# LeSN-Lab/diff-ViT

Hardware: AMD Instinct MI355X
Metric: images/sec DeiT-S int8 224^2 b=256 (quantized forward) (higher is better)
Workload: dtype int8; 1 GPU; deit_small PoT-PTQ forward, bit_config=[8]*50, 224x224, batch 256 per GPU; global_batch=256, parallelism=dp1, streams_per_gpu=3, collective=none, ranks_seen=1, distinct_devices=1

## Files before the change

diff-vit_amd/csrc/p2vit_attn.hip:

```cpp
#include "p2vit_attn_lis.h"

#define WA_HD 32
#define WA_KEYS 64
#define WA_DEAD(kb, r) (NT > 0 && (kb) * 16 + (r) >= NT)
#define WA_PAD(kb, r) (!(NT > 0 && (kb) * 16 + 12 + (r) < NT))
template <int NT, bool TAP>
__global__ __launch_bounds__(256, 3) void k_window_attention(std::conditional_t<TAP, WinAttnArgs, WinAttnKArgs> a) {
  constexpr int VSTRIDE = WA_KEYS + 4;
  __shared__ __attribute__((aligned(16))) int8_t sK[4][WA_KEYS * WA_HD];
  __shared__ __attribute__((aligned(16))) unsigned short sVt[4][WA_HD * VSTRIDE];
  __shared__ float sT[4][232];
  __shared__ __attribute__((aligned(16))) unsigned short sP[4][4][16];
  __shared__ unsigned short sMeta[WA_KEYS + 16];
  __shared__ long long lutE[258];
  __shared__ double lutFR[258];
  const int tid = threadIdx.x, lane = tid & 63, wave = tid >> 6, g = lane >> 4, l15 = lane & 15;
  const int ws = a.wa.ws, N = ws * ws, nW = a.wa.n_windows;
  const int hgroups = (a.H + 3) >> 2;
  const int blk = blockIdx.x;
  const int hg = blk % hgroups, w = (blk / hgroups) % nW, b = blk / (hgroups * nW);
  const int head = hg * 4 + wave;
  const int C = a.H * WA_HD;
  const long long ldq = a.wa.qkv_stride ? a.wa.qkv_stride : 3 * C, ldo = a.wa.out_stride ? a.wa.out_stride : C;
  const bool hok = head < a.H;
  const bool live = lane < N;
  const int rowj = a.wa.win_index[w * N + (live ? lane : 0)];
  const int tsz = (2 * ws - 1) * (2 * ws - 1);
  int8_t tcode[4] = {0, 0, 0, 0};
#pragma unroll
  for (int i = 0; i < 4; ++i)
    if (hok && lane + 64 * i < tsz) tcode[i] = a.wa.table_codes[(lane + 64 * i) * a.H + head];
  int reg_t = 0;
  if (a.wa.region && tid < N) reg_t = (int)a.wa.region[w * N + tid];
  for (int t = tid; t < 258; t += (int)blockDim.x) {
    int xi = -t;
    const int lim = 32 * a.wa.x0_int;
    xi = (xi < lim || t >= 256) ? lim : xi;
    const int q = xi / a.wa.x0_int;
    const int r = xi - a.wa.x0_int * q;
    const long long z = (long long)r * (r + a.wa.b_int) + a.wa.c_int;
    long long e = z << (32 - q);
    e = e < 0 ? 0 : e;
    if (t == 257) e = 0;
    const float ef = t == 257 ? 1.0f : (float)e;
    lutE[t] = e;
    lutFR[t] = 1.0 / (double)ef;
  }
  if (tid < WA_KEYS + 16) {
    const int t = tid < N ? tid : 0;
    sMeta[tid] = (unsigned short)(((t / ws) * (2 * ws - 1) + (t % ws)) | (reg_t << 10));
  }
  const int8_t* hbase = a.qkv + (long long)b * a.T * ldq + head * WA_HD;
  uint4 k0 = make_uint4(0, 0, 0, 0), k1 = k0, v0 = k0, v1 = k0;
  if (hok && live) {
    const int8_t* base = hbase + (long long)rowj * ldq;
    k0 = *reinterpret_cast<const uint4*>(base + C);
    k1 = *reinterpret_cast<const uint4*>(base + C + 16);
    v0 = *reinterpret_cast<const uint4*>(base + 2 * C);
    v1 = *reinterpret_cast<const uint4*>(base + 2 * C + 16);
  }
  int rowq_next = __shfl(rowj, l15 < N ? l15 : N - 1);
  v4i qc_next = {0, 0, 0, 0};
  if (hok) qc_next = *reinterpret_cast<const v4i*>(hbase + (long long)rowq_next * ldq + (g & 1) * 16);
  const float inv_sa = 1.0f / a.wa.s_attn, inv_s2 = 1.0f / a.wa.s_q2;
  const float tb_mul = a.wa.s_table * inv_s2, a1_mul = a.wa.s_attn * inv_s2;
#pragma unroll
  for (int i = 0; i < 4; ++i)
    if (lane + 64 * i < tsz) sT[wave][lane + 64 * i] = (float)tcode[i] * tb_mul;
  {
    *reinterpret_cast<uint4*>(&sK[wave][lane * WA_HD]) = k0;
    *reinterpret_cast<uint4*>(&sK[wave][lane * WA_HD + 16]) = k1;
    const unsigned vw[8] = {v0.x, v0.y, v0.z, v0.w, v1.x, v1.y, v1.z, v1.w};
#pragma unroll
    for (int c = 0; c < WA_HD; ++c) {
      const float f = (float)sx8(vw[c >> 2], c & 3);
      sVt[wave][c * VSTRIDE + lane] = (unsigned short)(__float_as_uint(f) >> 16);
    }
  }
  __syncthreads();
  if (!hok) return;
  const float sigma = a.wa.s_q1 * a.wa.qk_scale;
  const float inv_u = __uint_as_float((unsigned)(254 - (int)(__float_as_uint(sigma) >> 23) + 23) << 23);
  const float sig_m = sigma * inv_u;
  const double sig_int = (double)sig_m;
  const float x_mul = ((1.0f / inv_u) * a.wa.s_q1) * inv_sa;
  const float m100 = (float)(int)(100.0f * inv_s2);
  const float av_mul = (a.wa.s_q1 / a.wa.s_q3) * P2V_PROB_SCALE;
  const int c0 = (ws - 1) * (2 * ws - 1) + (ws - 1);
  const int nqb = (N + 15) >> 4;
  int linj[4][4];
  unsigned regj[4][4];
#pragma unroll
  for (int kb = 0; kb < 4; ++kb)
#pragma unroll
    for (int r = 0; r < 4; ++r) {
      const unsigned mj = sMeta[kb * 16 + 4 * g + r];
      linj[kb][r] = (int)(mj & 1023u);
      regj[kb][r] = mj >> 10;
    }
  for (int qb = 0; qb < nqb; ++qb) {
    const int qi = qb * 16 + l15;
    const int qr = qi < N ? qi : N - 1;
    const int rowq = rowq_next;
    const v4i qc = qc_next;
    if (qb + 1 < nqb) {
      const int qn = qi + 16 < N ? qi + 16 : N - 1;
      rowq_next = __shfl(rowj, qn);
      qc_next = *reinterpret_cast<const v4i*>(hbase + (long long)rowq_next * ldq + (g & 1) * 16);
    }
    unsigned eh[2];
    {
      const unsigned qh[2] = {(unsigned)(g < 2 ? qc[0] : qc[2]), (unsigned)(g < 2 ? qc[1] : qc[3])};
#pragma unroll
      for (int d = 0; d < 2; ++d) {
        float et[4];
#pragma unroll
        for (int e = 0; e < 4; ++e) {
          const float cf = (float)sx8(qh[d], e);
          const float v = cf * sig_m;
          et[e] = __builtin_fmaf(-cf, sig_m, v);
        }
        eh[d] = pack4_pre(et[0], et[1], et[2], et[3]);
      }
    }
    const auto up0 = __builtin_amdgcn_permlane32_swap(0u, eh[0], false, false);
    const auto up1 = __builtin_amdgcn_permlane32_swap(0u, eh[1], false, false);
    const v4i qeta = {(int)up0[0], (int)up1[0], (int)eh[0], (int)eh[1]};
    const v4i fq1 = g < 2 ? qc : (v4i){0, 0, 0, 0};
    const v4i fq2 = g < 2 ? (v4i){0, 0, 0, 0} : qeta;
    v4i s1[4], s2[4];
#pragma unroll
    for (int kb = 0; kb < 4; ++kb) {
      const v4i fk = *reinterpret_cast<const v4i*>(&sK[wave][(kb * 16 + l15) * WA_HD + (g & 1) * 16]);
      s1[kb] = __builtin_amdgcn_mfma_i32_16x16x64_i8(fk, fq1, (v4i){0, 0, 0, 0}, 0, 0, 0);
      s2[kb] = __builtin_amdgcn_mfma_i32_16x16x64_i8(fk, fq2, (v4i){0, 0, 0, 0}, 0, 0, 0);
    }
    const unsigned mi = sMeta[qr];
    const float* trow = &sT[wave][(int)(mi & 1023u) + c0];
    const unsigned reg_i = mi >> 10;
    v4i pb[2];
    if (NT == 49 && qb == 3) {
      const int t = l15 < 13 ? l15 : 12;
      int v1 = s1[0][0], v2 = s2[0][0];
#pragma unroll
      for (int u = 1; u < 13; ++u) {
        const int kb = u < 12 ? u >> 2 : 3, r = u < 12 ? u & 3 : 0;
        v1 = t == u ? s1[kb][r] : v1;
        v2 = t == u ? s2[kb][r] : v2;
      }
      const int j = t < 12 ? (t >> 2) * 16 + 4 * g + (t & 3) : 48 + 4 * g;
      const bool valid = l15 < 13 && j < N;
      const unsigned mj = sMeta[j];
      const double X = __builtin_fma(sig_int, (double)v1, (double)v2);
      const float a1 = __builtin_amdgcn_fmed3f(rintf((float)X * x_mul), -128.f, 127.f);
      const float a2 = __builtin_amdgcn_fmed3f(rintf(__builtin_fmaf(a1, a1_mul, trow[-(int)(mj & 1023u)])), -128.f, 127.f);
      float xi = a2;
      if (a.wa.region) xi -= (mj >> 10) != reg_i ? m100 : 0.f;
      xi = valid ? xi : -3.0e9f;
      float mx = xi;
#define WA_ROWMAX(ctrl) mx = fmaxf(mx, __int_as_float(__builtin_amdgcn_update_dpp(0, __float_as_int(mx), ctrl, 0xF, 0xF, false)));
      WA_ROWMAX(0xB1) WA_ROWMAX(0x4E) WA_ROWMAX(0x141) WA_ROWMAX(0x140)
#undef WA_ROWMAX
      mx = fmaxf(mx, __shfl_xor(mx, 16));
      mx = fmaxf(mx, __shfl_xor(mx, 32));
      const int d = valid ? (int)fminf(mx - xi, 256.f) : 257;
      long long S = lutE[d];
#pragma unroll
      for (int o_ = 1; o_ < 64; o_ <<= 1) S += __shfl_xor(S, o_);
      const double Sd = (double)(float)S;
      const float ratio = rintf((float)(Sd * lutFR[d]));
      const int E = (int)((__float_as_uint(ratio) + 0x00400000u) >> 23);
      if constexpr (TAP) if (valid) {
        const long long trow = (((long long)b * nW + w) * a.H + head) * N + (N - 1);
        if (a.probs_k) a.probs_k[trow * N + j] = (int8_t)(E - 127 > 16 ? 16 : E - 127);
        if (a.probs_kp) a.probs_kp[trow * a.pitch + j] = (int8_t)(E - 127 > 16 ? 16 : E - 127);
        if (a.attn1_codes) a.attn1_codes[trow * a.pitch + j] = (int8_t)(int)a1;
        if (a.qact2_codes) a.qact2_codes[trow * a.pitch + j] = (int8_t)(int)a2;
      }
      sP[wave][g][l15] = (unsigned short)((E < 143 && l15 < 13) ? (143 - E) << 7 : 0);
      __builtin_amdgcn_wave_barrier();
      asm volatile("" ::: "memory");
      pb[0] = *reinterpret_cast<const v4i*>(&sP[wave][g][0]);
      pb[1] = *reinterpret_cast<const v4i*>(&sP[wave][g][8]);
    } else {
      float xs[4][4];
      float mx = -3.0e9f;
      auto scores = [&](auto MASKc) {
        constexpr bool MASK = decltype(MASKc)::value;
#pragma unroll
        for (int kb = 0; kb < 4; ++kb) {
#pragma unroll
          for (int r = 0; r < 4; ++r) {
            if (WA_DEAD(kb, r)) continue;
            const double X = __builtin_fma(sig_int, (double)s1[kb][r], (double)s2[kb][r]);
            const float a1 = __builtin_amdgcn_fmed3f(rintf((float)X * x_mul), -128.f, 127.f);
            const float a2 = __builtin_amdgcn_fmed3f(rintf(__builtin_fmaf(a1, a1_mul, trow[-linj[kb][r]])), -128.f, 127.f);
            float xi = a2;
            if constexpr (TAP) if (qi < N && kb * 16 + 4 * g + r < N) {
              const long long at = ((((long long)b * nW + w) * a.H + head) * N + qi) * a.pitch + kb * 16 + 4 * g + r;
              if (a.attn1_codes) a.attn1_codes[at] = (int8_t)(int)a1;
              if (a.qact2_codes) a.qact2_codes[at] = (int8_t)(int)a2;
            }
            if (MASK) xi -= regj[kb][r] != reg_i ? m100 : 0.f;
            if (WA_PAD(kb, r)) xi = kb * 16 + 4 * g + r < N ? xi : -3.0e9f;
            xs[kb][r] = xi;
            mx = fmaxf(mx, xi);
          }
        }
      };
      if (a.wa.region) scores(std::integral_constant<bool, true>{});
      else scores(std::integral_constant<bool, false>{});
      mx = fmaxf(mx, __shfl_xor(mx, 16));
      mx = fmaxf(mx, __shfl_xor(mx, 32));
      long long S = 0;
#pragma unroll
      for (int kb = 0; kb < 4; ++kb)
#pragma unroll
        for (int r = 0; r < 4; ++r) {
          if (WA_DEAD(kb, r)) continue;
          int d = (int)fminf(mx - xs[kb][r], 256.f);
          if (WA_PAD(kb, r)) d = kb * 16 + 4 * g + r < N ? d : 257;
          s1[kb][r] = d;
          S += lutE[d];
        }
      S += __shfl_xor(S, 16);
      S += __shfl_xor(S, 32);
      const float Sf = (float)S;
      const double Sd = (double)Sf;
#pragma unroll
      for (int p = 0; p < 2; ++p) {
        unsigned pk[4];
#pragma unroll
        for (int e2 = 0; e2 < 4; ++e2) {
          float ratio[2];
#pragma unroll
          for (int e = 0; e < 2; ++e) {
            const int jj = 2 * e2 + e;
            const int kb = 2 * p + (jj >> 2), r = jj & 3;
            if (WA_DEAD(kb, r)) {
              ratio[e] = 4.0e9f;
              continue;
            }
            ratio[e] = rintf((float)(Sd * lutFR[s1[kb][r]]));
            if constexpr (TAP) if (qi < N && kb * 16 + 4 * g + r < N) {
              const int k = (int)((__float_as_uint(ratio[e]) + 0x00400000u) >> 23) - 127;
              const long long trow = (((long long)b * nW + w) * a.H + head) * N + qi;
              if (a.probs_k) a.probs_k[trow * N + kb * 16 + 4 * g + r] = (int8_t)(k > 16 ? 16 : k);
              if (a.probs_kp) a.probs_kp[trow * a.pitch + kb * 16 + 4 * g + r] = (int8_t)(k > 16 ? 16 : k);
            }
          }
          pk[e2] = lis_prob_pair(ratio[0], ratio[1]);
        }
        pb[p] = (v4i){(int)pk[0], (int)pk[1], (int)pk[2], (int)pk[3]};
      }
    }
    v4f o[2] = {(v4f){0.f, 0.f, 0.f, 0.f}, (v4f){0.f, 0.f, 0.f, 0.f}};
#pragma unroll
    for (int p = 0; p < 2; ++p) {
      const v8bf fb = __builtin_bit_cast(v8bf, pb[p]);
#pragma unroll
      for (int dt = 0; dt < 2; ++dt) {
        const unsigned short* vp = &sVt[wave][(dt * 16 + l15) * VSTRIDE + p * 32 + 4 * g];
        const uint2 lo = *reinterpret_cast<const uint2*>(vp);
        const uint2 hi = *reinterpret_cast<const uint2*>(vp + 16);
        v4i va = {(int)lo.x, (int)lo.y, (int)hi.x, (int)hi.y};
        o[dt] = __builtin_amdgcn_mfma_f32_16x16x32_bf16(__builtin_bit_cast(v8bf, va), fb, o[dt], 0, 0, 0);
      }
    }
    if (qi < N) {
      int8_t* dst = a.out + ((long long)b * a.T + rowq) * ldo + head * WA_HD + 4 * g;
#pragma unroll
      for (int dt = 0; dt < 2; ++dt)
        *reinterpret_cast<unsigned*>(dst + dt * 16) = pack4_rne_sat(o[dt][0] * av_mul, o[dt][1] * av_mul, o[dt][2] * av_mul, o[dt][3] * av_mul);
    }
  }
}


int g_attn_waves = 8;
int p2v_launch_window_attention_wide(const WinAttnArgs& a, hipStream_t st);
int p2v_launch_window_attention(const WinAttnArgs& a, hipStream_t st) {
  if (a.wa.ws > 8) return p2v_launch_window_attention_wide(a, st);
  const int hgroups = (a.H + 3) / 4;
  const dim3 grid((unsigned)(a.B * a.wa.n_windows * hgroups));
  if (a.wa.ws == 7) {
    if (a.tapped()) hipLaunchKernelGGL((k_window_attention<49, true>), grid, dim3(256), 0, st, a);
    else hipLaunchKernelGGL((k_window_attention<49, false>), grid, dim3(256), 0, st, a);
  } else {
    if (a.tapped()) hipLaunchKernelGGL((k_window_attention<0, true>), grid, dim3(256), 0, st, a);
    else hipLaunchKernelGGL((k_window_attention<0, false>), grid, dim3(256), 0, st, a);
  }
  CHECK_LAUNCH();
  return 0;
}

int p2v_launch_attention_wide(const AttnArgs& a, int head_dim, int nkb, hipStream_t st);

int g_attn_stream = 0;
int g_attn_packed = 1;
int p2v_attention_kernel_of(int head_dim, int tokens, int tapped) {
  const int resident = p2v_resident_tokens_of(head_dim);
  if (!resident || tokens <= 0 || tokens > P2V_MAX_TOKENS_STREAMED) return -1;
  if (g_attn_stream) return P2V_KERNEL_STREAMING;
  if (tokens <= resident) return P2V_KERNEL_RESIDENT;
  if (g_attn_packed && head_dim == 64 && !tapped && tokens <= P2V_MAX_TOKENS_PACKED) return P2V_KERNEL_PACKED;
  return P2V_KERNEL_STREAMING;
}

int p2v_launch_attention(const AttnArgs& a, int head_dim, hipStream_t st) {
  const int nkb = (a.N + 31) / 32;
  {
    int ex;
    const float m2 = a.at.s_qkv_sq * a.at.inv_s_attn;
    if (!(m2 > 0.f) || frexpf(m2, &ex) != 0.5f) return -2;
  }
  switch (p2v_attention_kernel_of(head_dim, a.N, a.tapped())) {
    case P2V_KERNEL_RESIDENT: break;
    case P2V_KERNEL_PACKED: return p2v_launch_attention_packed(a, st);
    case P2V_KERNEL_STREAMING: return p2v_launch_attention_stream(a, head_dim, st);
    default: return -1;
  }
  if (head_dim == 64) { P2V_ATTN_CASES(64, 19, true) }
  if (head_dim == 32) { P2V_ATTN_CASES(32, 19, false) }
  return p2v_launch_attention_wide(a, head_dim, nkb, st);
}
```

diff-vit_amd/csrc/p2vit_attn_lis.h:

```cpp
#pragma once
#include "p2vit_device.h"

extern int g_attn_waves;


#define P2V_PROB_SCALE 0x1p111f
__device__ __forceinline__ unsigned lis_prob_pair(float r0, float r1) {
  const unsigned hi2 = __builtin_amdgcn_perm(__float_as_uint(r1), __float_as_uint(r0), 0x07060302u);
  const unsigned eb = __builtin_bit_cast(unsigned, __builtin_bit_cast(v2u16, hi2) + (v2u16){0x40, 0x40}) & 0x7F807F80u;
  unsigned out;
  asm("v_pk_sub_u16 %0, %1, %2 clamp" : "=v"(out) : "s"(0x47804780u), "v"(eb));
  return out;
}

__device__ __forceinline__ void lis_table_entry(const p2v_attn& at, int t, long long* lutE, double* lutFR) {
  if (t >= 256) {
    lutE[256] = 0;
    lutFR[256] = 1.0;
    return;
  }
  int xi = -t;
  const int lim = 32 * at.x0_int;
  xi = xi < lim ? lim : xi;
  const int q = xi / at.x0_int;
  const int r = xi - at.x0_int * q;
  const long long z = (long long)r * (r + at.b_int) + at.c_int;
  long long e = z << (32 - q);
  e = e < 0 ? 0 : e;
  lutE[t] = e;
  lutFR[t] = 1.0 / (double)(float)e;
}

#ifdef P2V_DIAG
extern unsigned long long* g_gemm_stamps;
#define AT_STAMP(slot)                                                                                             \
  do {                                                                                                             \
    if (a.stamps && threadIdx.x == 0 && (slot) < 16) a.stamps[(long long)blockIdx.x * 16 + (slot)] = __builtin_readcyclecounter(); \
  } while (0)
#else
#define AT_STAMP(slot) do { } while (0)
#endif
template <int HD, int NKP, bool TAP, bool ISH>
__global__ __launch_bounds__(512, HD > 64 ? 2 : (NKP <= 7 ? 4 : (NKP <= 10 ? 3 : 2))) void k_lis_attention(std::conditional_t<TAP, AttnArgs, AttnKArgs> a) {
  static_assert(HD % 16 == 0 && HD >= 16 && HD <= 128, "head_dim");
  constexpr int KROWS = NKP * 32;
  constexpr int NKB = NKP * 2;
  constexpr int VSTRIDE = KROWS + 4;
  constexpr int CH = HD / 16;
  constexpr int NQ = (CH + 3) / 4;
  constexpr int NDT = HD / 16;
  extern __shared__ __attribute__((aligned(16))) unsigned char smem[];
  int8_t* sK = reinterpret_cast<int8_t*>(smem);
  unsigned short* sVt = reinterpret_cast<unsigned short*>(smem + KROWS * HD);
  unsigned char* lutE = smem + KROWS * HD + HD * VSTRIDE * 2;
  unsigned char* lutFR = lutE + 258 * 8;
  typedef __attribute__((address_space(3))) const long long* lds_i64p;
  typedef __attribute__((address_space(3))) const double* lds_f64p;
  const int ebase = (int)(unsigned)(uintptr_t)(__attribute__((address_space(3))) unsigned char*)lutE;

  const int tid = threadIdx.x, lane = tid & 63, wave = tid >> 6, g = lane >> 4, l15 = lane & 15;
  const int b = blockIdx.x / a.H, head = blockIdx.x % a.H;
  const int N = a.N, D = a.H * HD, ld = 3 * D;
  const int8_t* base = a.qkv + (long long)b * N * ld + head * HD;
  AT_STAMP(0);

  if (tid < 256) {
    int xi = -tid;
    const int lim = 32 * a.at.x0_int;
    xi = xi < lim ? lim : xi;
    const int q = xi / a.at.x0_int;
    const int r = xi - a.at.x0_int * q;
    const long long z = (long long)r * (r + a.at.b_int) + a.at.c_int;
    long long e = z << (32 - q);
    e = e < 0 ? 0 : e;
    const float ef = (float)e;
    reinterpret_cast<long long*>(lutE)[tid] = e;
    reinterpret_cast<double*>(lutFR)[tid] = 1.0 / (double)ef;
    if (tid == 0) {
      reinterpret_cast<long long*>(lutE)[256] = 0;
      reinterpret_cast<double*>(lutFR)[256] = 1.0;
    }
  }
  AT_STAMP(1);
  for (int i0 = tid; i0 < KROWS * CH; i0 += 2 * (int)blockDim.x) {
    uint4 kv[2], vv[2];
#pragma unroll
    for (int u = 0; u < 2; ++u) {
      const int i = i0 + u * (int)blockDim.x;
      const int row = i / CH, c = i % CH;
      kv[u] = make_uint4(0, 0, 0, 0);
      vv[u] = make_uint4(0, 0, 0, 0);
      if (i < KROWS * CH && row < N) {
        kv[u] = *reinterpret_cast<const uint4*>(base + (long long)row * ld + D + c * 16);
        vv[u] = *reinterpret_cast<const uint4*>(base + (long long)row * ld + 2 * D + c * 16);
      }
    }
#pragma unroll
    for (int u = 0; u < 2; ++u) {
      const int i = i0 + u * (int)blockDim.x;
      if (i >= KROWS * CH) break;
      const int row = i / CH, c = i % CH;
      const int sw = (HD == 64) ? (c ^ (((row >> 3) & 1) << 1)) : c;
      *reinterpret_cast<uint4*>(sK + row * HD + sw * 16) = kv[u];
      const unsigned w4[4] = {vv[u].x, vv[u].y, vv[u].z, vv[u].w};
#pragma unroll
      for (int j = 0; j < 16; ++j) {
        const float f = (float)sx8(w4[j >> 2], j & 3);
        sVt[(c * 16 + j) * VSTRIDE + row] = (unsigned short)(__float_as_uint(f) >> 16);
      }
    }
  }

  const float nmm = -(a.at.qk_scale * (a.at.s_qkv_sq * a.at.inv_s_attn));
  const float avm = a.at.av_mul * P2V_PROB_SCALE;
  const int nqb = ((a.nq > 0 && a.nq < N ? a.nq : N) + 15) >> 4;
  const int nwaves = (int)(blockDim.x >> 6);
  AT_STAMP(2);
  v4i fq_next[NQ];
#pragma unroll
  for (int j = 0; j < NQ; ++j) {
    fq_next[j] = (v4i){0, 0, 0, 0};
    if (4 * j + g < CH && wave < nqb) {
      const int qr0 = wave * 16 + l15;
      fq_next[j] = *reinterpret_cast<const v4i*>(base + (long long)(qr0 < N ? qr0 : N - 1) * ld + (4 * j + g) * 16);
    }
  }
  __syncthreads();
  AT_STAMP(3);
  [[maybe_unused]] int stamp_base = 4;
  for (int qb = wave; qb < nqb; qb += nwaves) {
    const int qrow = qb * 16 + l15;
    v4i fq[NQ];
#pragma unroll
    for (int j = 0; j < NQ; ++j) {
      fq[j] = fq_next[j];
      if (4 * j + g < CH && qb + nwaves < nqb) {
        const int qn = (qb + nwaves) * 16 + l15;
        fq_next[j] = *reinterpret_cast<const v4i*>(base + (long long)(qn < N ? qn : N - 1) * ld + (4 * j + g) * 16);
      }
    }
    v4i s[NKB];
#pragma unroll
    for (int kb = 0; kb < NKB; ++kb) {
      const int row = kb * 16 + l15;
#pragma unroll
      for (int j = 0; j < NQ; ++j) {
        const bool live = 4 * j + g < CH;
        const int c = live ? 4 * j + g : 0;
        const int sw = (HD == 64) ? (c ^ (((row >> 3) & 1) << 1)) : c;
        v4i fk = *reinterpret_cast<const v4i*>(sK + row * HD + sw * 16);
        if (!live) fk = (v4i){0, 0, 0, 0};
        if (j == 0) s[kb] = __builtin_amdgcn_mfma_i32_16x16x64_i8(fk, fq[0], (v4i){0, 0, 0, 0}, 0, 0, 0);
        else s[kb] = __builtin_amdgcn_mfma_i32_16x16x64_i8(fk, fq[j], s[kb], 0, 0, 0);
      }
    }
    const bool tail_empty = (NKB - 1) * 16 >= N;
#ifdef P2V_DIAG
    asm volatile("s_nop 0" :: "v"(s[NKB - 1][0]));
#endif
    AT_STAMP(stamp_base);
    long long S = 0;
    [[maybe_unused]] int rowmax = 0;
    if (ISH) {
      const int p = a.pshift, hm1 = (1 << (p - 1)) - 1;
      int mx = -100000;
#pragma unroll
      for (int kb = 0; kb < NKB; ++kb) {
        if (kb == NKB - 1 && tail_empty) continue;
#pragma unroll
        for (int r = 0; r < 4; ++r) {
          const int sv = s[kb][r];
          int code = (int)((unsigned)sv + (unsigned)hm1 + (((unsigned)sv >> p) & 1u)) >> p;
          code = code < -128 ? -128 : (code > 127 ? 127 : code);
          if (kb >= NKB - 2) code = (kb * 16 + 4 * g + r) < N ? code : -100000;
          s[kb][r] = code;
          mx = code > mx ? code : mx;
        }
      }
      {
        int o = __shfl_xor(mx, 16);
        mx = o > mx ? o : mx;
        o = __shfl_xor(mx, 32);
        mx = o > mx ? o : mx;
      }
      if (TAP) rowmax = mx;
      const int mx8 = (mx << 3) + ebase;
#pragma unroll
      for (int kb = 0; kb < NKB; ++kb) {
        if (kb == NKB - 1 && tail_empty) continue;
#pragma unroll
        for (int r = 0; r < 4; ++r) {
          int d8;
          asm("v_mad_i32_i24 %0, %1, -8, %2" : "=v"(d8) : "v"(s[kb][r]), "v"(mx8));
          if (kb >= NKB - 2) d8 = d8 > ebase + 2048 ? ebase + 2048 : d8;
          s[kb][r] = d8;
          S += *(lds_i64p)(uintptr_t)(unsigned)d8;
        }
        __builtin_amdgcn_sched_barrier(0);
      }
    } else {
    int mn = 1000;
#pragma unroll
    for (int kb = 0; kb < NKB; ++kb) {
      if (kb == NKB - 1 && tail_empty) continue;
#pragma unroll
      for (int r = 0; r < 4; ++r) {
        int nc = (int)__builtin_amdgcn_fmed3f(rintf((float)s[kb][r] * nmm), -127.f, 128.f);
        if (kb >= NKB - 2) nc = (kb * 16 + 4 * g + r) < N ? nc : 1000;
        s[kb][r] = nc;
        mn = nc < mn ? nc : mn;
      }
    }
    {
      int o = __shfl_xor(mn, 16);
      mn = o < mn ? o : mn;
      o = __shfl_xor(mn, 32);
      mn = o < mn ? o : mn;
    }
    if (TAP) rowmax = -mn;
    const int neg8mn = -8 * mn + ebase;
#pragma unroll
    for (int kb = 0; kb < NKB; ++kb) {
      if (kb == NKB - 1 && tail_empty) continue;
#pragma unroll
      for (int r = 0; r < 4; ++r) {
        int d8 = (s[kb][r] << 3) + neg8mn;
        if (kb >= NKB - 2) d8 = d8 > ebase + 2048 ? ebase + 2048 : d8;
        s[kb][r] = d8;
        S += *(lds_i64p)(uintptr_t)(unsigned)d8;
      }
      __builtin_amdgcn_sched_barrier(0);
    }
    }
    S += __shfl_xor(S, 16);
    S += __shfl_xor(S, 32);
    const float Sf = (float)S;
    const double Sd = (double)Sf;
    AT_STAMP(stamp_base + 1);

    v4f o[NDT];
#pragma unroll
    for (int dt = 0; dt < NDT; ++dt) o[dt] = (v4f){0.f, 0.f, 0.f, 0.f};
#pragma unroll
    for (int p = 0; p < NKP; ++p) {
      unsigned pk[4];
#pragma unroll
      for (int e2 = 0; e2 < 4; ++e2) {
        float ratio[2];
#pragma unroll
        for (int e = 0; e < 2; ++e) {
          const int j = 2 * e2 + e;
          const int kb = 2 * p + (j >> 2), r = j & 3;
          if (kb == NKB - 1 && tail_empty) {
            ratio[e] = 4.0e9f;
            continue;
          }
          const double rd = ((lds_f64p)(uintptr_t)(unsigned)s[kb][r])[258];
          ratio[e] = rintf((float)(Sd * rd));
          if constexpr (TAP) if (s[kb][r] < ebase + 2048 && qrow < N) {
            int k = (int)((__float_as_uint(ratio[e]) + 0x00400000u) >> 23) - 127;
            const int key = kb * 16 + 4 * g + r;
            const long long trow = ((long long)b * a.H + head) * N + qrow;
            if (a.probs_k) a.probs_k[trow * N + key] = (int8_t)(k > 16 ? 16 : k);
            if (a.probs_kp) a.probs_kp[trow * a.pitch + key] = (int8_t)(k > 16 ? 16 : k);
            if (a.score_codes) a.score_codes[trow * a.pitch + key] = (int8_t)(rowmax - ((s[kb][r] - ebase) >> 3));
          }
        }
        pk[e2] = lis_prob_pair(ratio[0], ratio[1]);
      }
      v4i pb = {(int)pk[0], (int)pk[1], (int)pk[2], (int)pk[3]};
      const v8bf fb = __builtin_bit_cast(v8bf, pb);
#pragma unroll
      for (int dt = 0; dt < NDT; ++dt) {
        const unsigned short* vp = sVt + (dt * 16 + l15) * VSTRIDE + p * 32 + 4 * g;
        const uint2 lo = *reinterpret_cast<const uint2*>(vp);
        const uint2 hi = *reinterpret_cast<const uint2*>(vp + 16);
        v4i va = {(int)lo.x, (int)lo.y, (int)hi.x, (int)hi.y};
        o[dt] = __builtin_amdgcn_mfma_f32_16x16x32_bf16(__builtin_bit_cast(v8bf, va), fb, o[dt], 0, 0, 0);
      }
      __builtin_amdgcn_sched_barrier(0);
    }
#ifdef P2V_DIAG
    asm volatile("s_nop 0" :: "v"(o[NDT - 1][0]));
#endif
    AT_STAMP(stamp_base + 2);
    {
      const int qs = qrow < N ? qrow : N - 1;
      int8_t* dst = a.out + ((long long)b * N + qs) * D + head * HD + 4 * g;
#pragma unroll
      for (int dt = 0; dt < NDT; ++dt)
        *reinterpret_cast<unsigned*>(dst + dt * 16) = pack4_rne_sat(o[dt][0] * avm, o[dt][1] * avm, o[dt][2] * avm, o[dt][3] * avm);
    }
    AT_STAMP(stamp_base + 3);
    stamp_base += 4;
  }
}

template <int HD, int NKB, bool ISH_OK = true>
static int launch_attn_t(const AttnArgs& a_, hipStream_t st) {
  constexpr int KROWS = NKB * 32;
  constexpr size_t smem = (size_t)KROWS * HD + (size_t)HD * (KROWS + 4) * 2 + 258 * 8 + 258 * 8;
  AttnArgs a = a_;
  {
    int ex;
    const float m = a.at.qk_scale * (a.at.s_qkv_sq * a.at.inv_s_attn);
    a.pshift = (m > 0.f && frexpf(m, &ex) == 0.5f && ex <= 0 && ex >= -23) ? 1 - ex : 0;
  }
#ifdef P2V_DIAG
  a.stamps = g_gemm_stamps;
#endif
  const dim3 grid(a.B * a.H), block(64 * g_attn_waves);
#define P2V_ATTN_LAUNCH(TAP_, ISH_)                                                                                          \
  do {                                                                                                                       \
    if (smem > 64 * 1024) {                      \
      static bool granted[16] = {false};                                                                                     \
      int dev = 0;                                                                                                           \
      if (hipGetDevice(&dev) != hipSuccess || dev < 0 || dev >= 16) dev = -1;                                                \
      if (dev < 0 || !granted[dev]) {                                                                                        \
        hipError_t e = hipFuncSetAttribute(reinterpret_cast<const void*>(&k_lis_attention<HD, NKB, TAP_, ISH_>),             \
                                           hipFuncAttributeMaxDynamicSharedMemorySize, (int)smem);                           \
        if (e != hipSuccess) return (int)e;                                                                                  \
        if (dev >= 0) granted[dev] = true;                                                                                   \
      }                                                                                                                      \
    }                                                                                                                        \
    hipLaunchKernelGGL((k_lis_attention<HD, NKB, TAP_, ISH_>), grid, block, smem, st, a);                                    \
  } while (0)
  if constexpr (!ISH_OK) a.pshift = 0;
  if (a.tapped()) {
    if constexpr (ISH_OK) { if (a.pshift) { P2V_ATTN_LAUNCH(true, true); CHECK_LAUNCH(); return 0; } }
    P2V_ATTN_LAUNCH(true, false);
  } else {
    if constexpr (ISH_OK) { if (a.pshift) { P2V_ATTN_LAUNCH(false, true); CHECK_LAUNCH(); return 0; } }
    P2V_ATTN_LAUNCH(false, false);
  }
// ... 16 lines not shown
```

diff-vit_amd/csrc/p2vit_capi.cpp:

```cpp
#include <hip/hip_runtime.h>
#include <math.h>
#include <stdarg.h>
#include <stdio.h>
#include <stdlib.h>
#include <string.h>

#include <initializer_list>
#include <memory>
#include <vector>

#include "p2vit_kernels.h"

static thread_local char g_err[512] = "";

static int fail(int code, const char* fmt, ...) {
  va_list ap;
  va_start(ap, fmt);
  vsnprintf(g_err, sizeof g_err, fmt, ap);
  va_end(ap);
  return code;
}
struct KeepLastError {
  char keep[sizeof g_err];
  KeepLastError() { memcpy(keep, g_err, sizeof keep); }
  ~KeepLastError() { memcpy(g_err, keep, sizeof keep); }
};
static int launch_rc(int rc, const char* what) {
  if (rc == 0) return 0;
  if (rc == -2) return fail(P2V_E_UNSUPPORTED, "%s: s_qkv_sq * inv_s_attn must be a power of two", what);
  if (rc < 0) return fail(P2V_E_UNSUPPORTED, "%s: no kernel instantiated for this shape", what);
  return fail(P2V_E_LAUNCH, "%s: %s", what, hipGetErrorString((hipError_t)rc));
}
static inline int round_up(int v, int m) { return (v + m - 1) / m * m; }
static bool is_pot(float v) {
  int ex;
  return v > 0.f && frexpf(v, &ex) == 0.5f;
}

static int check_lis_consts(const char* who, int x0_int, int b_int, int c_int) {
  if (x0_int >= 0) return fail(P2V_E_ARG, "%s: x0_int must be negative", who);
  if (c_int <= 0 || c_int >= (1 << 24) || b_int < 0 || b_int >= (1 << 23) || x0_int < -(1 << 12))
    return fail(P2V_E_UNSUPPORTED, "%s: log-int-softmax constants out of range (x0 %d, b %d, c %d): softmax input scale below 2^-11?", who, x0_int,
                b_int, c_int);
  return P2V_OK;
}
static int check_requant_scale(const char* who, float inv_s_out) {
  if (!(is_pot(inv_s_out) && inv_s_out >= 0x1p-40f && inv_s_out <= 0x1p40f))
    return fail(P2V_E_UNSUPPORTED, "%s: REQUANT 1/scale %g must be a power of two (it is folded into the column scales)", who, inv_s_out);
  return P2V_OK;
}
static int check_gelu_tab(const char* who, const p2v_gelu_tab& t) {
  if (t.table && (t.cells <= 0 || t.cells > 4096)) return fail(P2V_E_ARG, "%s: GELU table with %d cells", who, t.cells);
  return P2V_OK;
}
static int check_attn(const char* who, const p2v_attn& at) {
  const int rc = check_lis_consts(who, at.x0_int, at.b_int, at.c_int);
  if (rc != P2V_OK) return rc;
  if (!is_pot(at.s_qkv_sq * at.inv_s_attn)) return fail(P2V_E_UNSUPPORTED, "%s: s_qkv_sq * inv_s_attn must be a power of two", who);
  if (!(at.qk_scale > 0.f) || !(at.av_mul > 0.f)) return fail(P2V_E_ARG, "%s: qk_scale and av_mul must be positive", who);
  if (!is_pot(at.av_mul) || at.av_mul > 0x1p15f || at.av_mul < 0x1p-40f)
    return fail(P2V_E_UNSUPPORTED, "%s: av_mul %g must be a power of two in [2^-40, 2^15]", who, at.av_mul);
  return P2V_OK;
}

struct p2v_plan {
  p2v_model_desc d;
  int tokens, patches, k_patch, k_patch_pad, n_layers;
  std::vector<p2v_linear> lin[2];
  std::vector<char> lin_set[2];
  float inv_s_input;
  p2v_epilogue embed_epi;
  const int8_t* cls_codes;
  const int8_t* embed_cls_codes = nullptr;
  bool embed_set;
  std::vector<p2v_block> blocks;
  std::vector<char> block_set;
  p2v_ln final_ln;
  float head_inv_s, head_s;
  bool head_set;
  std::vector<float*> ln_pre_buf;
  float* final_pre_buf = nullptr;
  std::vector<char> block_folded;
  std::vector<const float*> resid_tab;
  std::vector<float*> resid_buf;
  int device = -1;
  ~p2v_plan() {
    int prev = -1;
    const bool sw = device >= 0 && hipGetDevice(&prev) == hipSuccess && prev != device && hipSetDevice(device) == hipSuccess;
    for (float* b : ln_pre_buf)
      if (b) (void)hipFree(b);
    for (float* b : resid_buf)
      if (b) (void)hipFree(b);
    if (final_pre_buf) (void)hipFree(final_pre_buf);
    if (sw) (void)hipSetDevice(prev);
  }
};

static void build_resid_tables(p2v_plan* plan, int block);
static int bit_index(int bits) { return bits == 4 ? 0 : (bits == 8 ? 1 : -1); }
template <class Block>
static auto& block_ln(Block& b, int i) { return i < 2 ? b.ln1[i] : b.ln2[(i - 2) >> 1][(i - 2) & 1]; }
static bool ln_constants_present(const p2v_ln& l, bool with_mask = true) {
  return (l.mask || !with_mask) && l.gamma && l.beta && l.inv_out && l.post_mul;
}

extern "C" {

extern int g_ln_generic;
extern int g_ln_rows;
extern int g_attn_waves;
extern int g_ln_gemm;
extern int g_ln_gemm_ver;
extern int g_gemm_tile;
extern int g_resid_pre;
extern int g_attn_stream;
extern int g_attn_packed;
extern int g_ln_pre;
extern int g_gemm_rows;
int g_cls_rows = 1;

enum { ANY_ENV = 1, ANY_API = 2 };
static const struct Switch {
  const char *name, *env;
  int* var;
  int lo, hi, step, any;
  bool takes(int v, int how) const { return (any & how) || (v >= lo && v <= hi && (v - lo) % step == 0); }
  void set(int v) const { *var = (hi == 1 && lo == 0) ? v != 0 : v; }
} kSwitches[] = {
    {"attn_waves", "P2V_ATTN_WAVES", &g_attn_waves, 4, 8, 1, 0},
    {"ln_gemm", "P2V_LN_GEMM", &g_ln_gemm, 0, 1, 1, ANY_ENV | ANY_API},
    {"ln_gemm_version", "P2V_LN_GEMM_V", &g_ln_gemm_ver, 1, 3, 1, 0},
    {"gemm_tile", "P2V_GEMM_TILE", &g_gemm_tile, 0, 256, 128, 0},
    {"attn_stream", "P2V_ATTN_STREAM", &g_attn_stream, 0, 1, 1, ANY_ENV | ANY_API},
    {"attn_packed", "P2V_ATTN_PACKED", &g_attn_packed, 0, 1, 1, 0},
    {"ln_pre", "P2V_LN_PRE", &g_ln_pre, 0, 1, 1, ANY_ENV | ANY_API},
    {"resid_pre", "P2V_RESID_PRE", &g_resid_pre, 0, 1, 1, ANY_ENV | ANY_API},
    {"gemm_rows", "P2V_GEMM_ROWS", &g_gemm_rows, 0, 2, 1, 0},
    {"cls_rows", "P2V_CLS_ROWS", &g_cls_rows, 0, 1, 1, ANY_ENV},
    {"ln_rows", "P2V_LN_ROWS", &g_ln_rows, 1, 64, 1, 0},
    {"ln_generic", "P2V_LN_GENERIC", &g_ln_generic, 0, 1, 1, ANY_API},
};

static void read_env_once() {
  static bool done = false;
  if (done) return;
  done = true;
  for (const Switch& s : kSwitches) {
    const char* e = getenv(s.env);
    if (e && s.takes(atoi(e), ANY_ENV)) s.set(atoi(e));
  }
}
int p2v_abi_version(void) { read_env_once(); return P2V_ABI_VERSION; }

int p2v_resident_tokens(int head_dim) { return p2v_resident_tokens_of(head_dim); }
int p2v_max_tokens(int head_dim) { return p2v_resident_tokens_of(head_dim) ? P2V_MAX_TOKENS_STREAMED : 0; }
int p2v_packed_tokens(int head_dim) { return head_dim == 64 ? P2V_MAX_TOKENS_PACKED : 0; }
int p2v_attention_kernel(int head_dim, int tokens, int tapped) {
  read_env_once();
  return p2v_attention_kernel_of(head_dim, tokens, tapped);
}

int p2v_set_tuning(const char* name, int value) {
  if (!name) return fail(P2V_E_ARG, "p2v_set_tuning: null name");
  read_env_once();
  for (const Switch& s : kSwitches)
    if (!strcmp(name, s.name) && s.takes(value, ANY_API)) {
      s.set(value);
      return P2V_OK;
    }
  return fail(P2V_E_ARG, "p2v_set_tuning: unknown switch or value out of range: %s = %d", name, value);
}
const char* p2v_last_error(void) { return g_err; }

int p2v_plan_create(const p2v_model_desc* desc, p2v_plan** out) {
  if (!desc || !out) return fail(P2V_E_ARG, "p2v_plan_create: null argument");
  read_env_once();
  if (desc->abi_version != P2V_ABI_VERSION) return fail(P2V_E_ARG, "ABI version %d != %d", desc->abi_version, P2V_ABI_VERSION);
  const p2v_model_desc& d = *desc;
  if (d.img_size <= 0 || d.patch_size <= 0 || d.img_size % d.patch_size) return fail(P2V_E_SHAPE, "img_size %% patch_size != 0");
  if (d.patch_size % 4) return fail(P2V_E_UNSUPPORTED, "patch_size must be a multiple of 4");
  if (d.embed_dim % d.num_heads) return fail(P2V_E_SHAPE, "embed_dim %% num_heads != 0");
  const int hd = d.embed_dim / d.num_heads;
  if (hd != 32 && hd != 48 && hd != 64 && hd != 80 && hd != 96 && hd != 128)
    return fail(P2V_E_UNSUPPORTED, "head_dim %d (32, 48, 64, 80, 96 and 128 are instantiated)", hd);
  if (d.embed_dim % 16 || d.mlp_hidden % 16) return fail(P2V_E_UNSUPPORTED, "embed_dim and mlp_hidden must be multiples of 16");
  {
    const int tokens = (d.img_size / d.patch_size) * (d.img_size / d.patch_size) + 1;
    if (tokens > P2V_MAX_TOKENS_STREAMED)
      return fail(P2V_E_UNSUPPORTED, "%d tokens per image: the attention kernels cover up to %d", tokens, P2V_MAX_TOKENS_STREAMED);
  }
  if (d.embed_dim > 2048) return fail(P2V_E_UNSUPPORTED, "embed_dim %d: the LayerNorm kernel covers up to 2048 channels", d.embed_dim);
  p2v_plan* p = new p2v_plan();
  p->d = d;
  p->patches = (d.img_size / d.patch_size) * (d.img_size / d.patch_size);
  p->tokens = p->patches + 1;
  p->k_patch = d.in_chans * d.patch_size * d.patch_size;
  p->k_patch_pad = round_up(p->k_patch, GBK_PAD);
  p->n_layers = 4 * d.depth + 2;
  for (int b = 0; b < 2; ++b) {
    p->lin[b].assign(p->n_layers, p2v_linear{nullptr, nullptr, nullptr, nullptr, 0});
    p->lin_set[b].assign(p->n_layers, 0);
  }
  p->blocks.resize(d.depth);
  p->block_set.assign(d.depth, 0);
  p->ln_pre_buf.assign(d.depth, nullptr);
  p->block_folded.assign(d.depth, 0);
  p->resid_tab.assign((size_t)d.depth * 4, nullptr);
  p->resid_buf.assign(d.depth, nullptr);
  p->embed_set = p->head_set = false;
  p->cls_codes = nullptr;
  *out = p;
  return P2V_OK;
}

void p2v_plan_destroy(p2v_plan* plan) { delete plan; }

int p2v_plan_set_linear(p2v_plan* plan, int layer, int bits, const p2v_linear* lin) {
  if (!plan || !lin) return fail(P2V_E_ARG, "p2v_plan_set_linear: null argument");
  const int bi = bit_index(bits);
  if (bi < 0) return fail(P2V_E_BITS, "bits %d not in {4, 8}", bits);
  if (layer < 0 || layer >= plan->n_layers) return fail(P2V_E_ARG, "layer %d out of range [0,%d)", layer, plan->n_layers);
  if (!lin->w_codes || !lin->colscale || !lin->bias) return fail(P2V_E_ARG, "p2v_plan_set_linear: null device pointer");
  if (lin->packed4 && bits != 4) return fail(P2V_E_BITS, "packed4 weights for a %d-bit layer", bits);
  plan->lin[bi][layer] = *lin;
  plan->lin_set[bi][layer] = 1;
  if (layer >= 1 && layer < plan->n_layers - 1 && ((layer - 1) & 1)) {
    const int block = (layer - 1) / 4;
    if (plan->block_set[block]) build_resid_tables(plan, block);
  }
  return P2V_OK;
}

int p2v_plan_set_embed(p2v_plan* plan, float inv_s_input, const p2v_epilogue* e, const int8_t* cls_row_codes) {
  if (!plan || !e || !cls_row_codes) return fail(P2V_E_ARG, "p2v_plan_set_embed: null argument");
  plan->inv_s_input = inv_s_input;
  plan->embed_epi = *e;
  plan->embed_epi.patches = plan->patches;
  plan->cls_codes = cls_row_codes;
  plan->embed_set = true;
  return P2V_OK;
}

int p2v_plan_set_embed_tap_cls(p2v_plan* plan, const int8_t* cls_embed_codes) {
  if (!plan || !cls_embed_codes) return fail(P2V_E_ARG, "p2v_plan_set_embed_tap_cls: null argument");
  plan->embed_cls_codes = cls_embed_codes;
  return P2V_OK;
}

struct OwnerDevice {
  int prev = -1, own = -1;
  explicit OwnerDevice(const void* ptr) {
    hipPointerAttribute_t pa;
    if (hipGetDevice(&prev) != hipSuccess || hipPointerGetAttributes(&pa, ptr) != hipSuccess) {
      (void)hipGetLastError();
      return;
    }
    if (pa.type != hipMemoryTypeDevice && pa.type != hipMemoryTypeManaged) return;
    own = pa.device;
    if (own != prev && hipSetDevice(own) != hipSuccess) own = -1;
  }
  ~OwnerDevice() { if (own >= 0 && own != prev) (void)hipSetDevice(prev); }
  bool ok() const { return own >= 0; }
};

static size_t resid_tab_floats(int N) { return (size_t)((N + 127) / 128) * 6 * 128; }

static int resid_prefold_impl(const p2v_linear& lin, const p2v_epilogue& ep, int N, float* tab, int* usable, hipStream_t st) {
  *usable = 0;
  unsigned* flags = nullptr;
  hipError_t e = hipMalloc(&flags, 2 * sizeof(unsigned));
  const unsigned init[2] = {1u, 0u};
  unsigned got[2] = {0u, 0u};
  if (e == hipSuccess) e = hipMemcpyAsync(flags, init, sizeof init, hipMemcpyHostToDevice, st);
  int rc = 0;
  if (e == hipSuccess) rc = p2v_launch_resid_prefold(lin, ep, N, tab, flags, st);
  if (e == hipSuccess && rc == 0) e = hipMemcpyAsync(got, flags, sizeof got, hipMemcpyDeviceToHost, st);
  if (e == hipSuccess && rc == 0) e = hipStreamSynchronize(st);
  if (flags) (void)hipFree(flags);
  if (e != hipSuccess) {
    (void)hipGetLastError();
    return fail(P2V_E_LAUNCH, "resid_prefold: %s", hipGetErrorString(e));
  }
  if (rc) return launch_rc(rc, "resid_prefold");
  *usable = got[0] ? 1 : 0;
  return P2V_OK;
}

static void build_resid_tables(p2v_plan* plan, int block) {
  KeepLastError keep;
  for (int j = 0; j < 4; ++j) plan->resid_tab[(size_t)block * 4 + j] = nullptr;
  if (!plan->block_set[block]) return;
  const p2v_block& blk = plan->blocks[block];
  OwnerDevice dev(blk.proj_epi.s_mid);
  if (!dev.ok() || (plan->device >= 0 && plan->device != dev.own)) return;
  const int D = plan->d.embed_dim;
  const size_t per = resid_tab_floats(D);
  if (hipDeviceSynchronize() != hipSuccess) { (void)hipGetLastError(); return; }
  float* buf = plan->resid_buf[block];
  if (!buf && hipMalloc(&buf, 4 * per * sizeof(float)) != hipSuccess) { (void)hipGetLastError(); return; }
  plan->resid_buf[block] = buf;
  plan->device = dev.own;
  for (int which = 0; which < 2; ++which)
    for (int bi = 0; bi < 2; ++bi) {
      const int layer = 1 + 4 * block + (which ? 3 : 1);
      if (!plan->lin_set[bi][layer]) continue;
      int usable = 0;
      float* tab = buf + (size_t)(which * 2 + bi) * per;
      if (resid_prefold_impl(plan->lin[bi][layer], which ? blk.fc2_epi : blk.proj_epi, D, tab, &usable, nullptr) == P2V_OK && usable)
        plan->resid_tab[(size_t)block * 4 + which * 2 + bi] = tab;
    }
}

static hipError_t fold_one_ln(const p2v_ln& l, int C, float* dev, p2v_ln_pre* out) {
  const int Cp = round_up(C, 256);
  std::vector<float> g(C), b(C), io(C), pm(C), host((size_t)2 * Cp, 0.f);
  hipError_t e = hipMemcpy(g.data(), l.gamma, C * sizeof(float), hipMemcpyDeviceToHost);
  if (e == hipSuccess) e = hipMemcpy(b.data(), l.beta, C * sizeof(float), hipMemcpyDeviceToHost);
  if (e == hipSuccess) e = hipMemcpy(io.data(), l.inv_out, C * sizeof(float), hipMemcpyDeviceToHost);
  if (e == hipSuccess) e = hipMemcpy(pm.data(), l.post_mul, C * sizeof(float), hipMemcpyDeviceToHost);
  if (e != hipSuccess) return e;
  float* go = host.data();
  float* bo = go + Cp;
  int pot = 1, pm1 = 1;
  float gmin = 3.0e38f, gmax = 0.f, bmax = 0.f;
  for (int c = 0; c < C; ++c) {
    unsigned ib;
    memcpy(&ib, &io[c], 4);
    const int p2 = (int)((ib & 0x807FFFFFu) == 0u) & (int)((ib >> 23) - 32u <= 190u);
    go[c] = g[c] * io[c];
    bo[c] = b[c] * io[c];
    const float ga = fabsf(go[c]), ba = fabsf(bo[c]);
    const int gok = (int)(g[c] == 0.f) | ((int)(ga >= 1.0e-30f) & (int)(ga <= 1.0e30f));
    const int bok = (int)(b[c] == 0.f) | ((int)(ba >= 1.0e-30f) & (int)(ba <= 1.0e30f));
    pot &= p2 & gok & bok;
    pm1 &= (int)(pm[c] == 1.f);
    gmin = fminf(gmin, ga);
    gmax = fmaxf(gmax, ga);
    bmax = fmaxf(bmax, ba);
  }
  e = hipMemcpy(dev, host.data(), host.size() * sizeof(float), hipMemcpyHostToDevice);
  if (e == hipSuccess) *out = p2v_ln_pre{dev, dev + Cp, gmin, gmax, bmax, pot, pm1};
  return e;
}
static const p2v_ln_pre kNoPre = {nullptr, nullptr, 0.f, 0.f, 0.f, 0, 0};

static bool fold_ln_constants(p2v_plan* plan, int block) {
  const int C = plan->d.embed_dim, Cp = round_up(C, 256);
  p2v_block& blk = plan->blocks[block];
  for (int i = 0; i < 6; ++i) block_ln(blk, i).pre = kNoPre;
  OwnerDevice own(blk.ln1[0].gamma);
  if (!own.ok()) {
    fail(P2V_OK, "p2v_plan_set_block: LayerNorm constants of block %d not folded at plan time (cannot locate the device of gamma)", block);
    return false;
  }
  if (plan->device >= 0 && plan->device != own.own) {
    fail(P2V_OK, "p2v_plan_set_block: block %d lives on device %d, earlier blocks on device %d: not folded at plan time", block, own.own, plan->device);
    return false;
  }
  hipError_t e = hipDeviceSynchronize();
  float* dev = plan->ln_pre_buf[block];
  if (e == hipSuccess && !dev) e = hipMalloc(&dev, (size_t)12 * Cp * sizeof(float));
  p2v_ln_pre pre[6];
  if (e == hipSuccess) {
    plan->ln_pre_buf[block] = dev;
    plan->device = own.own;
    for (int i = 0; i < 6 && e == hipSuccess; ++i) e = fold_one_ln(block_ln(blk, i), C, dev + (size_t)(2 * i) * Cp, &pre[i]);
  }
  if (e != hipSuccess) {
    (void)hipGetLastError();
    fail(P2V_OK, "p2v_plan_set_block: LayerNorm constants of block %d not folded at plan time (%s)", block, hipGetErrorString(e));
    return false;
  }
  for (int i = 0; i < 6; ++i) block_ln(blk, i).pre = pre[i];
  return true;
}

int p2v_plan_set_block(p2v_plan* plan, int block, const p2v_block* blk) {
  if (!plan || !blk) return fail(P2V_E_ARG, "p2v_plan_set_block: null argument");
  if (block < 0 || block >= plan->d.depth) return fail(P2V_E_ARG, "block %d out of range", block);
  int rc = check_attn("p2v_plan_set_block: attn", blk->attn);
  if (rc == P2V_OK) rc = check_gelu_tab("p2v_plan_set_block: gelu_fc1", blk->gelu_fc1);
  for (int b = 0; b < 2 && rc == P2V_OK; ++b) rc = check_requant_scale("p2v_plan_set_block: inv_s_qkv", blk->inv_s_qkv[b]);
  if (rc == P2V_OK && !(is_pot(blk->inv_s_fc1) && blk->inv_s_fc1 >= 0x1p-40f && blk->inv_s_fc1 <= 0x1p40f))
    rc = fail(P2V_E_UNSUPPORTED, "p2v_plan_set_block: 1/scale of mlp.qact1 %g must be a power of two", blk->inv_s_fc1);
  if (rc == P2V_OK && (!blk->proj_epi.s_mid || !blk->proj_epi.s_res || !blk->proj_epi.s_next || !blk->fc2_epi.s_mid || !blk->fc2_epi.s_res ||
                       !blk->fc2_epi.s_next))
    rc = fail(P2V_E_ARG, "p2v_plan_set_block: RESID epilogues need s_mid/s_res/s_next");
  for (int i = 0; i < 6 && rc == P2V_OK; ++i)
    if (!ln_constants_present(block_ln(*blk, i))) rc = fail(P2V_E_ARG, "p2v_plan_set_block: LayerNorm constants missing");
  if (rc != P2V_OK) return rc;
  plan->blocks[block] = *blk;
  plan->block_set[block] = 1;
  g_err[0] = 0;
  plan->block_folded[block] = fold_ln_constants(plan, block) ? 1 : 0;
  build_resid_tables(plan, block);
  return P2V_OK;
}

int p2v_plan_block_prefolded(const p2v_plan* plan, int block) {
  if (!plan || block < 0 || block >= plan->d.depth) return fail(P2V_E_ARG, "p2v_plan_block_prefolded: bad argument");
  return plan->block_folded[block] ? 1 : 0;
}

int p2v_plan_resid_prefolded(const p2v_plan* plan, int block) {
  if (!plan || block < 0 || block >= plan->d.depth) return fail(P2V_E_ARG, "p2v_plan_resid_prefolded: bad argument");
  int m = 0;
  for (int j = 0; j < 4; ++j) m |= plan->resid_tab[(size_t)block * 4 + j] ? 1 << j : 0;
  return m;
}

int p2v_plan_set_head(p2v_plan* plan, const p2v_ln* final_ln, float inv_s_out, float s_out) {
  if (!plan || !final_ln) return fail(P2V_E_ARG, "p2v_plan_set_head: null argument");
  if (!ln_constants_present(*final_ln))
    return fail(P2V_E_ARG, "p2v_plan_set_head: LayerNorm constants missing");
  if (!(inv_s_out > 0.f) || !(s_out > 0.f)) return fail(P2V_E_ARG, "p2v_plan_set_head: act_out scale must be positive");
  plan->final_ln = *final_ln;
  plan->final_ln.pre = kNoPre;
  {
    OwnerDevice own(final_ln->gamma);
    const int C = plan->d.embed_dim;
    if (own.ok() && (plan->device < 0 || plan->device == own.own) && hipDeviceSynchronize() == hipSuccess) {
      if (!plan->final_pre_buf && hipMalloc(&plan->final_pre_buf, (size_t)2 * round_up(C, 256) * sizeof(float)) != hipSuccess) plan->final_pre_buf = nullptr;
      p2v_ln_pre pre;
      if (plan->final_pre_buf && fold_one_ln(*final_ln, C, plan->final_pre_buf, &pre) == hipSuccess) {
        plan->final_ln.pre = pre;
        plan->device = own.own;
      }
    }
    (void)hipGetLastError();
  }
  plan->head_inv_s = inv_s_out;
  plan->head_s = s_out;
  plan->head_set = true;
  return P2V_OK;
}

struct WsLayout {
  size_t patches, x, ln, qkv, att, hid, cls, total;
};
static WsLayout ws_layout(const p2v_plan* p, int batch) {
  auto al = [](size_t v) { return (v + 255) / 256 * 256; };
  const size_t M = (size_t)batch * p->tokens, D = p->d.embed_dim;
  WsLayout w;
  size_t off = 0;
  w.patches = off; off += al((size_t)batch * p->patches * p->k_patch_pad);
  w.x = off;       off += al(M * D);
  w.ln = off;      off += al(M * D);
  w.qkv = off;     off += al(M * 3 * D);
  w.att = off;     off += al(M * D);
  w.hid = off;     off += al(M * (size_t)p->d.mlp_hidden);
  w.cls = off;     off += al((size_t)batch * D);
  w.total = off + 256;
  return w;
}

size_t p2v_workspace_bytes(const p2v_plan* plan, int batch) {
  if (!plan || batch <= 0) return 0;
  return ws_layout(plan, batch).total;
}

long long p2v_workspace_view(const p2v_plan* plan, int batch, const char* name) {
  if (!plan || !name || batch <= 0) return -1;
  const WsLayout w = ws_layout(plan, batch);
  const struct { const char* name; size_t off; } views[] = {{"patches", w.patches}, {"x", w.x}, {"ln", w.ln}, {"qkv", w.qkv}, {"att", w.att}, {"hid", w.hid}, {"cls", w.cls}};
  for (const auto& v : views)
    if (!strcmp(name, v.name)) return (long long)v.off;
  return -1;
}

}

static GemmArgs gemm_args(const int8_t* A, int lda, int M, const int8_t* W, int K, int N, const p2v_linear& lin, const p2v_epilogue& ep,
                          void* out, int ldo, int8_t* out_codes) {
  GemmArgs g;
  g.A = A; g.lda = lda; g.M = M; g.W = W; g.K = K; g.N = N; g.w4 = lin.packed4 ? 1 : 0;
  g.colscale = lin.colscale; g.bias = lin.bias; g.ep = ep; g.out = out; g.ldo = ldo; g.out_codes = out_codes; g.out_codes2 = nullptr; g.tiles_n = 0;
#ifdef P2V_DIAG
  g.stamps = nullptr;
#endif
  return g;
}

static int run_gemm(int epi, const int8_t* A, int lda, int M, int K, int N, const p2v_linear& lin, const p2v_epilogue& ep, void* out,
                    int ldo, int8_t* out_codes, hipStream_t st, bool few_rows = false) {
  const GemmArgs g = gemm_args(A, lda, M, lin.w_codes, K, N, lin, ep, out, ldo, out_codes);
  if (few_rows && g_gemm_rows != 2 && g_gemm_tile == 0 && !(epi == P2V_EPI_RESID && out_codes)) return launch_rc(p2v_launch_gemm_rows(epi, g, st), "gemm_rows");
  return launch_rc(p2v_launch_gemm(epi, g, st), "gemm_i8");
}

static int run_ln_gemm(int epi, const LnArgs& a, const p2v_linear& lin, const p2v_epilogue& ep, int N, int8_t* out, hipStream_t st) {
  if (!lin.w_frag) return fail(P2V_E_UNSUPPORTED, "ln_gemm: the layer has no fragment-order weights (p2v_linear.w_frag)");
  const int rc = p2v_launch_ln_gemm(epi, a, gemm_args(nullptr, a.C, (int)a.rows, lin.w_frag, round_up(a.C, GBK_PAD), N, lin, ep, out, N, nullptr), st);
  if (rc == -3) return fail(P2V_E_UNSUPPORTED, "ln_gemm: shape C=%d N=%d is not fused", a.C, N);
  return launch_rc(rc, "ln_gemm");
}

struct Prof {
  std::vector<hipEvent_t> ev;
  std::vector<int> kind;
  int used = 0;
  bool make_pool(int n) {
    ev.resize(n);
    kind.reserve(n);
    for (int i = 0; i < n; ++i)
      if (hipEventCreate(&ev[i]) != hipSuccess) { ev.resize(i); return false; }
    return true;
  }
  ~Prof() { for (hipEvent_t e : ev) (void)hipEventDestroy(e); }
};
static int prof_pool_size(const p2v_plan* p) { return p ? 7 * p->d.depth + 10 : 0; }

struct DdvCtx {
  int n;
  unsigned long long* partials;
  long long slots;
  double* sums;
  float* tap;
  int stage;
  float* scratch = nullptr;
  int8_t* attn = nullptr;
};
static int ddv_reduce(DdvCtx* c, const void* base, int rows, int cols, int dtype, const float* scale, hipStream_t st, long long sample_stride = 0,
                      long long row_stride = 0) {
  const size_t esz = dtype == P2V_COS_F32 ? 4 : 1;
  if (!row_stride) row_stride = cols;
  if (!sample_stride) sample_stride = (long long)rows * row_stride;
  const p2v_cos_layer l{base, reinterpret_cast<const char*>(base) + (size_t)c->n * sample_stride * esz, scale, sample_stride, row_stride, rows, cols, dtype};
  const CosDesc d = p2v_cos_desc(l, c->n, 0);
  if ((long long)c->n * d.nsplit > c->slots)
    return fail(P2V_E_WORKSPACE, "p2v_forward_ddv: a stage of %d x %d needs %lld partials, the workspace holds %lld", rows, cols,
                (long long)c->n * d.nsplit, c->slots);
  const int rc = launch_rc(p2v_launch_pair_cosine_one(d, c->n, c->partials, c->sums + (size_t)c->stage * c->n * 3, st), "pair_cosine");
  ++c->stage;
  return rc;
}

struct FwdOpts {
  const float* images = nullptr;
  const uint8_t* u8 = nullptr;
  int layout = 0;
  const void* lut = nullptr;
  int stop_after = -1;
  Prof* prof = nullptr;
  float *const *qkv_tap = nullptr, *const *fc1_tap = nullptr;
  float* const* lin_tap = nullptr;
  DdvCtx* ddv = nullptr;
};

struct RowSet {
  int rows;
  long long stride;
  int nq;
  bool few;
};

struct Fwd {
  const p2v_plan* p;
  const FwdOpts& o;
  hipStream_t st;
  int batch, D, T, M, Hd, hd, Dk, Hk;
  int8_t *P, *X, *LN, *QKV, *ATT, *HID, *CLS;
  int launched = 0;
  bool done = false;

  Fwd(const p2v_plan* plan, const FwdOpts& opts, int batch_, const WsLayout& w, void* workspace, hipStream_t stream)
      : p(plan), o(opts), st(stream), batch(batch_) {
    int8_t* ws = reinterpret_cast<int8_t*>(workspace);
    P = ws + w.patches; X = ws + w.x; LN = ws + w.ln; QKV = ws + w.qkv; ATT = ws + w.att; HID = ws + w.hid; CLS = ws + w.cls;
    D = p->d.embed_dim; T = p->tokens; M = batch * T; Hd = p->d.mlp_hidden; hd = D / p->d.num_heads; Dk = round_up(D, GBK_PAD); Hk = round_up(Hd, GBK_PAD);
  }

  template <class Launch>
  int step(int kind, Launch&& launch) {
    done = done || (o.stop_after >= 0 && launched >= o.stop_after);
    if (done) return P2V_OK;
    if (Prof* prof = o.prof) {
      if (prof->used + 1 >= (int)prof->ev.size()) return fail(P2V_E_LAUNCH, "profile: event pool exhausted");
      hipEventRecord(prof->ev[prof->used++], st);
      prof->kind.push_back(kind);
    }
    const int rc = launch();
    if (rc == P2V_OK) launched += (kind == P2V_K_LN_GEMM_QKV || kind == P2V_K_LN_GEMM_FC1) ? 2 : 1;
    return rc;
  }
  int lin_tap(int layer, const int8_t* A, int lda, int rows, int K, int N, const p2v_linear& lin) {
    if (done || !o.lin_tap || !o.lin_tap[layer]) return P2V_OK;
    return run_gemm(P2V_EPI_F32, A, lda, rows, K, N, lin, p2v_epilogue{}, o.lin_tap[layer], N, nullptr, st);
  }
  int ddv_i8(const void* buf, int rows, int cols, const float* scale) { return (done || !o.ddv) ? P2V_OK : ddv_reduce(o.ddv, buf, rows, cols, P2V_COS_I8, scale, st); }
  int ddv_f32(const void* buf, int rows, int cols) { return (done || !o.ddv) ? P2V_OK : ddv_reduce(o.ddv, buf, rows, cols, P2V_COS_F32, nullptr, st); }
  int ddv_i8_deq(const void* buf, int rows, int cols, const float* scale) { return (done || !o.ddv) ? P2V_OK : ddv_reduce(o.ddv, buf, rows, cols, P2V_COS_I8_DEQ, scale, st); }
  int ddv_tap(int rows, int cols) { return (o.ddv && o.ddv->tap) ? ddv_f32(o.ddv->tap, rows, cols) : P2V_OK; }
  float* full() const { return (!done && o.ddv) ? o.ddv->scratch : nullptr; }
  int layernorm(const LnArgs& a) { return step(P2V_K_LAYERNORM, [&] { return launch_rc(p2v_launch_layernorm(a, st), "int_layernorm"); }); }
  int gemm(int kind, bool few, int epi, const int8_t* A, int lda, int rows, int K, int N, const p2v_linear& lin, const p2v_epilogue& ep, void* out, int ldo,
           int8_t* out_codes = nullptr) {
    return step(kind, [&] { return run_gemm(epi, A, lda, rows, K, N, lin, ep, out, ldo, out_codes, st, few); });
  }
  int ln_linear(int k_fused, int k_gemm, int epi, long long stride, int rows, const p2v_ln& norm, const p2v_linear& lin, const p2v_epilogue& e, int N,
                int8_t* out, bool few) {
    LnArgs ln{X, stride, rows, D, norm, LN, D};
    ln.pre = norm.pre;
    if (float* vals = full()) {
      ln.tap_out = vals;
      int rc = layernorm(ln);
      if (rc || (rc = ddv_f32(vals, T, D))) return rc;
      return gemm(k_gemm, few, epi, LN, D, rows, Dk, N, lin, e, out, N);
    }
    if (!few && lin.w_frag && p2v_ln_gemm_supported(epi, D, N, e.gelu.table ? e.gelu.cells : 0)) {
      if (o.stop_after < 0) ln.out = nullptr;
      return step(k_fused, [&] { return run_ln_gemm(epi, ln, lin, e, N, out, st); });
    }
    const int rc = layernorm(ln);
    return rc ? rc : gemm(k_gemm, few, epi, LN, D, rows, Dk, N, lin, e, out, N);
  }

  int block(int i, const int8_t* bc, const RowSet& rs) {
    const p2v_block& b = p->blocks[i];
    const int bq = bit_index(bc[0]), bp = bit_index(bc[1]), b1 = bit_index(bc[2]), b2 = bit_index(bc[3]);
    const p2v_linear &qkv = p->lin[bq][1 + 4 * i], &proj = p->lin[bp][2 + 4 * i], &fc1 = p->lin[b1][3 + 4 * i], &fc2 = p->lin[b2][4 + 4 * i];
    const int ldx = (int)rs.stride;
    int rc;
    p2v_epilogue eq{};
    eq.inv_s_out = b.inv_s_qkv[bq];
    eq.tap_out = o.qkv_tap ? o.qkv_tap[i] : (o.lin_tap ? o.lin_tap[1 + 4 * i] : nullptr);
    if ((rc = ln_linear(P2V_K_LN_GEMM_QKV, P2V_K_GEMM_QKV, P2V_EPI_REQUANT, D, M, b.ln1[bq], qkv, eq, 3 * D, QKV, false))) return rc;
    if ((rc = ddv_tap(T, 3 * D)) || (rc = ddv_i8(QKV, T, 3 * D, nullptr))) return rc;
    AttnArgs at{{QKV, batch, T, p->d.num_heads, b.attn, ATT, nullptr}};
    at.nq = rs.nq;
    int8_t* planes = (!done && o.ddv) ? o.ddv->attn : nullptr;
    const int pitch = round_up(T, 16), HT = p->d.num_heads * T;
    if (planes) {
      at.score_codes = planes;
      at.probs_kp = planes + (size_t)batch * HT * pitch;
      at.pitch = pitch;
    }
    if ((rc = step(P2V_K_ATTENTION, [&] { return launch_rc(p2v_launch_attention(at, hd, st), "lis_attention"); }))) return rc;
    if (planes && !done &&
        ((rc = ddv_reduce(o.ddv, at.score_codes, HT, T, P2V_COS_I8, nullptr, st, 0, pitch)) ||
         (rc = ddv_reduce(o.ddv, at.probs_kp, HT, T, P2V_COS_LOG2K, nullptr, st, 0, pitch))))
      return rc;
    if ((rc = ddv_i8(ATT, T, D, nullptr))) return rc;
    p2v_epilogue ep = b.proj_epi;
    ep.residual = X;
    ep.resid_tab = p->resid_tab[(size_t)i * 4 + bp];
    if ((rc = gemm(P2V_K_GEMM_PROJ, rs.few, P2V_EPI_RESID, ATT, ldx, rs.rows, Dk, D, proj, ep, X, ldx, full() ? LN : nullptr))) return rc;
    if ((rc = lin_tap(2 + 4 * i, ATT, ldx, rs.rows, Dk, D, proj)) || (rc = ddv_tap(T, D))) return rc;
    if (full() && (rc = ddv_i8_deq(LN, T, D, b.proj_epi.s_mid))) return rc;
    if ((rc = ddv_i8(X, T, D, b.proj_epi.s_next))) return rc;
    p2v_epilogue e1{};
    e1.inv_s_out = b.inv_s_fc1;
    e1.gelu = b.gelu_fc1;
    e1.tap_out = o.fc1_tap ? o.fc1_tap[i] : (o.lin_tap ? o.lin_tap[3 + 4 * i] : nullptr);
    if ((rc = ln_linear(P2V_K_LN_GEMM_FC1, P2V_K_GEMM_FC1, P2V_EPI_GELU, rs.stride, rs.rows, b.ln2[bq][b1], fc1, e1, Hd, HID, rs.few))) return rc;
    if ((rc = ddv_tap(T, Hd)) || (rc = ddv_i8(HID, T, Hd, nullptr))) return rc;
    p2v_epilogue e2 = b.fc2_epi;
    e2.residual = X;
    e2.resid_tab = p->resid_tab[(size_t)i * 4 + 2 + b2];
    if ((rc = gemm(P2V_K_GEMM_FC2, rs.few, P2V_EPI_RESID, HID, Hd, rs.rows, Hk, D, fc2, e2, X, ldx, full() ? LN : nullptr))) return rc;
    if ((rc = lin_tap(4 + 4 * i, HID, Hd, rs.rows, Hk, D, fc2)) || (rc = ddv_tap(T, D))) return rc;
    if (full() && (rc = ddv_i8_deq(LN, T, D, b.fc2_epi.s_mid))) return rc;
    return ddv_i8(X, T, D, b.fc2_epi.s_next);
  }
};

static int forward_impl(p2v_plan* p, int batch, const int8_t* bit_config, int n_cfg, float* logits, void* workspace, size_t workspace_bytes,
                        void* stream, const FwdOpts& o) {
  if (!p || !(o.images || o.u8) || !bit_config || !logits || !workspace) return fail(P2V_E_ARG, "p2v_forward: null argument");
  if (batch <= 0) return fail(P2V_E_SHAPE, "batch must be positive");
  if (n_cfg != p->n_layers) return fail(P2V_E_BITS, "bit_config has %d entries, model needs %d", n_cfg, p->n_layers);
  for (int i = 0; i < n_cfg; ++i) {
    const int bi = bit_index(bit_config[i]);
    if (bi < 0) return fail(P2V_E_BITS, "%d is not in list", (int)bit_config[i]);
    if (!p->lin_set[bi][i]) return fail(P2V_E_STATE, "layer %d has no %d-bit weights", i, (int)bit_config[i]);
  }
  if (!p->embed_set || !p->head_set) return fail(P2V_E_STATE, "plan incomplete (embed/head)");
  for (int i = 0; i < p->d.depth; ++i)
    if (!p->block_set[i]) return fail(P2V_E_STATE, "plan incomplete (block %d)", i);
  const WsLayout w = ws_layout(p, batch);
  if (workspace_bytes < w.total) return fail(P2V_E_WORKSPACE, "workspace %zu < %zu bytes", workspace_bytes, w.total);
  if (o.lin_tap && o.lin_tap[0] && !(p->inv_s_input > 0.f))
    return fail(P2V_E_UNSUPPORTED, "p2v_forward_linear_taps: no patch-embed tap for input_quant = False (the fp32-image convolution); pass NULL for taps[0]");
  const p2v_model_desc& d = p->d;
  Fwd f(p, o, batch, w, workspace, (hipStream_t)stream);
  const hipStream_t st = f.st;
  const int D = f.D, T = f.T, Kp = p->k_patch_pad, rows_p = batch * p->patches;
  int rc;

  const p2v_linear& embed = p->lin[bit_index(bit_config[0])][0];
  if (p->inv_s_input > 0.f) {
    rc = f.step(P2V_K_PATCHIFY, [&] {
      return o.u8 ? launch_rc(p2v_launch_u8_patchify(o.u8, batch, d.in_chans, d.img_size, d.img_size, d.patch_size, o.layout, (const int8_t*)o.lut, f.P, Kp, st), "u8_patchify")
                  : launch_rc(p2v_launch_patchify(o.images, batch, d.in_chans, d.img_size, d.img_size, d.patch_size, p->inv_s_input, f.P, Kp, st), "quantize_patchify");
    });
    if (rc) return rc;
    if (f.full()) {
      int8_t *pe = f.QKV, *em = f.QKV + (size_t)f.M * D;
      GemmArgs g = gemm_args(f.P, Kp, rows_p, embed.w_codes, Kp, D, embed, p->embed_epi, f.X, D, pe);
      g.out_codes2 = em;
      if ((rc = f.ddv_i8(f.P, p->patches, Kp, nullptr)) ||
          (rc = f.step(P2V_K_GEMM_EMBED, [&] { return launch_rc(p2v_launch_gemm(P2V_EPI_EMBED, g, st), "gemm_i8"); })) ||
          (rc = ddv_reduce(o.ddv, pe + D, p->patches, D, P2V_COS_I8, nullptr, st, (long long)T * D)) ||
          (rc = launch_rc(p2v_launch_fill_cls(em, batch, T, D, p->embed_cls_codes, st), "fill_cls")) ||
          (rc = f.ddv_i8(em, T, D, nullptr)))
        return rc;
    } else if ((rc = f.gemm(P2V_K_GEMM_EMBED, false, P2V_EPI_EMBED, f.P, Kp, rows_p, Kp, D, embed, p->embed_epi, f.X, D))) {
      return rc;
    }
    if ((rc = f.lin_tap(0, f.P, Kp, rows_p, Kp, D, embed))) return rc;
  } else {
    if (embed.packed4) return fail(P2V_E_UNSUPPORTED, "input_quant = False: the patch-embed weights must be unpacked codes (packed4 = 0)");
    const GemmArgs g = gemm_args(nullptr, 0, rows_p, embed.w_codes, Kp, D, embed, p->embed_epi, f.X, D, nullptr);
    rc = f.step(P2V_K_GEMM_EMBED, [&] {
      return o.u8 ? launch_rc(p2v_launch_embed_u8(o.u8, o.layout, (const float*)o.lut, batch, d.in_chans, d.img_size, d.img_size, d.patch_size, g, st), "embed_u8")
                  : launch_rc(p2v_launch_embed_fp32(o.images, batch, d.in_chans, d.img_size, d.img_size, d.patch_size, g, st), "embed_fp32");
    });
    if (rc) return rc;
  }
  if ((rc = f.step(P2V_K_FILL_CLS, [&] { return launch_rc(p2v_launch_fill_cls(f.X, batch, T, D, p->cls_codes, st), "fill_cls"); })) ||
      (rc = f.ddv_i8(f.X, T, D, p->embed_epi.s_next)))
    return rc;

  const bool cls_only = g_cls_rows && o.stop_after < 0 && !o.qkv_tap && !o.fc1_tap && !o.lin_tap && !o.ddv && (long long)T * D <= 0x7fffffffLL;
  const RowSet all_rows{f.M, D, 0, false}, cls_rows{batch, (long long)T * D, 1, true};
  for (int i = 0; i < d.depth && !f.done; ++i)
    if ((rc = f.block(i, bit_config + 1 + 4 * i, (cls_only && i == d.depth - 1) ? cls_rows : all_rows))) return rc;

  if (float* vals = f.full()) {
    LnArgs la{f.X, D, f.M, D, p->final_ln, f.LN, D};
    la.pre = p->final_ln.pre;
    la.tap_out = vals;
    if ((rc = launch_rc(p2v_launch_layernorm(la, st), "int_layernorm")) || (rc = f.ddv_f32(vals, T, D))) return rc;
  }
  LnArgs lf{f.X, (long long)T * D, batch, D, p->final_ln, f.CLS, D};
  lf.pre = p->final_ln.pre;
  if ((rc = f.layernorm(lf)) || (rc = f.ddv_i8(f.CLS, 1, D, nullptr))) return rc;
  const p2v_linear& head = p->lin[bit_index(bit_config[n_cfg - 1])][n_cfg - 1];
  p2v_epilogue eh{};
  eh.inv_s_out = p->head_inv_s;
  eh.s_out = p->head_s;
  if ((rc = f.gemm(P2V_K_GEMM_HEAD, false, P2V_EPI_HEAD, f.CLS, D, batch, f.Dk, d.num_classes, head, eh, logits, d.num_classes))) return rc;
  if ((rc = f.lin_tap(n_cfg - 1, f.CLS, D, batch, f.Dk, d.num_classes, head)) || (rc = f.ddv_tap(1, d.num_classes)) ||
      (rc = f.ddv_f32(logits, 1, d.num_classes)))
    return rc;
  if (f.done) return P2V_OK;
  if (Prof* prof = o.prof) {
    if (prof->used + 2 > (int)prof->ev.size()) return fail(P2V_E_LAUNCH, "profile: event pool exhausted");
    hipEventRecord(prof->ev[prof->used++], st);
    hipEventRecord(prof->ev[prof->used++], st);
    prof->kind.push_back(P2V_K_EVENT_GAP);
  }
  return P2V_OK;
}

extern "C" {

int p2v_forward(p2v_plan* p, const float* images, int batch, const int8_t* bit_config, int n_cfg, float* logits, void* workspace,
                size_t workspace_bytes, int stop_after, void* stream) {
  FwdOpts o;
  o.images = images; o.stop_after = stop_after;
  return forward_impl(p, batch, bit_config, n_cfg, logits, workspace, workspace_bytes, stream, o);
}

static int check_u8_input(const char* what, const uint8_t* img, int layout, const void* lut) {
  if (!img || !lut) return fail(P2V_E_ARG, "%s: null images or lut", what);
  if (layout != P2V_LAYOUT_NCHW && layout != P2V_LAYOUT_NHWC) return fail(P2V_E_ARG, "%s: unknown layout %d (P2V_LAYOUT_NCHW = 0, NHWC = 1)", what, layout);
  if (reinterpret_cast<uintptr_t>(img) & 3) return fail(P2V_E_ARG, "%s: images must start on a 4-byte boundary", what);
  return P2V_OK;
}

int p2v_forward_u8(p2v_plan* p, const uint8_t* images, int layout, const void* lut, int batch, const int8_t* bit_config, int n_cfg,
                   float* logits, void* workspace, size_t workspace_bytes, int stop_after, void* stream) {
  const int rc = check_u8_input("p2v_forward_u8", images, layout, lut);
  if (rc) return rc;
  FwdOpts o;
  o.u8 = images; o.layout = layout; o.lut = lut; o.stop_after = stop_after;
  return forward_impl(p, batch, bit_config, n_cfg, logits, workspace, workspace_bytes, stream, o);
}

int p2v_forward_taps(p2v_plan* p, const float* images, int batch, const int8_t* bit_config, int n_cfg, float* logits, void* workspace,
                     size_t workspace_bytes, float* const* qkv_out, float* const* fc1_out, void* stream) {
  FwdOpts o;
  o.images = images; o.qkv_tap = qkv_out; o.fc1_tap = fc1_out;
  return forward_impl(p, batch, bit_config, n_cfg, logits, workspace, workspace_bytes, stream, o);
}

int p2v_forward_linear_taps(p2v_plan* p, const float* images, int batch, const int8_t* bit_config, int n_cfg, float* logits, void* ws,
                            size_t ws_bytes, float* const* taps, void* stream) {
  if (!taps) return fail(P2V_E_ARG, "p2v_forward_linear_taps: null taps array");
  FwdOpts o;
  o.images = images; o.lin_tap = taps;
  return forward_impl(p, batch, bit_config, n_cfg, logits, ws, ws_bytes, stream, o);
}

static int prof_collect(Prof& prof, float* ms_out, int32_t* kind_out, int max_launches) {
  hipEventSynchronize(prof.ev[prof.used - 1]);
  int n = (int)prof.kind.size();
  n = n < max_launches ? n : max_launches;
  for (int i = 0; i < n; ++i) {
    float ms = 0.f;
    hipEventElapsedTime(&ms, prof.ev[i], prof.ev[i + 1]);
    ms_out[i] = ms;
    kind_out[i] = prof.kind[i];
  }
  return n;
}

int p2v_forward_profile_begin(p2v_plan* p, const float* images, int batch, const int8_t* bit_config, int n_cfg, float* logits, void* workspace,
                              size_t workspace_bytes, void* stream, void** token) {
  if (!p || !token) return fail(P2V_E_ARG, "p2v_forward_profile_begin: null argument");
  *token = nullptr;
  std::unique_ptr<Prof> prof(new Prof());
  if (!prof->make_pool(prof_pool_size(p))) return fail(P2V_E_LAUNCH, "hipEventCreate failed");
  FwdOpts o;
  o.images = images; o.prof = prof.get();
  const int rc = forward_impl(p, batch, bit_config, n_cfg, logits, workspace, workspace_bytes, stream, o);
  if (rc == P2V_OK) *token = prof.release();
  return rc;
}

int p2v_forward_profile_end(void* token, float* ms_out, int32_t* kind_out, int max_launches) {
  if (!token) return fail(P2V_E_ARG, "p2v_forward_profile_end: null argument");
  Prof* prof = reinterpret_cast<Prof*>(token);
  int n = 0;
  if (ms_out && kind_out && max_launches > 0) n = prof_collect(*prof, ms_out, kind_out, max_launches);
  else hipEventSynchronize(prof->ev[prof->used - 1]);
  delete prof;
  return n;
}

int p2v_forward_profile(p2v_plan* p, const float* images, int batch, const int8_t* bit_config, int n_cfg, float* logits, void* workspace,
                        size_t workspace_bytes, void* stream, float* ms_out, int32_t* kind_out, int max_launches) {
  if (!p || !ms_out || !kind_out || max_launches <= 0) return fail(P2V_E_ARG, "p2v_forward_profile: null argument");
  void* token;
  const int rc = p2v_forward_profile_begin(p, images, batch, bit_config, n_cfg, logits, workspace, workspace_bytes, stream, &token);
  return rc == P2V_OK ? p2v_forward_profile_end(token, ms_out, kind_out, max_launches) : rc;
}

static int check_patchify_shape(int chans, int height, int width, int patch, int k_pad) {
  if (patch <= 0 || patch % 4 || height % patch || width % patch) return fail(P2V_E_SHAPE, "image %dx%d not divisible into %d-patches", height, width, patch);
  if (k_pad % 4 || k_pad < chans * patch * patch) return fail(P2V_E_ARG, "k_pad %d too small / unaligned", k_pad);
  return P2V_OK;
}

int p2v_quantize_patchify(const float* img, int batch, int chans, int height, int width, int patch, float inv_s, int8_t* out,
                          int k_pad, void* stream) {
  if (!img || !out) return fail(P2V_E_ARG, "p2v_quantize_patchify: null argument");
  if (const int rc = check_patchify_shape(chans, height, width, patch, k_pad)) return rc;
  return launch_rc(p2v_launch_patchify(img, batch, chans, height, width, patch, inv_s, out, k_pad, (hipStream_t)stream), "quantize_patchify");
}

int p2v_u8_patchify(const uint8_t* img, int layout, const void* lut_i8, int batch, int chans, int height, int width, int patch, int8_t* out,
                    int k_pad, void* stream) {
  int rc = check_u8_input("p2v_u8_patchify", img, layout, lut_i8);
  if (rc) return rc;
  if (!out) return fail(P2V_E_ARG, "p2v_u8_patchify: null argument");
  if (batch <= 0 || chans <= 0) return fail(P2V_E_SHAPE, "p2v_u8_patchify: batch %d, %d channels", batch, chans);
  if ((rc = check_patchify_shape(chans, height, width, patch, k_pad))) return rc;
  return launch_rc(p2v_launch_u8_patchify(img, batch, chans, height, width, patch, layout, (const int8_t*)lut_i8, out, k_pad, (hipStream_t)stream),
                   "u8_patchify");
}

int p2v_gemm_i8(int kind, const int8_t* A, int lda, int M, int K, int N, const p2v_linear* lin, const p2v_epilogue* epi, void* out,
                int ldo, int8_t* out_codes, void* stream) {
  if (!A || !lin || !epi || !out) return fail(P2V_E_ARG, "p2v_gemm_i8: null argument");
  if (kind < P2V_EPI_REQUANT || kind > P2V_EPI_HEAD) return fail(P2V_E_ARG, "unknown epilogue %d", kind);
  if (M <= 0 || N <= 0 || K <= 0 || K % GBK_PAD) return fail(P2V_E_SHAPE, "K=%d must be a positive multiple of %d", K, GBK_PAD);
  if (kind != P2V_EPI_HEAD && (N % 16 || ldo % 16)) return fail(P2V_E_UNSUPPORTED, "N and ldo must be multiples of 16 for int8 outputs");
  if (lda % 16) return fail(P2V_E_UNSUPPORTED, "lda must be a multiple of 16");
  if (lda <= 0 || ldo < N) return fail(P2V_E_SHAPE, "p2v_gemm_i8: lda=%d must be positive and ldo=%d must cover the %d outputs of a row", lda, ldo, N);
  if (kind == P2V_EPI_REQUANT && check_requant_scale("p2v_gemm_i8", epi->inv_s_out) != P2V_OK) return P2V_E_UNSUPPORTED;
  if (kind == P2V_EPI_GELU && check_gelu_tab("p2v_gemm_i8", epi->gelu) != P2V_OK) return P2V_E_ARG;
  if (kind == P2V_EPI_RESID && (!epi->s_mid || !epi->s_res || !epi->s_next || !epi->residual)) return fail(P2V_E_ARG, "RESID epilogue needs s_mid/s_res/s_next/residual");
  if (kind == P2V_EPI_EMBED && (!epi->s_next || !epi->pos_deq || epi->patches <= 0)) return fail(P2V_E_ARG, "EMBED epilogue needs s_next/pos_deq/patches");
  if (kind == P2V_EPI_RESID && out_codes) {
    if ((uintptr_t)out_codes % 16 || (uintptr_t)out % 16) return fail(P2V_E_ARG, "p2v_gemm_i8: RESID out_codes and out must be 16-byte aligned");
    if (lin->packed4) return fail(P2V_E_UNSUPPORTED, "p2v_gemm_i8: the RESID mid-code tap takes int8-stored weights (packed4 = 0); p2v_gemm_resid_tap takes both");
  }
  if (kind != P2V_EPI_RESID && kind != P2V_EPI_HEAD) out_codes = nullptr;
  return run_gemm(kind, A, lda, M, K, N, *lin, *epi, out, ldo, out_codes, (hipStream_t)stream);
}

int p2v_gemm_resid_tap(const int8_t* A, int lda, int M, int K, int N, const p2v_linear* lin, const p2v_epilogue* epi, int8_t* out, int ldo,
                       int8_t* out_codes, void* stream) {
  if (!A || !lin || !epi || !out || !out_codes) return fail(P2V_E_ARG, "p2v_gemm_resid_tap: null argument");
  if (M <= 0 || N <= 0 || K <= 0 || K % GBK_PAD) return fail(P2V_E_SHAPE, "K=%d must be a positive multiple of %d", K, GBK_PAD);
  if (N % 16 || ldo % 16 || lda % 16) return fail(P2V_E_UNSUPPORTED, "p2v_gemm_resid_tap: N, lda and ldo must be multiples of 16");
  if (lda <= 0 || ldo < N) return fail(P2V_E_SHAPE, "p2v_gemm_resid_tap: lda=%d must be positive and ldo=%d must cover the %d outputs of a row", lda, ldo, N);
  if (!epi->s_mid || !epi->s_res || !epi->s_next || !epi->residual) return fail(P2V_E_ARG, "RESID epilogue needs s_mid/s_res/s_next/residual");
  if ((uintptr_t)out_codes % 16 || (uintptr_t)out % 16) return fail(P2V_E_ARG, "p2v_gemm_resid_tap: out_codes and out must be 16-byte aligned");
  if ((long long)M * ldo >= (1LL << 32)) return fail(P2V_E_SHAPE, "p2v_gemm_resid_tap: M * ldo = %lld passes the 32-bit offsets of the tapped stores", (long long)M * ldo);
  return run_gemm(P2V_EPI_RESID, A, lda, M, K, N, *lin, *epi, out, ldo, out_codes, (hipStream_t)stream);
}

int p2v_gemm_embed_tap(const int8_t* A, int lda, int M, int K, int N, const p2v_linear* lin, const p2v_epilogue* epi, int8_t* out, int ldo,
                       int8_t* pe_codes, int8_t* embed_codes, void* stream) {
  if (!A || !lin || !epi || !out || !pe_codes || !embed_codes) return fail(P2V_E_ARG, "p2v_gemm_embed_tap: null argument");
  if (M <= 0 || N <= 0 || K <= 0 || K % GBK_PAD) return fail(P2V_E_SHAPE, "K=%d must be a positive multiple of %d", K, GBK_PAD);
  if (N % 16 || ldo % 16 || lda % 16) return fail(P2V_E_UNSUPPORTED, "p2v_gemm_embed_tap: N, lda and ldo must be multiples of 16");
  if (lda <= 0 || ldo < N) return fail(P2V_E_SHAPE, "p2v_gemm_embed_tap: lda=%d must be positive and ldo=%d must cover the %d outputs of a row", lda, ldo, N);
  if (!epi->s_next || !epi->pos_deq || epi->patches <= 0) return fail(P2V_E_ARG, "EMBED epilogue needs s_next/pos_deq/patches");
  if ((uintptr_t)out % 16 || (uintptr_t)pe_codes % 16 || (uintptr_t)embed_codes % 16)
    return fail(P2V_E_ARG, "p2v_gemm_embed_tap: out, pe_codes and embed_codes must be 16-byte aligned");
  GemmArgs g = gemm_args(A, lda, M, lin->w_codes, K, N, *lin, *epi, out, ldo, pe_codes);
  g.out_codes2 = embed_codes;
  return launch_rc(p2v_launch_gemm(P2V_EPI_EMBED, g, (hipStream_t)stream), "gemm_i8");
}

size_t p2v_ln_prefold_bytes(int C) { return C > 0 ? (size_t)2 * round_up(C, 256) * sizeof(float) : 0; }

int p2v_ln_prefold(p2v_ln* ln, int C, float* buf, size_t buf_bytes) {
  if (!ln || !buf) return fail(P2V_E_ARG, "p2v_ln_prefold: null argument");
  ln->pre = kNoPre;
  if (C <= 0 || C % 4 || C > P2V_LN_MAX_C) return fail(P2V_E_SHAPE, "p2v_ln_prefold: C must be a positive multiple of 4 up to %d", P2V_LN_MAX_C);
  if (!ln_constants_present(*ln, false)) return fail(P2V_E_ARG, "p2v_ln_prefold: LayerNorm constants missing");
  if (buf_bytes < p2v_ln_prefold_bytes(C)) return fail(P2V_E_WORKSPACE, "p2v_ln_prefold: buffer %zu < %zu bytes", buf_bytes, p2v_ln_prefold_bytes(C));
  OwnerDevice own(buf);
  if (!own.ok()) return fail(P2V_E_ARG, "p2v_ln_prefold: buf is not a device pointer");
  hipError_t e = hipDeviceSynchronize();
  p2v_ln_pre pre;
  if (e == hipSuccess) e = fold_one_ln(*ln, C, buf, &pre);
  if (e != hipSuccess) {
    (void)hipGetLastError();
    return fail(P2V_E_LAUNCH, "p2v_ln_prefold: %s", hipGetErrorString(e));
  }
  ln->pre = pre;
  return P2V_OK;
}

size_t p2v_resid_prefold_bytes(int N) { return N > 0 ? resid_tab_floats(N) * sizeof(float) : 0; }

int p2v_resid_prefold(const p2v_linear* lin, const p2v_epilogue* epi, int N, float* tab, size_t tab_bytes, int* usable, void* stream) {
  if (!lin || !epi || !tab || !usable) return fail(P2V_E_ARG, "p2v_resid_prefold: null argument");
  *usable = 0;
  if (N <= 0) return fail(P2V_E_SHAPE, "p2v_resid_prefold: N must be positive");
  if (!lin->colscale || !lin->bias || !epi->s_mid || !epi->s_res || !epi->s_next) return fail(P2V_E_ARG, "p2v_resid_prefold: needs colscale / bias / s_mid / s_res / s_next");
  if (tab_bytes < p2v_resid_prefold_bytes(N)) return fail(P2V_E_WORKSPACE, "p2v_resid_prefold: table %zu < %zu bytes", tab_bytes, p2v_resid_prefold_bytes(N));
  OwnerDevice dev(tab);
  if (!dev.ok()) return fail(P2V_E_ARG, "p2v_resid_prefold: tab is not a device pointer");
  return resid_prefold_impl(*lin, *epi, N, tab, usable, (hipStream_t)stream);
}

int p2v_int_layernorm(const int8_t* x, long long row_stride, int rows, int C, const p2v_ln* ln, int8_t* out, long long out_stride,
                      void* stream) {
  if (!x || !ln || !out) return fail(P2V_E_ARG, "p2v_int_layernorm: null argument");
  if (C % 4 || row_stride % 4 || out_stride % 4) return fail(P2V_E_UNSUPPORTED, "C and strides must be multiples of 4");
  if (rows <= 0) return fail(P2V_E_SHAPE, "rows must be positive");
  if (C <= 0 || row_stride < 0 || out_stride < C) return fail(P2V_E_SHAPE, "p2v_int_layernorm: C=%d must be positive, row_stride non-negative, out_stride >= C", C);
  if (C > P2V_LN_MAX_C) return fail(P2V_E_SHAPE, "p2v_int_layernorm: C=%d, the LayerNorm kernels cover up to %d channels", C, P2V_LN_MAX_C);
  if (C > 2048 && row_stride < C)
    return fail(P2V_E_SHAPE, "p2v_int_layernorm: C=%d beyond 2048 channels needs row_stride >= C (got %lld)", C, row_stride);
  LnArgs a{x, row_stride, rows, C, *ln, out, out_stride};
  a.pre = ln->pre;
  return launch_rc(p2v_launch_layernorm(a, (hipStream_t)stream), "int_layernorm");
}

int p2v_int_layernorm_tap(const int8_t* x, long long row_stride, int rows, int C, const p2v_ln* ln, int8_t* out, long long out_stride,
                          float* tap_out, void* stream) {
  if (!x || !ln || !out || !tap_out) return fail(P2V_E_ARG, "p2v_int_layernorm_tap: null argument");
  if (C % 4 || row_stride % 4 || out_stride % 4) return fail(P2V_E_UNSUPPORTED, "C and strides must be multiples of 4");
  if (rows <= 0) return fail(P2V_E_SHAPE, "rows must be positive");
  if (C <= 0 || row_stride < 0 || out_stride < C) return fail(P2V_E_SHAPE, "p2v_int_layernorm_tap: C=%d must be positive, row_stride non-negative, out_stride >= C", C);
  if (C > 2048) return fail(P2V_E_UNSUPPORTED, "p2v_int_layernorm_tap: C=%d, the value tap covers rows of up to 2048 channels", C);
  if ((uintptr_t)tap_out % 16) return fail(P2V_E_ARG, "p2v_int_layernorm_tap: tap_out must be 16-byte aligned");
  LnArgs a{x, row_stride, rows, C, *ln, out, out_stride};
  a.pre = ln->pre;
  a.tap_out = tap_out;
  return launch_rc(p2v_launch_layernorm(a, (hipStream_t)stream), "int_layernorm");
}

int p2v_ln_gemm_i8(int kind, const int8_t* x, long long row_stride, int M, int C, const p2v_ln* ln, int N, const p2v_linear* lin,
                   const p2v_epilogue* epi, int8_t* out, int ldo, int8_t* ln_out, void* stream) {
  if (!x || !ln || !lin || !epi || !out) return fail(P2V_E_ARG, "p2v_ln_gemm_i8: null argument");
  if (kind != P2V_EPI_REQUANT && kind != P2V_EPI_GELU) return fail(P2V_E_ARG, "p2v_ln_gemm_i8: epilogue %d (REQUANT and GELU are fused)", kind);
  if (M <= 0 || C <= 0 || N <= 0) return fail(P2V_E_SHAPE, "p2v_ln_gemm_i8: bad shape");
  if (C % 4 || row_stride % 4 || N % 16 || ldo != N) return fail(P2V_E_UNSUPPORTED, "p2v_ln_gemm_i8: C, row_stride multiples of 4; N multiple of 16; ldo == N");
  if (row_stride < 0) return fail(P2V_E_SHAPE, "p2v_ln_gemm_i8: negative row_stride");
  if (kind == P2V_EPI_REQUANT && check_requant_scale("p2v_ln_gemm_i8", epi->inv_s_out) != P2V_OK) return P2V_E_UNSUPPORTED;
  if (kind == P2V_EPI_GELU && check_gelu_tab("p2v_ln_gemm_i8", epi->gelu) != P2V_OK) return P2V_E_ARG;
  read_env_once();
  LnArgs a{x, row_stride, M, C, *ln, ln_out, C};
  a.pre = ln->pre;
  return run_ln_gemm(kind, a, *lin, *epi, N, out, (hipStream_t)stream);
}

int p2v_ln_gemm_fusable(int kind, int C, int N, int cells) {
  read_env_once();
  return (C > 0 && N > 0 && cells >= 0 && cells <= 4096 && p2v_ln_gemm_supported(kind, C, N, cells)) ? 1 : 0;
}

static int check_tap_planes(const char* who, int row, int pitch, std::initializer_list<const void*> planes) {
  bool any = false;
  for (const void* q : planes) any = any || q;
  if (!any) return P2V_OK;
  if (pitch < row || pitch % 16) return fail(P2V_E_ARG, "%s: pitch %d must be a multiple of 16 and at least the row length %d", who, pitch, row);
  for (const void* q : planes)
    if ((uintptr_t)q % 16) return fail(P2V_E_ARG, "%s: the tap planes must be 16-byte aligned", who);
  return P2V_OK;
}

static int lis_attention(const char* who, const int8_t* qkv, int batch, int tokens, int heads, int head_dim, const p2v_attn* at, int min_rows,
                         int query_rows, int8_t* out, int8_t* probs_k, void* stream, int8_t* score_codes = nullptr, int8_t* probs_kp = nullptr,
                         int pitch = 0) {
  if (!qkv || !at || !out) return fail(P2V_E_ARG, "%s: null argument", who);
  if (batch <= 0 || tokens <= 0 || heads <= 0) return fail(P2V_E_SHAPE, "bad attention shape");
  if (query_rows < min_rows || query_rows > tokens) return fail(P2V_E_SHAPE, "%s: query_rows %d outside 1 .. %d", who, query_rows, tokens);
  const int rc = check_attn(who, *at);
  if (rc != P2V_OK) return rc;
  const int rp = check_tap_planes(who, tokens, pitch, {score_codes, probs_kp});
  if (rp != P2V_OK) return rp;
  AttnArgs a{{qkv, batch, tokens, heads, *at, out, probs_k}};
  a.nq = query_rows;
  a.score_codes = score_codes; a.probs_kp = probs_kp; a.pitch = pitch;
  return launch_rc(p2v_launch_attention(a, head_dim, (hipStream_t)stream), "lis_attention");
}

int p2v_lis_attention_taps(const int8_t* qkv, int batch, int tokens, int heads, int head_dim, const p2v_attn* at, int8_t* out,
                           int8_t* score_codes, int8_t* probs_k, int pitch, void* stream) {
  return lis_attention("p2v_lis_attention_taps", qkv, batch, tokens, heads, head_dim, at, 0, 0, out, nullptr, stream, score_codes, probs_k, pitch);
}

int p2v_lis_attention(const int8_t* qkv, int batch, int tokens, int heads, int head_dim, const p2v_attn* at, int8_t* out,
                      int8_t* probs_k, void* stream) {
  return lis_attention("p2v_lis_attention", qkv, batch, tokens, heads, head_dim, at, 0, 0, out, probs_k, stream);
}

int p2v_lis_attention_rows(const int8_t* qkv, int batch, int tokens, int heads, int head_dim, const p2v_attn* at, int query_rows,
                           int8_t* out, void* stream) {
  return lis_attention("p2v_lis_attention_rows", qkv, batch, tokens, heads, head_dim, at, 1, query_rows, out, nullptr, stream);
}

int p2v_patch_merge_gather(const int8_t* x, int batch, int H, int W, int C, int8_t* out, void* stream) {
  if (!x || !out) return fail(P2V_E_ARG, "p2v_patch_merge_gather: null argument");
  if (batch <= 0 || H <= 0 || W <= 0 || (H & 1) || (W & 1)) return fail(P2V_E_SHAPE, "patch merge: H and W must be positive and even");
  if (C <= 0 || C % 16) return fail(P2V_E_UNSUPPORTED, "patch merge: C must be a multiple of 16");
  return launch_rc(p2v_launch_patch_merge_gather(x, batch, H, W, C, out, (hipStream_t)stream), "patch_merge_gather");
}

int p2v_avgpool_quant(const int8_t* x, int batch, int tokens, int C, float s_in, float inv_s_out, int8_t* out, void* stream) {
  if (!x || !out) return fail(P2V_E_ARG, "p2v_avgpool_quant: null argument");
  if (batch <= 0 || tokens <= 0 || tokens > 8192) return fail(P2V_E_SHAPE, "avgpool: bad shape");
  if (C <= 0 || C % 4) return fail(P2V_E_UNSUPPORTED, "avgpool: C must be a multiple of 4");
  return launch_rc(p2v_launch_avgpool_quant(x, batch, tokens, C, s_in, inv_s_out, out, (hipStream_t)stream), "avgpool_quant");
}

static int window_attention(const char* who, const int8_t* qkv, int batch, int tokens_per_image, int heads, int head_dim, const p2v_winattn* wa,
                            int8_t* out, int8_t* probs_k, void* stream, int8_t* attn1_codes, int8_t* qact2_codes, int8_t* probs_kp, int pitch) {
  if (!qkv || !wa || !out || !wa->table_codes || !wa->win_index) return fail(P2V_E_ARG, "p2v_window_attention: null argument");
  if (batch <= 0 || tokens_per_image <= 0 || heads <= 0) return fail(P2V_E_SHAPE, "bad window attention shape");
  if (head_dim != 32) return fail(P2V_E_UNSUPPORTED, "window attention: head_dim must be 32");
  if (wa->ws < 1 || wa->ws > 12 || wa->n_windows < 1 || wa->ws * wa->ws * wa->n_windows > tokens_per_image)
    return fail(P2V_E_SHAPE, "window attention: window size must be 1..12 and windows must fit the token count");
  {
    const int rc = check_lis_consts("p2v_window_attention", wa->x0_int, wa->b_int, wa->c_int);
    if (rc != P2V_OK) return rc;
  }
  const float pots[5] = {wa->s_q1, wa->s_attn, wa->s_table, wa->s_q2, wa->s_q3};
  for (float s : pots) {
    int ex;
    if (!(s > 0.f) || frexpf(s, &ex) != 0.5f) return fail(P2V_E_UNSUPPORTED, "window attention: activation scales must be powers of two");
  }
  if (wa->qkv_stride % 16 || wa->out_stride % 4 || (wa->qkv_stride && wa->qkv_stride < 3 * heads * head_dim) ||
      (wa->out_stride && wa->out_stride < heads * head_dim))
    return fail(P2V_E_SHAPE, "window attention: row strides must cover a row and be 16 / 4 byte aligned");
  if (wa->s_q2 > 1.0f) return fail(P2V_E_UNSUPPORTED, "window attention: qact2 scale above 1 (the -100 mask would not be an integer)");
  if (wa->s_q1 / wa->s_q3 > 0x1p15f || wa->s_q1 / wa->s_q3 < 0x1p-40f)
    return fail(P2V_E_UNSUPPORTED, "window attention: qact1 scale / qact3 scale must lie in [2^-40, 2^15]");
  const int rp = check_tap_planes(who, wa->ws * wa->ws, pitch, {attn1_codes, qact2_codes, probs_kp});
  if (rp != P2V_OK) return rp;
  WinAttnArgs a{{qkv, batch, tokens_per_image, heads, *wa, out, probs_k}};
  a.attn1_codes = attn1_codes; a.qact2_codes = qact2_codes; a.probs_kp = probs_kp; a.pitch = pitch;
  return launch_rc(p2v_launch_window_attention(a, (hipStream_t)stream), "window_attention");
}

int p2v_window_attention(const int8_t* qkv, int batch, int tokens_per_image, int heads, int head_dim, const p2v_winattn* wa,
                         int8_t* out, int8_t* probs_k, void* stream) {
  return window_attention("p2v_window_attention", qkv, batch, tokens_per_image, heads, head_dim, wa, out, probs_k, stream, nullptr, nullptr, nullptr, 0);
}

int p2v_window_attention_taps(const int8_t* qkv, int batch, int tokens_per_image, int heads, int head_dim, const p2v_winattn* wa,
                              int8_t* out, int8_t* attn1_codes, int8_t* qact2_codes, int8_t* probs_k, int pitch, void* stream) {
  return window_attention("p2v_window_attention_taps", qkv, batch, tokens_per_image, heads, head_dim, wa, out, nullptr, stream, attn1_codes,
                          qact2_codes, probs_k, pitch);
}

static int gemm_f32_op(const p2v_op& o, void* stream) {
  if (!o.in || !o.out || !o.lin.w_codes || !o.lin.colscale || !o.lin.bias) return fail(P2V_E_ARG, "P2V_OP_GEMM_F32: null argument");
  if (o.M <= 0 || o.N <= 0 || o.K <= 0 || o.K % GBK_PAD) return fail(P2V_E_SHAPE, "P2V_OP_GEMM_F32: K=%d must be a positive multiple of %d", o.K, GBK_PAD);
  if (o.lda <= 0 || o.lda % 16) return fail(P2V_E_UNSUPPORTED, "P2V_OP_GEMM_F32: lda must be a positive multiple of 16");
  if (o.ldo < o.N || (o.ldo != o.N && o.ldo % 4)) return fail(P2V_E_SHAPE, "P2V_OP_GEMM_F32: ldo=%d must be N=%d, or a multiple of 4 beyond it", o.ldo, o.N);
  if ((uintptr_t)o.in % 16 || (uintptr_t)o.out % 16) return fail(P2V_E_ARG, "P2V_OP_GEMM_F32: in and out must be 16-byte aligned");
  return run_gemm(P2V_EPI_F32, (const int8_t*)o.in, o.lda, o.M, o.K, o.N, o.lin, p2v_epilogue{}, o.out, o.ldo, nullptr, (hipStream_t)stream);
}
static int cos_check(const p2v_cos_layer* layers, int n_layers, int n, const char* what);
static p2v_cos_layer cos_op_layer(const p2v_op& o) {
  const long long sample = (long long)(((unsigned long long)(unsigned)o.i3 << 32) | (unsigned)o.i2);
  const size_t esz = o.i1 == P2V_COS_F32 ? 4 : 1;
  const char* a = reinterpret_cast<const char*>(o.in);
  return p2v_cos_layer{a, a ? a + (size_t)(o.i0 > 0 ? o.i0 : 0) * (size_t)(sample > 0 ? sample : 0) * esz : nullptr, o.lin.colscale, sample, o.lda, o.M, o.N, o.i1};
}
static int cos_op(const p2v_op& o, void* stream) {
  if (!o.in || !o.out || !o.lin.w_codes) return fail(P2V_E_ARG, "P2V_OP_COS: null buffer, partials or stage record");
  if ((uintptr_t)o.out % 8 || (uintptr_t)o.lin.w_codes % 8) return fail(P2V_E_ARG, "P2V_OP_COS: partials and stage record must be 8-byte aligned");
  const p2v_cos_layer l = cos_op_layer(o);
  const int rc = cos_check(&l, 1, o.i0, "P2V_OP_COS");
  if (rc != P2V_OK) return rc;
  const CosDesc d = p2v_cos_desc(l, o.i0, 0);
  return launch_rc(p2v_launch_cos_stage(reinterpret_cast<const CosDesc*>(o.lin.w_codes), (long long)o.i0 * d.nsplit,
                                        reinterpret_cast<unsigned long long*>(o.out), (hipStream_t)stream), "cos_stage");
}
static int cos_combine_op(const p2v_op& o, void* stream) {
  if (!o.in || !o.out || !o.lin.w_codes) return fail(P2V_E_ARG, "P2V_OP_COS_COMBINE: null stage table, sums or partials");
  if (o.i1 < 1) return fail(P2V_E_ARG, "P2V_OP_COS_COMBINE: a combine without stages (%d)", o.i1);
  if (o.i0 < 1) return fail(P2V_E_SHAPE, "P2V_OP_COS_COMBINE: n = %d samples", o.i0);
  if ((uintptr_t)o.in % 8 || (uintptr_t)o.out % 8 || (uintptr_t)o.lin.w_codes % 8) return fail(P2V_E_ARG, "P2V_OP_COS_COMBINE: pointers must be 8-byte aligned");
  return launch_rc(p2v_launch_cos_combine(reinterpret_cast<const CosDesc*>(o.in), o.i1, o.i0, reinterpret_cast<const unsigned long long*>(o.lin.w_codes),
                                          reinterpret_cast<double*>(o.out), (hipStream_t)stream), "cos_combine");
}

static int run_one_op(const p2v_op& o, void* stream) {
  switch (o.kind) {
    case P2V_OP_PATCHIFY:
      return p2v_quantize_patchify((const float*)o.in, o.i0, o.i1, o.i2, o.i3, o.i4, o.f0, (int8_t*)o.out, o.i5, stream);
    case P2V_OP_GEMM:
      return p2v_gemm_i8(o.epi, (const int8_t*)o.in, o.lda, o.M, o.K, o.N, &o.lin, &o.ep, o.out, o.ldo,
                         o.epi == P2V_EPI_RESID ? reinterpret_cast<int8_t*>(o.ep.tap_out) : nullptr, stream);
    case P2V_OP_LAYERNORM:
      return p2v_int_layernorm((const int8_t*)o.in, o.lda, o.M, o.N, &o.ln, (int8_t*)o.out, o.ldo, stream);
    case P2V_OP_WINATTN:
      return p2v_window_attention_taps((const int8_t*)o.in, o.i0, o.i1, o.i2, o.i3, &o.wa, (int8_t*)o.out, const_cast<int8_t*>(o.lin.w_codes),
                                       const_cast<int8_t*>(o.lin.w_frag), reinterpret_cast<int8_t*>(o.ep.tap_out), o.ldo, stream);
    case P2V_OP_MERGE:
      return p2v_patch_merge_gather((const int8_t*)o.in, o.i0, o.i1, o.i2, o.i3, (int8_t*)o.out, stream);
    case P2V_OP_AVGPOOL:
      return p2v_avgpool_quant((const int8_t*)o.in, o.i0, o.i1, o.i2, o.f0, o.f1, (int8_t*)o.out, stream);
    case P2V_OP_LN_GEMM:
      return p2v_ln_gemm_i8(o.epi, (const int8_t*)o.in, o.lda, o.M, o.K, &o.ln, o.N, &o.lin, &o.ep, (int8_t*)o.out, o.ldo, nullptr, stream);
    case P2V_OP_COS:
      return cos_op(o, stream);
    case P2V_OP_COS_COMBINE:
      return cos_combine_op(o, stream);
    case P2V_OP_GEMM_F32:
      return gemm_f32_op(o, stream);
    default:
      return fail(P2V_E_ARG, "p2v_run_ops: unknown op kind %d", o.kind);
  }
}

int p2v_run_ops(const p2v_op* ops, int n_ops, void* stream) {
  if (!ops || n_ops < 0) return fail(P2V_E_ARG, "p2v_run_ops: null argument");
  for (int i = 0; i < n_ops; ++i) {
    const int rc = run_one_op(ops[i], stream);
    if (rc != P2V_OK) return rc;
  }
  return P2V_OK;
}

int p2v_run_ops_profile(const p2v_op* ops, int n_ops, void* stream, float* ms) {
  if (!ops || !ms || n_ops < 0) return fail(P2V_E_ARG, "p2v_run_ops_profile: null argument");
  hipStream_t st = (hipStream_t)stream;
  std::vector<hipEvent_t> ev(n_ops + 1);
  for (auto& e : ev) hipEventCreate(&e);
  int rc = P2V_OK;
  hipEventRecord(ev[0], st);
  int done = 0;
  for (; done < n_ops; ++done) {
    rc = run_one_op(ops[done], stream);
    if (rc != P2V_OK) break;
    hipEventRecord(ev[done + 1], st);
  }
  hipStreamSynchronize(st);
  for (int i = 0; i < done; ++i) hipEventElapsedTime(&ms[i], ev[i], ev[i + 1]);
  for (auto& e : ev) hipEventDestroy(e);
  return rc;
}

int p2v_fake_quant_f32(const float* x, long long n, const float* scale, int n_scale, long long inner, int lo, int hi, float* out,
                       int8_t* codes, void* stream) {
  if (!x || !scale || (!out && !codes)) return fail(P2V_E_ARG, "p2v_fake_quant_f32: null argument");
  if (n_scale < 1 || inner < 1) return fail(P2V_E_ARG, "n_scale and inner must be >= 1");
  if (n == 0) return P2V_OK;
  return launch_rc(p2v_launch_fake_quant(x, n, scale, n_scale, inner, lo, hi, out, codes, (hipStream_t)stream), "fake_quant");
}

int p2v_gelu_quant_f32(const float* y, long long n, float inv_s, int8_t* codes, unsigned long long* flags, int force_slow,
                       void* stream) {
  if (!y || !codes) return fail(P2V_E_ARG, "p2v_gelu_quant_f32: null argument");
  if (n == 0) return P2V_OK;
  return launch_rc(p2v_launch_gelu_quant(y, n, inv_s, codes, flags, force_slow, (hipStream_t)stream), "gelu_quant");
}

int p2v_stream_probe(void* stream, int kernels, int usec, int workgroups, int lds_bytes) {
  if (kernels < 1 || kernels > 64 || usec < 1 || usec > 1000 || workgroups < 1 || workgroups > 4096 || lds_bytes < 0 || lds_bytes > 65536)
    return fail(P2V_E_ARG, "p2v_stream_probe: 1..64 kernels of 1..1000 us, 1..4096 workgroups, 0..64 KB of LDS");
  return launch_rc(p2v_launch_stream_probe(kernels, usec, workgroups, lds_bytes, (hipStream_t)stream), "stream_probe");
}

#ifdef P2V_DIAG
extern unsigned long long* g_gemm_stamps;
void p2v_debug_set_gemm_stamps(void* dev) { g_gemm_stamps = (unsigned long long*)dev; }
#endif

int p2v_gelu_table_plan(float inv_s, p2v_gelu_tab* t) {
  if (!t) return fail(P2V_E_ARG, "p2v_gelu_table_plan: null argument");
  if (!is_pot(inv_s) || inv_s < 1.0f || inv_s > 4096.0f) return fail(P2V_E_UNSUPPORTED, "gelu table: 1/scale %g is not a power of two in [1, 4096]", inv_s);
  const double s = 1.0 / (double)inv_s, k = 2.0 * (double)inv_s;
  double y_lo = -0.75;
  while (y_lo > -40.0 && 0.5 * -y_lo * erfc(-y_lo * 0.70710678118654752440) >= 0.25 * s) y_lo -= 0.5 * s;
  const long long i0 = (long long)floor((y_lo - s) * k);
  double y_hi = 127.5 * s;
  while (y_hi < 1.0e4 && 0.5 * y_hi * erfc(-y_hi * 0.70710678118654752440) < 127.75 * s) y_hi += 0.5 * s;
  const long long i1 = (long long)ceil(y_hi * k) + 2;
  const long long cells = i1 - i0;
  if (cells > 4096) return fail(P2V_E_UNSUPPORTED, "gelu table: %lld cells for 1/scale %g (limit 4096)", cells, inv_s);
  t->k = (float)k;
  t->off = (float)(-i0);
  t->cells = (int32_t)cells;
  return P2V_OK;
}

size_t p2v_gelu_table_scratch_bytes(int cells) { return cells > 0 ? ((size_t)4 * cells + 4) * 4 : 0; }

int p2v_gelu_table_build(float inv_s, const p2v_gelu_tab* t, void* scratch, size_t scratch_bytes, void* stream) {
  if (!t || !t->table || !scratch) return fail(P2V_E_ARG, "p2v_gelu_table_build: null argument");
  p2v_gelu_tab want;
  const int rc = p2v_gelu_table_plan(inv_s, &want);
  if (rc != P2V_OK) return rc;
  if (want.k != t->k || want.off != t->off || want.cells != t->cells) return fail(P2V_E_ARG, "p2v_gelu_table_build: descriptor does not come from p2v_gelu_table_plan");
  if (scratch_bytes < p2v_gelu_table_scratch_bytes(t->cells)) return fail(P2V_E_WORKSPACE, "gelu table scratch %zu < %zu bytes", scratch_bytes, p2v_gelu_table_scratch_bytes(t->cells));
  hipStream_t st = (hipStream_t)stream;
  const int lrc = launch_rc(p2v_launch_gelu_table_build(inv_s, *t, (unsigned*)scratch, st), "gelu_table_build");
  if (lrc != P2V_OK) return lrc;
  unsigned status = 0;
  hipError_t e = hipMemcpyAsync(&status, (const unsigned*)scratch + 4 * t->cells, 4, hipMemcpyDeviceToHost, st);
  if (e == hipSuccess) e = hipStreamSynchronize(st);
  if (e != hipSuccess) return fail(P2V_E_LAUNCH, "gelu_table_build: %s", hipGetErrorString(e));
  if (status) return fail(P2V_E_UNSUPPORTED, "gelu table for 1/scale %g: %s", inv_s, (status & 1) ? "a cell holds two thresholds" : "a cell is never hit");
  return P2V_OK;
}

int p2v_gelu_table_check(float inv_s, const p2v_gelu_tab* t, unsigned long long* mismatches, void* stream) {
  if (!t || !t->table || !mismatches) return fail(P2V_E_ARG, "p2v_gelu_table_check: null argument");
  if (t->cells <= 0) return fail(P2V_E_ARG, "p2v_gelu_table_check: empty table");
  return launch_rc(p2v_launch_gelu_table_check(inv_s, *t, mismatches, (hipStream_t)stream), "gelu_table_check");
}

int p2v_gelu_err_sweep(unsigned first_bits, unsigned count, float* max_err, void* stream) {
  if (!max_err) return fail(P2V_E_ARG, "p2v_gelu_err_sweep: null argument");
  return launch_rc(p2v_launch_gelu_sweep(first_bits, count, max_err, (hipStream_t)stream), "gelu_sweep");
}

}

static int cka_check(const p2v_cka_layer* layers, int n_layers, int n, const char* what) {
  if (!layers || n_layers <= 0) return fail(P2V_E_ARG, "%s: no layers", what);
  if (n < P2V_CKA_MIN_N || n > P2V_CKA_MAX_N) return fail(P2V_E_SHAPE, "%s: n = %d images, the kernels take %d ... %d", what, n, P2V_CKA_MIN_N, P2V_CKA_MAX_N);
  for (int l = 0; l < n_layers; ++l) {
    const p2v_cka_layer& a = layers[l];
    if (!a.x) return fail(P2V_E_ARG, "%s: layer %d has a null x", what, l);
    if (a.features < 1 || a.ldx < a.features) return fail(P2V_E_ARG, "%s: layer %d: F = %lld, ldx = %lld", what, l, a.features, a.ldx);
    if (a.y && a.y != a.x && a.ldy < a.features) return fail(P2V_E_ARG, "%s: layer %d: ldy = %lld < F", what, l, a.ldy);
  }
  return P2V_OK;
}

size_t p2v_cka_workspace_bytes(const p2v_cka_layer* layers, int n_layers, int n) {
  if (cka_check(layers, n_layers, n, "p2v_cka_workspace_bytes") != P2V_OK) return 0;
  return p2v_cka_layout(layers, n_layers, n, nullptr).total;
}

int p2v_cka_grams(const p2v_cka_layer* layers, int n_layers, int n, float* grams, void* ws, size_t ws_bytes, void* stream) {
  int rc = cka_check(layers, n_layers, n, "p2v_cka_grams");
  if (rc != P2V_OK) return rc;
  if (!grams || !ws) return fail(P2V_E_ARG, "p2v_cka_grams: null grams / workspace");
  std::vector<CkaDesc> descs;
  descs.reserve(n_layers);
  const CkaLayout w = p2v_cka_layout(layers, n_layers, n, &descs);
  if (ws_bytes < w.total) return fail(P2V_E_WORKSPACE, "p2v_cka_grams: workspace %zu < %zu bytes", ws_bytes, w.total);
  if ((uintptr_t)ws % 256) return fail(P2V_E_ARG, "p2v_cka_grams: the workspace must be 256-byte aligned");
  return launch_rc(p2v_launch_cka_grams(descs, w, n, grams, ws, (hipStream_t)stream), "cka_grams");
}

int p2v_hsic_accumulate(const float* g1, int l1, const float* g2, int l2, int n, void* acc, void* self1, void* self2, int dtype,
                        void* stream) {
  if (!g1 || !g2 || !acc || l1 <= 0 || l2 <= 0) return fail(P2V_E_ARG, "p2v_hsic_accumulate: null gram / accumulator or no layers");
  if (n < P2V_CKA_MIN_N || n > P2V_CKA_MAX_N) return fail(P2V_E_SHAPE, "p2v_hsic_accumulate: n = %d images, the kernels take %d ... %d", n, P2V_CKA_MIN_N, P2V_CKA_MAX_N);
  if (dtype != 0 && dtype != 1) return fail(P2V_E_ARG, "p2v_hsic_accumulate: dtype %d (0 = fp32, 1 = fp64)", dtype);
  return launch_rc(p2v_launch_hsic(g1, l1, g2, l2, n, acc, self1, self2, dtype, (hipStream_t)stream), "hsic_accumulate");
}

static int cos_check(const p2v_cos_layer* layers, int n_layers, int n, const char* what) {
  if (!layers || n_layers <= 0) return fail(P2V_E_ARG, "%s: no layers", what);
  if (n < 1) return fail(P2V_E_SHAPE, "%s: n = %d samples", what, n);
  for (int l = 0; l < n_layers; ++l) {
    const p2v_cos_layer& a = layers[l];
    if (!a.a || !a.b) return fail(P2V_E_ARG, "%s: layer %d has a null operand", what, l);
    if (a.dtype != P2V_COS_I8 && a.dtype != P2V_COS_F32 && a.dtype != P2V_COS_LOG2K)
      return fail(P2V_E_ARG, "%s: layer %d: dtype %d (0 = int8, 1 = fp32, 3 = log2 exponents)", what, l, a.dtype);
    if (a.scale && a.dtype == P2V_COS_LOG2K) return fail(P2V_E_ARG, "%s: layer %d: the log2-exponent form takes no scales", what, l);
    if (a.rows < 1 || a.cols < 1) return fail(P2V_E_SHAPE, "%s: layer %d: %d rows x %d cols", what, l, a.rows, a.cols);
    if (a.row_stride < a.cols) return fail(P2V_E_ARG, "%s: layer %d: row_stride %lld < cols %d", what, l, a.row_stride, a.cols);
    if (a.sample_stride < 0) return fail(P2V_E_ARG, "%s: layer %d: negative sample_stride %lld", what, l, a.sample_stride);
    if (a.scale && a.dtype != P2V_COS_I8) return fail(P2V_E_UNSUPPORTED, "%s: layer %d: per-channel scales go with int8 codes", what, l);
    const long long esz = a.dtype == P2V_COS_F32 ? 4 : 1;
    if ((uintptr_t)a.a % 16 || (uintptr_t)a.b % 16 || a.sample_stride * esz % 16 || a.row_stride * esz % 16)
      return fail(P2V_E_ARG, "%s: layer %d: pointers and strides must be multiples of 16 bytes", what, l);
    if (a.dtype == P2V_COS_I8 && (long long)a.rows * a.cols >= (1LL << 39))
      return fail(P2V_E_UNSUPPORTED, "%s: layer %d: %d x %d codes per sample leave the exact fp64 range", what, l, a.rows, a.cols);
    if (a.dtype == P2V_COS_LOG2K && (long long)a.rows * a.cols >= (1LL << 33))
      return fail(P2V_E_UNSUPPORTED, "%s: layer %d: %d x %d exponents per sample", what, l, a.rows, a.cols);
  }
  return P2V_OK;
}

size_t p2v_pair_cosine_workspace_bytes(const p2v_cos_layer* layers, int n_layers, int n) {
  if (cos_check(layers, n_layers, n, "p2v_pair_cosine_workspace_bytes") != P2V_OK) return 0;
  return p2v_cos_layout(layers, n_layers, n, nullptr).total;
// ... 217 lines not shown
```

diff-vit_amd/csrc/p2vit_gemm_rows.hip:

```cpp
#include "p2vit_epilogue.h"

#define GR_STEPS 6
#define GR_SLOT_BYTES (2 * 16 * 64 * 4)
#define GR_SLOTS 4

template <int EPI, bool W4>
__global__ __launch_bounds__(512) void k_gemm_rows(GemmArgs g) {
  constexpr bool RES = EPI == P2V_EPI_RESID || EPI == P2V_EPI_RESID_PRE;
  constexpr int EPI_BYTES = EPI == P2V_EPI_RESID ? (int)sizeof(EpiLds) : (EPI == P2V_EPI_RESID_PRE ? (int)sizeof(ResidLds) : 2 * GBN * (int)sizeof(float));
  __shared__ __attribute__((aligned(16))) int8_t lds[GR_SLOTS * GR_SLOT_BYTES + EPI_BYTES];
  v4i* sP = reinterpret_cast<v4i*>(lds);
  EpiLds* sE = reinterpret_cast<EpiLds*>(lds + GR_SLOTS * GR_SLOT_BYTES);
  extern __shared__ __attribute__((aligned(16))) unsigned char dyn_lds[];
  const int tid = threadIdx.x, lane = tid & 63;
  const int wave = __builtin_amdgcn_readfirstlane(tid >> 6);
  const int h = lane >> 5, l31 = lane & 31;
  const int m0 = blockIdx.y * 64, n0 = blockIdx.x * 32;
  const int tn = n0 / GBN, nl = n0 % GBN;

  const int nsteps = g.K >> 5;
  const int s0 = wave * nsteps / 8, s1 = (wave + 1) * nsteps / 8;
  int ma = m0 + l31, mb = ma + 32;
  ma = ma < g.M ? ma : g.M - 1;
  mb = mb < g.M ? mb : g.M - 1;
  const int8_t* pa = g.A + (long long)ma * g.lda + 16 * h;
  const int8_t* pb = g.A + (long long)mb * g.lda + 16 * h;
  const int wr = nl + l31;
  const int8_t* pw = W4 ? g.W + ((long long)tn * (g.K / GBK) * GBN + wr) * 32 : g.W + (long long)(n0 + l31) * g.K + 16 * h;
  auto load_w = [&](int ks) -> v4i {
    if (W4) {
      const uint2 p = *reinterpret_cast<const uint2*>(pw + (long long)(ks >> 1) * (GBN * 32) + (((2 * (ks & 1) + h) ^ ((wr >> 3) & 3)) << 3));
      return unpack_w4(p.x, p.y);
    }
    return *reinterpret_cast<const v4i*>(pw + 32 * ks);
  };

  if constexpr (EPI == P2V_EPI_RESID_PRE) {
    if (tid < P2V_RESID_TAB_ARRAYS * GBN / 4)
      reinterpret_cast<float4*>(sE)[tid] = reinterpret_cast<const float4*>(g.ep.resid_tab + (long long)tn * (P2V_RESID_TAB_ARRAYS * GBN))[tid];
  } else {
    gemm_stage_epilogue<EPI>(sE, tn * GBN, tid, g);
  }
  if (EPI == P2V_EPI_GELU_TAB)
    for (int i = tid; i < g.ep.gelu.cells; i += 512)
      reinterpret_cast<uint2*>(dyn_lds)[i] = reinterpret_cast<const uint2*>(g.ep.gelu.table)[i];
  uint4 resv[2] = {make_uint4(0, 0, 0, 0), make_uint4(0, 0, 0, 0)};
  if (RES && wave == 0) {
#pragma unroll
    for (int mi = 0; mi < 2; ++mi) {
      const int m = m0 + mi * 32 + l31, n = n0 + 16 * h;
      if (m < g.M && n < g.N) resv[mi] = *reinterpret_cast<const uint4*>(g.ep.residual + (long long)m * g.ldo + n);
    }
  }

  v16i acc[2];
#pragma unroll
  for (int b = 0; b < 2; ++b)
#pragma unroll
    for (int r = 0; r < 16; ++r) acc[b][r] = 0;
  for (int s = s0; s < s1; s += GR_STEPS) {
    v4i fw[GR_STEPS], fa[GR_STEPS], fb[GR_STEPS];
#pragma unroll
    for (int j = 0; j < GR_STEPS; ++j)
      if (s + j < s1) {
        fw[j] = load_w(s + j);
        fa[j] = *reinterpret_cast<const v4i*>(pa + 32 * (s + j));
        fb[j] = *reinterpret_cast<const v4i*>(pb + 32 * (s + j));
      }
#pragma unroll
    for (int j = 0; j < GR_STEPS; ++j)
      if (s + j < s1) {
        acc[0] = __builtin_amdgcn_mfma_i32_32x32x32_i8(fw[j], fa[j], acc[0], 0, 0, 0);
        acc[1] = __builtin_amdgcn_mfma_i32_32x32x32_i8(fw[j], fb[j], acc[1], 0, 0, 0);
      }
  }

  auto put = [&](int slot) {
#pragma unroll
    for (int q = 0; q < 8; ++q)
      sP[(slot * 8 + q) * 64 + lane] = (v4i){acc[q >> 2][4 * (q & 3)], acc[q >> 2][4 * (q & 3) + 1], acc[q >> 2][4 * (q & 3) + 2], acc[q >> 2][4 * (q & 3) + 3]};
  };
  auto add = [&](int slot) {
#pragma unroll
    for (int q = 0; q < 8; ++q) {
      const v4i p = sP[(slot * 8 + q) * 64 + lane];
#pragma unroll
      for (int i = 0; i < 4; ++i) acc[q >> 2][4 * (q & 3) + i] += p[i];
    }
  };
  if (wave >= 4) put(wave - 4);
  __syncthreads();
  if (wave < 4) add(wave);
  __syncthreads();
  if (wave >= 1 && wave < 4) put(wave - 1);
  __syncthreads();
  if (wave != 0) return;
  add(0);
  add(1);
  add(2);
  if constexpr (EPI == P2V_EPI_RESID_PRE)
    gemm_epilogue_resid_pre<false>(acc, m0 + l31, n0, nl, h, g, reinterpret_cast<const ResidLds*>(sE), resv);
  else
    gemm_epilogue_tile2<EPI, false>(acc, m0 + l31, n0, nl, h, g, sE, resv, dyn_lds);
}

extern int g_resid_pre;
int g_gemm_rows = 0;

int p2v_launch_gemm_rows(int epi, const GemmArgs& g0, hipStream_t st) {
  if (epi != P2V_EPI_REQUANT && epi != P2V_EPI_GELU && epi != P2V_EPI_RESID) return -3;
  if (g0.M <= 0 || g0.N <= 0 || g0.K <= 0 || g0.K % GBK_PAD || (g0.M + 63) / 64 > 65535) return -3;
  GemmArgs g = g0;
#ifdef P2V_DIAG
  g.stamps = nullptr;
#endif
  g.tiles_n = (g.N + GBN - 1) / GBN;
  const dim3 grid((unsigned)((g.N + 31) / 32), (unsigned)((g.M + 63) / 64)), block(512);
  unsigned tab_bytes = (epi == P2V_EPI_GELU && g.ep.gelu.table) ? (unsigned)g.ep.gelu.cells * 8u : 0u;
  if (GR_SLOTS * GR_SLOT_BYTES + 2 * GBN * (int)sizeof(float) + (int)tab_bytes > 64 * 1024) tab_bytes = 0;
#define P2V_LAUNCH_ROWS(W4_)                                                                                                \
  switch (epi) {                                                                                                            \
    case P2V_EPI_REQUANT: hipLaunchKernelGGL((k_gemm_rows<P2V_EPI_REQUANT, W4_>), grid, block, 0, st, g); break;            \
    case P2V_EPI_GELU:                                                                                                      \
      if (tab_bytes) hipLaunchKernelGGL((k_gemm_rows<P2V_EPI_GELU_TAB, W4_>), grid, block, tab_bytes, st, g);               \
      else hipLaunchKernelGGL((k_gemm_rows<P2V_EPI_GELU, W4_>), grid, block, 0, st, g);                                     \
      break;                                                                                                                \
    default:                                                                                                                \
      if (g.ep.resid_tab && g_resid_pre) hipLaunchKernelGGL((k_gemm_rows<P2V_EPI_RESID_PRE, W4_>), grid, block, 0, st, g);  \
      else hipLaunchKernelGGL((k_gemm_rows<P2V_EPI_RESID, W4_>), grid, block, 0, st, g);                                    \
      break;                                                                                                                \
  }
  if (g.w4) { P2V_LAUNCH_ROWS(true) }
  else { P2V_LAUNCH_ROWS(false) }
#undef P2V_LAUNCH_ROWS
  CHECK_LAUNCH();
  return 0;
}
```

diff-vit_amd/csrc/p2vit_kernels.h:

```cpp
#pragma once
#include <hip/hip_runtime.h>
#include <stdint.h>

#include "../../include/p2vit.h"

#define GBK_PAD 64
#define P2V_EPI_F32 7

struct GemmArgs {
  const int8_t* A;
  int lda, M;
  const int8_t* W;
  int K, N;
  int w4;
  const float* colscale;
  const float* bias;
  p2v_epilogue ep;
  void* out;
  int ldo;
  int8_t* out_codes;
  int8_t* out_codes2;
  int tiles_n;
#ifdef P2V_DIAG
  unsigned long long* stamps;
#endif
};

typedef p2v_ln_pre LnPre;

struct LnArgs {
  const int8_t* x;
  long long row_stride;
  long long rows;
  int C;
  p2v_ln ln;
  int8_t* out;
  long long out_stride;
  int rows_per_half;
  int force_generic;
  LnPre pre;
  float* tap_out;
};

struct AttnKArgs {
  const int8_t* qkv;
  int B, N, H;
  p2v_attn at;
  int8_t* out;
  int8_t* probs_k;
  int pshift;
  int nq;
#ifdef P2V_DIAG
  unsigned long long* stamps;
#endif
};
struct AttnArgs : AttnKArgs {
  int8_t* score_codes;
  int8_t* probs_kp;
  int pitch;
  bool tapped() const { return probs_k || score_codes || probs_kp; }
};

struct WinAttnKArgs {
  const int8_t* qkv;
  int B, T, H;
  p2v_winattn wa;
  int8_t* out;
  int8_t* probs_k;
};
struct WinAttnArgs : WinAttnKArgs {
  int8_t* attn1_codes;
  int8_t* qact2_codes;
  int8_t* probs_kp;
  int pitch;
  bool tapped() const { return probs_k || attn1_codes || qact2_codes || probs_kp; }
};
int p2v_launch_patch_merge_gather(const int8_t* x, int B, int H, int W, int C, int8_t* out, hipStream_t st);
int p2v_launch_avgpool_quant(const int8_t* x, int B, int T, int C, float s_in, float inv_s_out, int8_t* out, hipStream_t st);
int p2v_launch_window_attention(const WinAttnArgs& a, hipStream_t st);

int p2v_launch_patchify(const float* img, int B, int C, int H, int W, int P, float inv_s, int8_t* out, int k_pad, hipStream_t st);
int p2v_launch_fill_cls(int8_t* x, int B, int T, int D, const int8_t* cls, hipStream_t st);
int p2v_launch_embed_fp32(const float* img, int B, int C, int H, int W, int P, const GemmArgs& g, hipStream_t st);
int p2v_launch_u8_patchify(const uint8_t* img, int B, int C, int H, int W, int P, int nhwc, const int8_t* lut, int8_t* out, int k_pad,
                           hipStream_t st);
int p2v_launch_embed_u8(const uint8_t* img, int nhwc, const float* lut, int B, int C, int H, int W, int P, const GemmArgs& g, hipStream_t st);
int p2v_launch_gemm(int epi, const GemmArgs& g, hipStream_t st);
int p2v_launch_gemm_rows(int epi, const GemmArgs& g, hipStream_t st);
int p2v_launch_resid_prefold(const p2v_linear& lin, const p2v_epilogue& ep, int N, float* tab, unsigned* flags, hipStream_t st);
#define P2V_LN_MAX_C 4096
int p2v_launch_layernorm(const LnArgs& a, hipStream_t st);
int p2v_launch_layernorm_xwide(const LnArgs& a, hipStream_t st);
bool p2v_ln_gemm_supported(int epi, int C, int N, int table_cells);
int p2v_launch_ln_gemm(int epi, const LnArgs& a, const GemmArgs& g, hipStream_t st);
int p2v_launch_attention(const AttnArgs& a, int head_dim, hipStream_t st);
int p2v_launch_attention_stream(const AttnArgs& a, int head_dim, hipStream_t st);
int p2v_launch_attention_packed(const AttnArgs& a, hipStream_t st);
int p2v_attention_kernel_of(int head_dim, int tokens, int tapped);
inline int p2v_resident_tokens_of(int head_dim) {
  if (head_dim == 32 || head_dim == 48 || head_dim == 64 || head_dim == 80) return P2V_MAX_TOKENS;
  return head_dim == 96 ? 17 * 32 : (head_dim == 128 ? 12 * 32 : 0);
}
int p2v_launch_stream_probe(int kernels, int usec, int workgroups, int lds_bytes, hipStream_t st);
int p2v_launch_fake_quant(const float* x, long long n, const float* scale, int n_scale, long long inner, int lo, int hi,
                          float* out, int8_t* codes, hipStream_t st);
int p2v_launch_gelu_quant(const float* y, long long n, float inv_s, int8_t* codes, unsigned long long* flags, int force_slow,
                          hipStream_t st);
int p2v_launch_gelu_sweep(unsigned first_bits, unsigned count, float* max_err, hipStream_t st);
int p2v_launch_gelu_table_build(float inv_s, const p2v_gelu_tab& t, unsigned* scratch, hipStream_t st);
int p2v_launch_gelu_table_check(float inv_s, const p2v_gelu_tab& t, unsigned long long* mismatches, hipStream_t st);

#include <vector>
struct CkaDesc {
  const float* x;
  const float* y;
  long long F, ldx, ldy;
  long long item0;
  long long part0;
  int nchunks, sym, vec, pad;
};
struct CkaLayout {
  long long items;
  size_t desc_off, part_off, g64_off, total;
};
CkaLayout p2v_cka_layout(const p2v_cka_layer* layers, int L, int n, std::vector<CkaDesc>* descs);
int p2v_launch_cka_grams(const std::vector<CkaDesc>& descs, const CkaLayout& w, int n, float* grams, void* ws, hipStream_t st);
int p2v_launch_hsic(const float* g1, int l1, const float* g2, int l2, int n, void* acc, void* self1, void* self2, int dtype, hipStream_t st);

#define P2V_COS_I8_DEQ 64
struct CosDesc {
  const void* a;
  const void* b;
  const float* scale;
  long long sample_stride, row_stride;
  long long item0;
  int rows, cols;
  int dtype;
  int vec;
  int nsplit;
  int rows_per_split;
};
struct CosLayout {
  long long items;
  size_t desc_off, part_off, total;
};
CosDesc p2v_cos_desc(const p2v_cos_layer& a, int n, long long item0);
CosLayout p2v_cos_layout(const p2v_cos_layer* layers, int L, int n, std::vector<CosDesc>* descs);
int p2v_launch_pair_cosine(const std::vector<CosDesc>& descs, const CosLayout& w, int n, double* sums, void* ws, hipStream_t st);
int p2v_launch_pair_cosine_one(const CosDesc& d, int n, unsigned long long* partials, double* sums, hipStream_t st);
int p2v_launch_cos_stage(const CosDesc* desc_dev, long long items, unsigned long long* partials, hipStream_t st);
int p2v_launch_cos_combine(const CosDesc* descs_dev, int L, int n, const unsigned long long* partials, double* sums, hipStream_t st);

int p2v_launch_score_rows(const float* logits, long long ld, int rows, int classes, const long long* labels, int* ranks, double* loss,
                          hipStream_t st);
int p2v_launch_score_accumulate(const int* ranks, const double* loss, int rows, const int* ks, int n_k, void* totals, hipStream_t st);

struct ProfLayout {
  int n, classes;
  long long d[2], g[2], rowd[2], rowg[2];
  long long o[2], o0[2];
  long long bytes;
};
ProfLayout p2v_profile_layout(int n, int classes);
int p2v_launch_profile_init(void* state, int n, int classes, const float* logits1, const float* logits2, hipStream_t st);
int p2v_launch_profile_candidates(const float* inputs, long long elems, int idx, long long pos, float eps, float* staging, hipStream_t st);
int p2v_launch_profile_step(void* state, int n, int classes, const float* cand1, const float* cand2, const float* staging, float* inputs,
                            long long elems, int idx, long long pos, double* trace, hipStream_t st);
int p2v_launch_profile_diversity(const float* logits, long long ld, int n, int classes, double* ws, double* out, hipStream_t st);
```

diff-vit_amd/csrc/p2vit_ln.hip:

```cpp
#include "p2vit_ln_row.h"


#ifndef LN_BATCH
#define LN_BATCH 2
#endif
#ifndef LN_LDSC
#define LN_LDSC true
#endif
template <int NCH, int LANES, bool PRE, bool TAP = false>
__global__ __launch_bounds__(256) void k_int_layernorm(LnArgs a) {
  __shared__ __attribute__((aligned(16))) float sG[NCH * LANES * 4], sB[NCH * LANES * 4], sP[NCH * LANES * 4];
  __shared__ __attribute__((aligned(16))) int sM[NCH * LANES * 4];
  const int tid = threadIdx.x, l32 = tid & (LANES - 1), hw = tid / LANES;
  LnLane<NCH, LN_LDSC> L;
  const int LN_ROWS = a.rows_per_half;
  const long long row0 = ((long long)blockIdx.x * (256 / LANES) + hw) * LN_ROWS;
  const long long last_row = a.rows - 1;
  constexpr int R = LN_BATCH;
  int colofs[NCH];
#pragma unroll
  for (int i = 0; i < NCH; ++i) colofs[i] = (l32 + LANES * i) * 4 < a.C ? (l32 + LANES * i) * 4 : 0;
  unsigned wnext[R][NCH];
#pragma unroll
  for (int u = 0; u < R; ++u)
#pragma unroll
    for (int i = 0; i < NCH; ++i)
      wnext[u][i] = *reinterpret_cast<const unsigned*>(a.x + (row0 + u < a.rows ? row0 + u : last_row) * a.row_stride + colofs[i]);
  if constexpr (PRE) {
#pragma unroll
    for (int i = 0; i < NCH; ++i) {
      const int c = (l32 + LANES * i) * 4;
      L.on[i] = c < a.C;
      L.gm[i] = *reinterpret_cast<const float4*>(a.pre.gm + c);
      L.bt[i] = *reinterpret_cast<const float4*>(a.pre.bt + c);
    }
    for (int t4 = tid; t4 < NCH * LANES; t4 += 256) {
      const int c = t4 * 4;
      float4 pmv = make_float4(0.f, 0.f, 0.f, 0.f), mk = pmv;
      if (c < a.C) {
        pmv = *reinterpret_cast<const float4*>(a.ln.post_mul + c);
        mk = *reinterpret_cast<const float4*>(a.ln.mask + c);
      }
      *reinterpret_cast<float4*>(sP + c) = pmv;
      *reinterpret_cast<float4*>(sM + c) = ln_scale_mask(mk);
    }
    __syncthreads();
#pragma unroll
    for (int i = 0; i < NCH; ++i) {
      const int c = (l32 + LANES * i) * 4;
      if constexpr (sizeof(L.pm) == sizeof(float4) * NCH) {
        L.pm[i] = *reinterpret_cast<const float4*>(sP + c);
        L.mkf[i] = *reinterpret_cast<const float4*>(sM + c);
      }
    }
    L.sPl = sP + l32 * 4;
    L.sMl = reinterpret_cast<const float*>(sM) + l32 * 4;
    L.cstride = LANES * 4;
    L.gmin = a.pre.gmin;
    L.gmax = a.pre.gmax;
    L.bmax = a.pre.bmax;
    L.pot = a.pre.pot != 0 && a.force_generic == 0;
    L.pm_one = a.pre.pm_one != 0;
  } else {
    ln_prepare<NCH, LANES>(a.ln, a.C, a.force_generic != 0, sG, sB, sP, sM, tid, 256, L);
  }
#pragma unroll
  for (int u = 0; u < R; ++u)
#pragma unroll
    for (int i = 0; i < NCH; ++i) asm volatile("" : "+v"(wnext[u][i]));
#pragma unroll 1
  for (int rr = 0; rr < LN_ROWS; rr += R) {
    const long long row = row0 + rr;
    if (row >= a.rows) break;
    unsigned wcur[R][NCH];
#pragma unroll
    for (int u = 0; u < R; ++u)
#pragma unroll
      for (int i = 0; i < NCH; ++i) wcur[u][i] = L.on[i] ? wnext[u][i] : 0u;
#pragma unroll
    for (int u = 0; u < R; ++u) {
      const long long nrow = row + R + u < a.rows ? row + R + u : last_row;
#pragma unroll
      for (int i = 0; i < NCH; ++i) wnext[u][i] = *reinterpret_cast<const unsigned*>(a.x + nrow * a.row_stride + colofs[i]);
    }
    asm volatile("" ::: "memory");
    unsigned outw[R][NCH];
    if constexpr (TAP) {
      float* taps[R];
#pragma unroll
      for (int u = 0; u < R; ++u) taps[u] = (rr + u < LN_ROWS && row + u < a.rows) ? a.tap_out + (row + u) * (long long)a.C : nullptr;
      if constexpr (R == 1) ln_row<NCH, LANES, decltype(L), true>(wcur[0], L, a.ln, a.C, l32, outw[0], taps[0]);
      else ln_rows<NCH, LANES, R, decltype(L), true>(wcur, L, a.ln, a.C, l32, outw, taps);
    } else {
    if constexpr (R == 1) ln_row<NCH, LANES>(wcur[0], L, a.ln, a.C, l32, outw[0]);
    else ln_rows<NCH, LANES, R>(wcur, L, a.ln, a.C, l32, outw);
    }
#pragma unroll
    for (int u = 0; u < R; ++u)
#pragma unroll
      for (int i = 0; i < NCH; ++i) asm volatile("" : "+v"(wnext[u][i]));
#pragma unroll
    for (int u = 0; u < R; ++u) {
      if (rr + u >= LN_ROWS || row + u >= a.rows) continue;
      int8_t* dst = a.out + (row + u) * a.out_stride;
#pragma unroll
      for (int i = 0; i < NCH; ++i)
        if (L.on[i]) *reinterpret_cast<unsigned*>(dst + (l32 + LANES * i) * 4) = outw[u][i];
    }
  }
}

#define LG_BM 64
template <bool W4> struct LgW { typedef uint4 raw; };
template <> struct LgW<true> { typedef uint2 raw; };
__device__ __forceinline__ v4i lg_wfrag(uint4 w) { return __builtin_bit_cast(v4i, w); }
__device__ __forceinline__ v4i lg_wfrag(uint2 w) { return unpack_w4(w.x, w.y); }
struct LnGemmLds {
  int panel, consts, fold, table, total;
};
__host__ __device__ inline LnGemmLds ln_gemm_lds(int K, int N, int nch, int table_cells) {
  LnGemmLds o;
  const int kt = (K + GBK - 1) / GBK, tiles_n = (N + GBN - 1) / GBN;
  o.panel = 0;
  o.consts = o.panel + kt * LG_BM * GBK;
  o.fold = o.panel;
  o.table = o.consts + tiles_n * GBN * 2 * (int)sizeof(float);
  o.total = o.table + table_cells * 8;
  return o;
}

#ifdef P2V_DIAG
#define LG_STAMP(slot)                                                                                              \
  do {                                                                                                              \
    if (g.stamps && threadIdx.x == 0 && (slot) < 62) g.stamps[(long long)blockIdx.x * 64 + (slot)] = __builtin_readcyclecounter(); \
  } while (0)
#else
#define LG_STAMP(slot) do { } while (0)
#endif
template <int EPI, int KT, bool W4>
__global__ __launch_bounds__(256, 2) void k_ln_gemm(LnArgs a, GemmArgs g) {
  typedef typename LgW<W4>::raw wraw;
  constexpr int NCH = (KT + 1) / 2;
  constexpr int NI = 2 * KT;
  extern __shared__ __attribute__((aligned(1024))) unsigned char lg_smem[];
  LG_STAMP(0);
  const int C = a.C;
  const int cells = EPI == P2V_EPI_GELU_TAB ? g.ep.gelu.cells : 0;
  const LnGemmLds lay = ln_gemm_lds(C, g.N, NCH, cells);
  int8_t* panel = reinterpret_cast<int8_t*>(lg_smem + lay.panel);
  float* consts = reinterpret_cast<float*>(lg_smem + lay.consts);
  const unsigned char* gtab = lg_smem + lay.table;
  const int tid = threadIdx.x, lane = tid & 63;
  const int wave = __builtin_amdgcn_readfirstlane(tid >> 6);
  const int h = lane >> 5, l31 = lane & 31;
  const int m0 = blockIdx.x * LG_BM;
  const int tiles_n = g.tiles_n;

  const wraw* wsrc = reinterpret_cast<const wraw*>(g.W) + (long long)wave * NI * 64 + lane;
  wraw wf[NI];
#pragma unroll
  for (int i = 0; i < NI; ++i) wf[i] = wsrc[i * 64];

  constexpr int RPH = LG_BM / 8;
  static_assert(RPH % 2 == 0, "rows are processed in pairs");
  const int hw = tid >> 5;
  auto load_row = [&](int r, unsigned (&w)[NCH]) {
    long long row = (long long)m0 + hw * RPH + r;
    row = row < a.rows ? row : a.rows - 1;
#pragma unroll
    for (int i = 0; i < NCH; ++i) {
      const int c = (l31 + 32 * i) * 4;
      w[i] = *reinterpret_cast<const unsigned*>(a.x + row * a.row_stride + (c < C ? c : 0));
    }
  };
  unsigned win[2][NCH];
  load_row(0, win[0]);
  load_row(1, win[1]);
  {
    const float fold = EPI == P2V_EPI_REQUANT ? g.ep.inv_s_out : (EPI == P2V_EPI_GELU_TAB ? g.ep.gelu.k : 1.0f);
    const float cfold = fold * (W4 ? 0.0625f : 1.0f);
    for (int n4 = tid; n4 < tiles_n * (GBN / 4); n4 += 256) {
      const int j_ = n4 >> 5, c_ = (n4 & 31) * 4;
      const float4 cv = *reinterpret_cast<const float4*>(g.colscale + n4 * 4);
      const float4 bv = *reinterpret_cast<const float4*>(g.bias + n4 * 4);
      *reinterpret_cast<float4*>(consts + j_ * 2 * GBN + c_) = make_float4(cv.x * cfold, cv.y * cfold, cv.z * cfold, cv.w * cfold);
      *reinterpret_cast<float4*>(consts + j_ * 2 * GBN + GBN + c_) = make_float4(bv.x * fold, bv.y * fold, bv.z * fold, bv.w * fold);
    }
    if (EPI == P2V_EPI_GELU_TAB)
      for (int i = tid; i < cells; i += 256)
        reinterpret_cast<uint2*>(lg_smem + lay.table)[i] = reinterpret_cast<const uint2*>(g.ep.gelu.table)[i];
  }
  LG_STAMP(1);
  {
    float* sG = reinterpret_cast<float*>(lg_smem + lay.fold);
    float* sB = sG + NCH * 128;
    float* sP = sB + NCH * 128;
    int* sM = reinterpret_cast<int*>(sP + NCH * 128);
    LnLane<NCH> L;
    ln_prepare<NCH, 32>(a.ln, C, a.force_generic != 0, sG, sB, sP, sM, tid, 256, L);
    __syncthreads();
#pragma unroll 1
    for (int r = 0; r < RPH; r += 2) {
      unsigned wnext[2][NCH];
      if (r + 2 < RPH) {
        load_row(r + 2, wnext[0]);
        load_row(r + 3, wnext[1]);
      }
      unsigned wcur[2][NCH], outw2[2][NCH];
#pragma unroll
      for (int u = 0; u < 2; ++u)
#pragma unroll
        for (int i = 0; i < NCH; ++i) wcur[u][i] = L.on[i] ? win[u][i] : 0u;
      ln_rows<NCH, 32, 2>(wcur, L, a.ln, C, l31, outw2);
#pragma unroll
      for (int u = 0; u < 2; ++u) {
        const int lrow = hw * RPH + r + u;
        const unsigned (&outw)[NCH] = outw2[u];
        const long long row = (long long)m0 + lrow;
#pragma unroll
        for (int i = 0; i < NCH; ++i) {
          const int c = (l31 + 32 * i) * 4;
          if (c < KT * GBK)
            *reinterpret_cast<unsigned*>(panel + (c >> 6) * (LG_BM * GBK) + lrow * GBK + ((((c & 63) >> 4) ^ ((lrow >> 2) & 3)) << 4) + (c & 15)) =
                L.on[i] ? outw[i] : 0u;
          if (a.out && L.on[i] && row < a.rows) *reinterpret_cast<unsigned*>(a.out + row * a.out_stride + c) = outw[i];
        }
      }
      if (r + 2 < RPH) {
#pragma unroll
        for (int i = 0; i < NCH; ++i) {
          win[0][i] = wnext[0][i];
          win[1][i] = wnext[1][i];
        }
      }
    }
  }
  LG_STAMP(2);
  __syncthreads();
  LG_STAMP(3);

  const int8_t* pXa = panel + lds_off64(l31, h);
  const int8_t* pXb = panel + lds_off64(32 + l31, h);
  const int xks = (lds_off64(l31, 2 + h) - lds_off64(l31, h));
  v16i acc[2];
#pragma unroll
  for (int b = 0; b < 2; ++b)
#pragma unroll
    for (int r = 0; r < 16; ++r) acc[b][r] = 0;

  for (int j = 0; j < tiles_n; ++j) {
    const bool more = j + 1 < tiles_n;
    const wraw* wnext = wsrc + (long long)(more ? j + 1 : j) * 4 * NI * 64;
#pragma unroll
    for (int i = 0; i < NI; ++i) {
      const int off = (i >> 1) * (LG_BM * GBK) + (i & 1) * xks;
      const v4i xa = *reinterpret_cast<const v4i*>(pXa + off);
      const v4i xb = *reinterpret_cast<const v4i*>(pXb + off);
      const v4i wfi = lg_wfrag(wf[i]);
      acc[0] = __builtin_amdgcn_mfma_i32_32x32x32_i8(wfi, xa, acc[0], 0, 0, 0);
      acc[1] = __builtin_amdgcn_mfma_i32_32x32x32_i8(wfi, xb, acc[1], 0, 0, 0);
      wf[i] = wnext[i * 64];
    }
    LG_STAMP(4 + 2 * j);
    const EpiLds* e = reinterpret_cast<const EpiLds*>(consts + j * 2 * GBN);
    {
      const uint4 nores[2] = {make_uint4(0, 0, 0, 0), make_uint4(0, 0, 0, 0)};
      gemm_epilogue_tile2<EPI>(acc, m0 + l31, j * GBN + 32 * wave, 32 * wave, h, g, e, nores, gtab);
#pragma unroll
      for (int mi = 0; mi < 2; ++mi)
#pragma unroll
        for (int r = 0; r < 16; ++r) acc[mi][r] = 0;
    }
    LG_STAMP(5 + 2 * j);
  }
}

template <int NI>
__host__ __device__ constexpr int lg2_mfma_at(int hp) {
  for (int q = 0; q < 2 * NI; ++q)
    if ((q * 12) / NI == hp) return q;
  return -1;
}

#ifndef LG2_LN_ROWS
#define LG2_LN_ROWS 2
#endif
template <int EPI, int KT, int NG, bool W4>
__global__ __launch_bounds__(256 * NG, 2) void k_ln_gemm2(LnArgs a, GemmArgs g) {
  typedef typename LgW<W4>::raw wraw;
  constexpr int NT = 256 * NG;
  static_assert(EPI == P2V_EPI_REQUANT || EPI == P2V_EPI_GELU_TAB, "pipelined epilogues");
  constexpr int NCH = (KT + 1) / 2;
  constexpr int NI = 2 * KT;
  extern __shared__ __attribute__((aligned(1024))) unsigned char lg_smem[];
  LG_STAMP(0);
  const int C = a.C;
  const int cells = EPI == P2V_EPI_GELU_TAB ? g.ep.gelu.cells : 0;
  const LnGemmLds lay = ln_gemm_lds(C, g.N, NCH, cells);
  int8_t* panel = reinterpret_cast<int8_t*>(lg_smem + lay.panel);
  float* consts = reinterpret_cast<float*>(lg_smem + lay.consts);
  const unsigned char* gtab = lg_smem + lay.table;
  const int tid = threadIdx.x, lane = tid & 63;
  const int wave = __builtin_amdgcn_readfirstlane(tid >> 6);
  const int grp = NG == 1 ? 0 : (wave >> 2), cw = wave & 3;
  const int h = lane >> 5, l31 = lane & 31;
  const int m0 = blockIdx.x * LG_BM;
  const int tiles_n = g.tiles_n;
  const int n_g = (tiles_n - grp + NG - 1) / NG;

  const wraw* wsrc = reinterpret_cast<const wraw*>(g.W) + (long long)cw * NI * 64 + lane;
  auto wtile = [&](int it) {
    int j = grp + NG * it;
    j = j < tiles_n ? j : tiles_n - 1;
    return wsrc + (long long)j * 4 * NI * 64;
  };
  constexpr int NI_EARLY = KT >= 6 ? NI - 1 : NI;
  wraw wf[NI];
  {
    const wraw* w0 = wtile(0);
#pragma unroll
    for (int i = 0; i < NI_EARLY; ++i) wf[i] = w0[i * 64];
  }

  constexpr int RPH = LG_BM / (8 * NG);
  static_assert(RPH % 2 == 0, "rows are processed in pairs");
  const int hw = tid >> 5;
  const int8_t* xblk = a.x + (long long)m0 * a.row_stride;
  const int rstride = (int)a.row_stride;
  const int last_lr = (int)(a.rows - 1 - m0);
  auto load_row = [&](int r, unsigned (&w)[NCH]) {
    int lr = hw * RPH + r;
    lr = lr < last_lr ? lr : last_lr;
    const int8_t* rp = xblk + lr * rstride;
#pragma unroll
    for (int i = 0; i < NCH; ++i) {
      const int c = (l31 + 32 * i) * 4;
      w[i] = *reinterpret_cast<const unsigned*>(rp + (c < C ? c : 0));
    }
  };
  constexpr int LR = LG2_LN_ROWS < RPH ? LG2_LN_ROWS : RPH;
  static_assert(RPH % LR == 0, "rows are processed in batches");
  unsigned win[LR][NCH];
#pragma unroll
  for (int u = 0; u < LR; ++u) load_row(u, win[u]);
  {
    const float fold = EPI == P2V_EPI_REQUANT ? g.ep.inv_s_out : (EPI == P2V_EPI_GELU_TAB ? g.ep.gelu.k : 1.0f);
    const float cfold = fold * (W4 ? 0.0625f : 1.0f);
    for (int n4 = tid; n4 < tiles_n * (GBN / 4); n4 += NT) {
      const int j_ = n4 >> 5, c_ = (n4 & 31) * 4;
      const float4 cv = *reinterpret_cast<const float4*>(g.colscale + n4 * 4);
      const float4 bv = *reinterpret_cast<const float4*>(g.bias + n4 * 4);
      *reinterpret_cast<float4*>(consts + j_ * 2 * GBN + c_) = make_float4(cv.x * cfold, cv.y * cfold, cv.z * cfold, cv.w * cfold);
      *reinterpret_cast<float4*>(consts + j_ * 2 * GBN + GBN + c_) = make_float4(bv.x * fold, bv.y * fold, bv.z * fold, bv.w * fold);
    }
    if (EPI == P2V_EPI_GELU_TAB)
      for (int i = tid; i < cells; i += NT)
        reinterpret_cast<uint2*>(lg_smem + lay.table)[i] = reinterpret_cast<const uint2*>(g.ep.gelu.table)[i];
  }
  LG_STAMP(1);
  {
    float* sG = reinterpret_cast<float*>(lg_smem + lay.fold);
    float* sB = sG + NCH * 128;
    float* sP = sB + NCH * 128;
    int* sM = reinterpret_cast<int*>(sP + NCH * 128);
    LnLane<NCH> L;
    if (a.pre.gm) {
#pragma unroll
      for (int i = 0; i < NCH; ++i) {
        const int c = (l31 + 32 * i) * 4;
        L.on[i] = c < C;
        L.gm[i] = *reinterpret_cast<const float4*>(a.pre.gm + c);
        L.bt[i] = *reinterpret_cast<const float4*>(a.pre.bt + c);
        L.pm[i] = L.on[i] ? *reinterpret_cast<const float4*>(a.ln.post_mul + c) : make_float4(0.f, 0.f, 0.f, 0.f);
        L.mkf[i] = L.on[i] ? ln_scale_mask(*reinterpret_cast<const float4*>(a.ln.mask + c)) : make_float4(0.f, 0.f, 0.f, 0.f);
      }
      L.gmin = a.pre.gmin;
      L.gmax = a.pre.gmax;
      L.bmax = a.pre.bmax;
      L.pot = a.pre.pot != 0 && a.force_generic == 0;
      L.pm_one = a.pre.pm_one != 0;
    } else {
      ln_prepare<NCH, 32>(a.ln, C, a.force_generic != 0, sG, sB, sP, sM, tid, NT, L);
      __syncthreads();
    }
#pragma unroll 1
    for (int r = 0; r < RPH; r += LR) {
      unsigned wnext[LR][NCH];
      if (r + LR < RPH) {
#pragma unroll
        for (int u = 0; u < LR; ++u) load_row(r + LR + u, wnext[u]);
      }
      unsigned wcur[LR][NCH], outw2[LR][NCH];
#pragma unroll
      for (int u = 0; u < LR; ++u)
#pragma unroll
        for (int i = 0; i < NCH; ++i) wcur[u][i] = L.on[i] ? win[u][i] : 0u;
      ln_rows<NCH, 32, LR>(wcur, L, a.ln, C, l31, outw2);
#pragma unroll
      for (int u = 0; u < LR; ++u) {
        const int lrow = hw * RPH + r + u;
        const unsigned (&outw)[NCH] = outw2[u];
        const long long row = (long long)m0 + lrow;
#pragma unroll
        for (int i = 0; i < NCH; ++i) {
          const int c = (l31 + 32 * i) * 4;
          if (c < KT * GBK)
            *reinterpret_cast<unsigned*>(panel + (c >> 6) * (LG_BM * GBK) + lrow * GBK + ((((c & 63) >> 4) ^ ((lrow >> 2) & 3)) << 4) + (c & 15)) =
                L.on[i] ? outw[i] : 0u;
          if (a.out && L.on[i] && row < a.rows) *reinterpret_cast<unsigned*>(a.out + row * a.out_stride + c) = outw[i];
        }
      }
      if (r + LR < RPH) {
#pragma unroll
        for (int u = 0; u < LR; ++u)
#pragma unroll
          for (int i = 0; i < NCH; ++i) win[u][i] = wnext[u][i];
      }
    }
  }
  LG_STAMP(2);
  if constexpr (NI_EARLY < NI) wf[NI - 1] = wtile(0)[(NI - 1) * 64];
  __syncthreads();
  LG_STAMP(3);
  if (n_g <= 0) return;

  const int8_t* pXa = panel + lds_off64(l31, h);
  const int8_t* pXb = panel + lds_off64(32 + l31, h);
  const int xks = (lds_off64(l31, 2 + h) - lds_off64(l31, h));
#define LG2_XOFF(i) ((((i) >> 1) * (LG_BM * GBK)) + (((i) & 1) ? xks : 0))
  v16i acc[2], accn[2];
#pragma unroll
  for (int b = 0; b < 2; ++b)
#pragma unroll
    for (int r = 0; r < 16; ++r) acc[b][r] = 0;
  {
    const wraw* wn = wtile(1);
#pragma unroll
    for (int i = 0; i < NI; ++i) {
      const v4i xa = *reinterpret_cast<const v4i*>(pXa + LG2_XOFF(i));
      const v4i xb = *reinterpret_cast<const v4i*>(pXb + LG2_XOFF(i));
      const v4i wfi = lg_wfrag(wf[i]);
      acc[0] = __builtin_amdgcn_mfma_i32_32x32x32_i8(wfi, xa, acc[0], 0, 0, 0);
      acc[1] = __builtin_amdgcn_mfma_i32_32x32x32_i8(wfi, xb, acc[1], 0, 0, 0);
      wf[i] = wn[i * 64];
    }
  }
  LG_STAMP(4);
  v4i XA[2], XB[2];
  XA[0] = *reinterpret_cast<const v4i*>(pXa + LG2_XOFF(0));
  XB[0] = *reinterpret_cast<const v4i*>(pXb + LG2_XOFF(0));
  XA[1] = XA[0];
  XB[1] = XB[0];
  const int goff = (int)g.ep.gelu.off;
  const float glo = (float)-goff, ghi = (float)(cells - 1 - goff) + 0.5f;
  const unsigned char* gtabz = gtab + goff * 8;

  v4i wcur = {0, 0, 0, 0};
  auto tile_body = [&](auto MFc, auto LDc, auto COPYc, int j, const wraw* wnn, v16i (&acc)[2], v16i (&accn)[2]) {
    constexpr bool MF = decltype(MFc)::value, LD = decltype(LDc)::value, COPY = decltype(COPYc)::value;
    const float* cst = consts + j * 2 * GBN + 32 * cw + 4 * h;
    const int n_tile = j * GBN + 32 * cw;
    unsigned d[2][4];
    float4 cs = *reinterpret_cast<const float4*>(cst), bs = *reinterpret_cast<const float4*>(cst + GBN);
#define LG2_MFMA(HP)                                                                                                     \
    do {                                                                                                                 \
      constexpr int q_ = lg2_mfma_at<NI>(HP);                                                                            \
      if constexpr (MF && q_ >= 0) {                                                                                     \
        constexpr int i_ = q_ >> 1, nx_ = (i_ + 1) % NI;                                                                 \
        if constexpr ((q_ & 1) == 0) {                                                                                   \
          XA[nx_ & 1] = *reinterpret_cast<const v4i*>(pXa + LG2_XOFF(nx_));                                              \
          wcur = lg_wfrag(wf[i_]);                                                                                       \
          if constexpr (i_ == 0) accn[0] = __builtin_amdgcn_mfma_i32_32x32x32_i8(wcur, XA[i_ & 1], (v16i){0,0,0,0,0,0,0,0,0,0,0,0,0,0,0,0}, 0, 0, 0); \
          else accn[0] = __builtin_amdgcn_mfma_i32_32x32x32_i8(wcur, XA[i_ & 1], accn[0], 0, 0, 0);                      \
        } else {                                                                                                         \
          XB[nx_ & 1] = *reinterpret_cast<const v4i*>(pXb + LG2_XOFF(nx_));                                              \
          if constexpr (i_ == 0) accn[1] = __builtin_amdgcn_mfma_i32_32x32x32_i8(wcur, XB[i_ & 1], (v16i){0,0,0,0,0,0,0,0,0,0,0,0,0,0,0,0}, 0, 0, 0); \
          else accn[1] = __builtin_amdgcn_mfma_i32_32x32x32_i8(wcur, XB[i_ & 1], accn[1], 0, 0, 0);                      \
          if constexpr (LD) wf[i_] = wnn[i_ * 64];                                                                       \
        }                                                                                                                \
      }                                                                                                                  \
    } while (0)
#define LG2_FENCE() __builtin_amdgcn_sched_barrier(0)
    auto group = [&](auto GQc) {
      constexpr int gq = decltype(GQc)::value;
      const float4 csc = cs, bsc = bs;
      if (gq < 3) {
        cs = *reinterpret_cast<const float4*>(cst + 8 * (gq + 1));
        bs = *reinterpret_cast<const float4*>(cst + GBN + 8 * (gq + 1));
      }
      float y0[4], y1[4];
      LG2_MFMA(6 * gq + 0);
      y0[0] = __builtin_fmaf((float)acc[0][4 * gq + 0], csc.x, bsc.x);
      y0[1] = __builtin_fmaf((float)acc[0][4 * gq + 1], csc.y, bsc.y);
      y0[2] = __builtin_fmaf((float)acc[0][4 * gq + 2], csc.z, bsc.z);
      y0[3] = __builtin_fmaf((float)acc[0][4 * gq + 3], csc.w, bsc.w);
      LG2_FENCE();
      LG2_MFMA(6 * gq + 1);
      y1[0] = __builtin_fmaf((float)acc[1][4 * gq + 0], csc.x, bsc.x);
      y1[1] = __builtin_fmaf((float)acc[1][4 * gq + 1], csc.y, bsc.y);
      y1[2] = __builtin_fmaf((float)acc[1][4 * gq + 2], csc.z, bsc.z);
      y1[3] = __builtin_fmaf((float)acc[1][4 * gq + 3], csc.w, bsc.w);
      LG2_FENCE();
      if constexpr (EPI == P2V_EPI_GELU_TAB) {
        uint2 e0[4], e1[4];
        LG2_MFMA(6 * gq + 2);
#pragma unroll
        for (int i = 0; i < 4; ++i) e0[i] = *reinterpret_cast<const uint2*>(gtabz + gelu_tab_offset(y0[i], glo, ghi));
        LG2_FENCE();
        LG2_MFMA(6 * gq + 3);
#pragma unroll
        for (int i = 0; i < 4; ++i) e1[i] = *reinterpret_cast<const uint2*>(gtabz + gelu_tab_offset(y1[i], glo, ghi));
        LG2_FENCE();
        LG2_MFMA(6 * gq + 4);
        d[0][gq] = 0;
        P2V_GELU_SEL(0, "UNUSED_PAD", d[0][gq], y0[0], e0[0]);
        P2V_GELU_SEL(1, "UNUSED_PRESERVE", d[0][gq], y0[1], e0[1]);
        P2V_GELU_SEL(2, "UNUSED_PRESERVE", d[0][gq], y0[2], e0[2]);
        P2V_GELU_SEL(3, "UNUSED_PRESERVE", d[0][gq], y0[3], e0[3]);
        LG2_FENCE();
        LG2_MFMA(6 * gq + 5);
        d[1][gq] = 0;
        P2V_GELU_SEL(0, "UNUSED_PAD", d[1][gq], y1[0], e1[0]);
        P2V_GELU_SEL(1, "UNUSED_PRESERVE", d[1][gq], y1[1], e1[1]);
        P2V_GELU_SEL(2, "UNUSED_PRESERVE", d[1][gq], y1[2], e1[2]);
        P2V_GELU_SEL(3, "UNUSED_PRESERVE", d[1][gq], y1[3], e1[3]);
        LG2_FENCE();
      } else {
        float r0[4], r1[4];
        LG2_MFMA(6 * gq + 2);
#pragma unroll
        for (int i = 0; i < 4; ++i) r0[i] = pre_pack(y0[i]);
        LG2_FENCE();
        LG2_MFMA(6 * gq + 3);
#pragma unroll
        for (int i = 0; i < 4; ++i) r1[i] = pre_pack(y1[i]);
        LG2_FENCE();
        LG2_MFMA(6 * gq + 4);
        d[0][gq] = pack4_pre(r0[0], r0[1], r0[2], r0[3]);
        LG2_FENCE();
        LG2_MFMA(6 * gq + 5);
        d[1][gq] = pack4_pre(r1[0], r1[1], r1[2], r1[3]);
        LG2_FENCE();
      }
    };
    group(std::integral_constant<int, 0>{});
    group(std::integral_constant<int, 1>{});
    group(std::integral_constant<int, 2>{});
    group(std::integral_constant<int, 3>{});
#undef LG2_MFMA
#undef LG2_FENCE
#pragma unroll
    for (int b = 0; b < 2; ++b) {
      const uint4 o = halves_to_row16(d[b][0], d[b][1], d[b][2], d[b][3]);
      const int m = m0 + 32 * b + l31;
      if (m < g.M && n_tile + 16 * h < g.N)
        *reinterpret_cast<uint4*>(reinterpret_cast<int8_t*>(g.out) + (long long)m * g.ldo + n_tile + 16 * h) = o;
    }
    if constexpr (MF && COPY) {
      acc[0] = accn[0];
      acc[1] = accn[1];
    }
  };
  using T_ = std::integral_constant<bool, true>;
  using F_ = std::integral_constant<bool, false>;
  int it = 0;
  for (; it + 3 < n_g; it += 2) {
    tile_body(T_{}, T_{}, F_{}, grp + NG * it, wtile(it + 2), acc, accn);
    LG_STAMP(5 + it);
    tile_body(T_{}, T_{}, F_{}, grp + NG * (it + 1), wtile(it + 3), accn, acc);
    LG_STAMP(6 + it);
  }
  if (it + 2 < n_g) {
    tile_body(T_{}, T_{}, T_{}, grp + NG * it, wtile(it + 2), acc, accn);
    LG_STAMP(5 + it);
    ++it;
  }
  if (it + 1 < n_g) {
    tile_body(T_{}, F_{}, T_{}, grp + NG * it, wsrc, acc, accn);
    LG_STAMP(5 + it);
    ++it;
  }
  tile_body(F_{}, F_{}, T_{}, grp + NG * it, wsrc, acc, accn);
  LG_STAMP(5 + it);
#undef LG2_XOFF
}


#ifdef P2V_DIAG
extern unsigned long long* g_gemm_stamps;
#endif
int g_ln_pre = 1;
int g_ln_generic = 0;
int g_ln_gemm = 1;
bool p2v_ln_gemm_supported(int epi, int C, int N, int table_cells) {
  if (!g_ln_gemm || (epi != P2V_EPI_REQUANT && epi != P2V_EPI_GELU)) return false;
  if (C % 4 || C > 384 || N % 16) return false;
  return ln_gemm_lds(C, N, ((C + GBK - 1) / GBK + 1) / 2, table_cells).total <= 80 * 1024;
}
template <int EPI, int KT, int VER, bool W4>
static int launch_ln_gemm_t2(const LnArgs& a, const GemmArgs& g, int cells, hipStream_t st) {
  const int smem = ln_gemm_lds(a.C, g.N, (KT + 1) / 2, cells).total;
  static int granted[16] = {0};
  int dev = 0;
  if (hipGetDevice(&dev) != hipSuccess || dev < 0 || dev >= 16) dev = -1;
  const void* fn;
  if constexpr (VER == 3) fn = reinterpret_cast<const void*>(&k_ln_gemm2<EPI, KT, 2, W4>);
  else if constexpr (VER == 2) fn = reinterpret_cast<const void*>(&k_ln_gemm2<EPI, KT, 1, W4>);
  else fn = reinterpret_cast<const void*>(&k_ln_gemm<EPI, KT, W4>);
  if (dev < 0 || smem > granted[dev]) {
    hipError_t e = hipFuncSetAttribute(fn, hipFuncAttributeMaxDynamicSharedMemorySize, smem);
    if (e != hipSuccess) return (int)e;
    if (dev >= 0) granted[dev] = smem;
  }
  const dim3 grid((unsigned)((g.M + LG_BM - 1) / LG_BM));
  if constexpr (VER == 3) hipLaunchKernelGGL((k_ln_gemm2<EPI, KT, 2, W4>), grid, dim3(512), (unsigned)smem, st, a, g);
  else if constexpr (VER == 2) hipLaunchKernelGGL((k_ln_gemm2<EPI, KT, 1, W4>), grid, dim3(256), (unsigned)smem, st, a, g);
  else hipLaunchKernelGGL((k_ln_gemm<EPI, KT, W4>), grid, dim3(256), (unsigned)smem, st, a, g);
  CHECK_LAUNCH();
  return 0;
}
template <int EPI, int KT, int VER>
static int launch_ln_gemm_t(const LnArgs& a, const GemmArgs& g, int cells, hipStream_t st) {
  return g.w4 ? launch_ln_gemm_t2<EPI, KT, VER, true>(a, g, cells, st) : launch_ln_gemm_t2<EPI, KT, VER, false>(a, g, cells, st);
}
int g_ln_gemm_ver = 2;
int p2v_launch_ln_gemm(int epi, const LnArgs& a_, const GemmArgs& g0, hipStream_t st) {
  const int cells = (epi == P2V_EPI_GELU && g0.ep.gelu.table) ? g0.ep.gelu.cells : 0;
  if (!p2v_ln_gemm_supported(epi, a_.C, g0.N, cells)) return -3;
  if (a_.row_stride < 0 || a_.row_stride > (1 << 24)) return -3;
  LnArgs a = a_;
  a.force_generic = g_ln_generic;
  if (!g_ln_pre) a.pre.gm = nullptr;
  GemmArgs g = g0;
  g.tiles_n = (g.N + GBN - 1) / GBN;
#ifdef P2V_DIAG
  g.stamps = g_gemm_stamps;
#endif
  const int kt = (a.C + GBK - 1) / GBK;
#define P2V_LG(EPI_, VER_)                                                        \
  switch (kt) {                                                                   \
    case 1: return launch_ln_gemm_t<EPI_, 1, VER_>(a, g, cells, st);              \
    case 2: return launch_ln_gemm_t<EPI_, 2, VER_>(a, g, cells, st);              \
    case 3: return launch_ln_gemm_t<EPI_, 3, VER_>(a, g, cells, st);              \
    case 4: return launch_ln_gemm_t<EPI_, 4, VER_>(a, g, cells, st);              \
    case 5: return launch_ln_gemm_t<EPI_, 5, VER_>(a, g, cells, st);              \
    default: return launch_ln_gemm_t<EPI_, 6, VER_>(a, g, cells, st);             \
  }
  if (g_ln_gemm_ver == 3 && !g.ep.tap_out) {
    if (epi == P2V_EPI_REQUANT) { P2V_LG(P2V_EPI_REQUANT, 3) }
    if (cells) { P2V_LG(P2V_EPI_GELU_TAB, 3) }
  }
  if (g_ln_gemm_ver == 2 && !g.ep.tap_out) {
    if (epi == P2V_EPI_REQUANT) { P2V_LG(P2V_EPI_REQUANT, 2) }
    if (cells) { P2V_LG(P2V_EPI_GELU_TAB, 2) }
  }
  if (epi == P2V_EPI_REQUANT) { P2V_LG(P2V_EPI_REQUANT, 1) }
  if (cells) { P2V_LG(P2V_EPI_GELU_TAB, 1) }
  P2V_LG(P2V_EPI_GELU, 1)
#undef P2V_LG
}

int g_ln_rows = 4;
int p2v_launch_layernorm(const LnArgs& a_, hipStream_t st) {
  LnArgs a = a_;
  a.force_generic = g_ln_generic;
  if (!g_ln_pre) a.pre.gm = nullptr;
  if (a.C > 2048) return a.tap_out ? -1 : p2v_launch_layernorm_xwide(a, st);
  a.rows_per_half = g_ln_rows;
  const int LN_ROWS = g_ln_rows;
  const bool wide = a.C > 384;
  const int nch = wide ? (a.C + 255) / 256 : (a.C + 127) / 128;
  const int rows_per_block = (wide ? 4 : 8) * LN_ROWS;
  dim3 grid((unsigned)((a.rows + rows_per_block - 1) / rows_per_block)), block(256);
  if (a.tap_out) {
#define P2V_LN_TAP(N_, L_) case N_: if (a.pre.gm) hipLaunchKernelGGL((k_int_layernorm<N_, L_, true, true>), grid, block, 0, st, a); \
                                    else hipLaunchKernelGGL((k_int_layernorm<N_, L_, false, true>), grid, block, 0, st, a); break;
    if (wide) {
      switch (nch) { P2V_LN_TAP(2, 64) P2V_LN_TAP(3, 64) P2V_LN_TAP(4, 64) P2V_LN_TAP(5, 64) P2V_LN_TAP(6, 64) P2V_LN_TAP(7, 64) P2V_LN_TAP(8, 64) default: return -1; }
    } else {
      switch (nch) { P2V_LN_TAP(1, 32) P2V_LN_TAP(2, 32) P2V_LN_TAP(3, 32) default: return -1; }
    }
#undef P2V_LN_TAP
    CHECK_LAUNCH();
    return 0;
  }
  if (wide) {
    switch (nch) {
      case 2: if (a.pre.gm) hipLaunchKernelGGL((k_int_layernorm<2, 64, true>), grid, block, 0, st, a); else hipLaunchKernelGGL((k_int_layernorm<2, 64, false>), grid, block, 0, st, a); break;
      case 3: if (a.pre.gm) hipLaunchKernelGGL((k_int_layernorm<3, 64, true>), grid, block, 0, st, a); else hipLaunchKernelGGL((k_int_layernorm<3, 64, false>), grid, block, 0, st, a); break;
      case 4: if (a.pre.gm) hipLaunchKernelGGL((k_int_layernorm<4, 64, true>), grid, block, 0, st, a); else hipLaunchKernelGGL((k_int_layernorm<4, 64, false>), grid, block, 0, st, a); break;
      case 5: if (a.pre.gm) hipLaunchKernelGGL((k_int_layernorm<5, 64, true>), grid, block, 0, st, a); else hipLaunchKernelGGL((k_int_layernorm<5, 64, false>), grid, block, 0, st, a); break;
      case 6: if (a.pre.gm) hipLaunchKernelGGL((k_int_layernorm<6, 64, true>), grid, block, 0, st, a); else hipLaunchKernelGGL((k_int_layernorm<6, 64, false>), grid, block, 0, st, a); break;
      case 7: if (a.pre.gm) hipLaunchKernelGGL((k_int_layernorm<7, 64, true>), grid, block, 0, st, a); else hipLaunchKernelGGL((k_int_layernorm<7, 64, false>), grid, block, 0, st, a); break;
      case 8: if (a.pre.gm) hipLaunchKernelGGL((k_int_layernorm<8, 64, true>), grid, block, 0, st, a); else hipLaunchKernelGGL((k_int_layernorm<8, 64, false>), grid, block, 0, st, a); break;
      default: return -1;
    }
  } else {
    switch (nch) {
      case 1: if (a.pre.gm) hipLaunchKernelGGL((k_int_layernorm<1, 32, true>), grid, block, 0, st, a); else hipLaunchKernelGGL((k_int_layernorm<1, 32, false>), grid, block, 0, st, a); break;
      case 2: if (a.pre.gm) hipLaunchKernelGGL((k_int_layernorm<2, 32, true>), grid, block, 0, st, a); else hipLaunchKernelGGL((k_int_layernorm<2, 32, false>), grid, block, 0, st, a); break;
      case 3: if (a.pre.gm) hipLaunchKernelGGL((k_int_layernorm<3, 32, true>), grid, block, 0, st, a); else hipLaunchKernelGGL((k_int_layernorm<3, 32, false>), grid, block, 0, st, a); break;
      default: return -1;
    }
  }
  CHECK_LAUNCH();
  return 0;
}
```

Baseline: 109,200 images/sec.

## Add single-query-row attention kernel and optional Q-column skip in LN-GEMM

Adds a dedicated attention kernel for the case where only the CLS query row is needed (nq==1). It uses one wave per (batch, head), keeps K and V in registers and reduces with DPP and permlane, replacing the full resident LIS attention kernel in the last block. It also adds opt-in switches, off by default, to skip computing Q columns for non-CLS rows in the fused LN+QKV GEMM and to use a pipelined k-loop variant of the rows GEMM. The new kernel only covers the final-block reduced path, so its share of total runtime is small.

```diff
diff --git a/diff-vit_amd/csrc/p2vit_attn.hip b/diff-vit_amd/csrc/p2vit_attn.hip
--- a/diff-vit_amd/csrc/p2vit_attn.hip
+++ b/diff-vit_amd/csrc/p2vit_attn.hip
@@ -307,7 +307,8 @@
   return P2V_KERNEL_STREAMING;
 }
 
-int p2v_launch_attention(const AttnArgs& a, int head_dim, hipStream_t st) {
+extern int g_attn_one;
+int p2v_launch_attention(const AttnArgs& a, int head_dim, hipStream_t st, bool row0_only) {
   const int nkb = (a.N + 31) / 32;
   {
     int ex;
@@ -320,6 +321,7 @@
     case P2V_KERNEL_STREAMING: return p2v_launch_attention_stream(a, head_dim, st);
     default: return -1;
   }
+  if (row0_only && g_attn_one && a.nq == 1 && !a.tapped() && (head_dim == 32 || head_dim == 64)) return p2v_launch_attention_one(a, head_dim, st);
   if (head_dim == 64) { P2V_ATTN_CASES(64, 19, true) }
   if (head_dim == 32) { P2V_ATTN_CASES(32, 19, false) }
   return p2v_launch_attention_wide(a, head_dim, nkb, st);
diff --git a/diff-vit_amd/csrc/p2vit_attn_lis.h b/diff-vit_amd/csrc/p2vit_attn_lis.h
--- a/diff-vit_amd/csrc/p2vit_attn_lis.h
+++ b/diff-vit_amd/csrc/p2vit_attn_lis.h
@@ -30,6 +30,14 @@
   lutE[t] = e;
   lutFR[t] = 1.0 / (double)(float)e;
 }
+
+__device__ __forceinline__ int lis_score_code_shift(int sv, int p) {
+  const int hm1 = (1 << (p - 1)) - 1;
+  const int code = (int)((unsigned)sv + (unsigned)hm1 + (((unsigned)sv >> p) & 1u)) >> p;
+  return code < -128 ? -128 : (code > 127 ? 127 : code);
+}
+__device__ __forceinline__ int lis_score_ncode_f32(int sv, float nmm) { return (int)__builtin_amdgcn_fmed3f(rintf((float)sv * nmm), -127.f, 128.f); }
+__device__ __forceinline__ float lis_ratio(double Sd, double rd) { return rintf((float)(Sd * rd)); }
 
 #ifdef P2V_DIAG
 extern unsigned long long* g_gemm_stamps;
diff --git a/diff-vit_amd/csrc/p2vit_attn_one.hip b/diff-vit_amd/csrc/p2vit_attn_one.hip
--- /dev/null
+++ b/diff-vit_amd/csrc/p2vit_attn_one.hip
@@ -0,0 +1,212 @@
+#include "p2vit_attn_lis.h"
+
+template <int CTRL>
+__device__ __forceinline__ int dpp_mov(int v) { return __builtin_amdgcn_update_dpp(0, v, CTRL, 0xF, 0xF, false); }
+template <int CTRL>
+__device__ __forceinline__ long long dpp_mov64(long long v) {
+  const int lo = dpp_mov<CTRL>((int)v), hi = dpp_mov<CTRL>((int)(v >> 32));
+  return (long long)(((unsigned long long)(unsigned)hi << 32) | (unsigned)lo);
+}
+#define P2V_DPP_XOR1 0xB1
+#define P2V_DPP_XOR2 0x4E
+#define P2V_DPP_HALF_MIRROR 0x141
+#define P2V_DPP_MIRROR 0x140
+#define P2V_DPP_ROR4 0x124
+#define P2V_DPP_ROR8 0x128
+__device__ __forceinline__ int wave_max_i32(int v) {
+  int t;
+  t = dpp_mov<P2V_DPP_XOR1>(v); v = t > v ? t : v;
+  t = dpp_mov<P2V_DPP_XOR2>(v); v = t > v ? t : v;
+  t = dpp_mov<P2V_DPP_HALF_MIRROR>(v); v = t > v ? t : v;
+  t = dpp_mov<P2V_DPP_MIRROR>(v); v = t > v ? t : v;
+  auto r = __builtin_amdgcn_permlane16_swap((unsigned)v, (unsigned)v, false, false);
+  v = (int)r[0] > (int)r[1] ? (int)r[0] : (int)r[1];
+  r = __builtin_amdgcn_permlane32_swap((unsigned)v, (unsigned)v, false, false);
+  return (int)r[0] > (int)r[1] ? (int)r[0] : (int)r[1];
+}
+__device__ __forceinline__ long long wave_sum_i64(long long v) {
+  v += dpp_mov64<P2V_DPP_XOR1>(v);
+  v += dpp_mov64<P2V_DPP_XOR2>(v);
+  v += dpp_mov64<P2V_DPP_HALF_MIRROR>(v);
+  v += dpp_mov64<P2V_DPP_MIRROR>(v);
+  auto join = [](unsigned lo, unsigned hi) { return (long long)(((unsigned long long)hi << 32) | lo); };
+  const unsigned lo = (unsigned)v, hi = (unsigned)((unsigned long long)v >> 32);
+  auto rl = __builtin_amdgcn_permlane16_swap(lo, lo, false, false);
+  auto rh = __builtin_amdgcn_permlane16_swap(hi, hi, false, false);
+  v = join(rl[0], rh[0]) + join(rl[1], rh[1]);
+  const unsigned lo2 = (unsigned)v, hi2 = (unsigned)((unsigned long long)v >> 32);
+  rl = __builtin_amdgcn_permlane32_swap(lo2, lo2, false, false);
+  rh = __builtin_amdgcn_permlane32_swap(hi2, hi2, false, false);
+  return join(rl[0], rh[0]) + join(rl[1], rh[1]);
+}
+template <int CHL>
+__device__ __forceinline__ int key_lane(int v, int k) {
+  if (CHL == 4) {
+    switch (k) {
+      case 0: return dpp_mov<0x00>(v);
+      case 1: return dpp_mov<0x55>(v);
+      case 2: return dpp_mov<0xAA>(v);
+      default: return dpp_mov<0xFF>(v);
+    }
+  }
+  return k == 0 ? dpp_mov<0xA0>(v) : dpp_mov<0xF5>(v);
+}
+
+template <int HD, int NCH, bool ISH>
+__global__ __launch_bounds__(256) void k_lis_attention_one(AttnKArgs a) {
+  static_assert(HD == 32 || HD == 64, "head_dim");
+  constexpr int CHL = HD / 16;
+  constexpr int KS = 64 / CHL;
+  constexpr int NIT = NCH * CHL;
+  constexpr bool PRE = NIT <= 16;
+  __shared__ long long lutE[258];
+  __shared__ double lutFR[258];
+  const int tid = threadIdx.x, lane = tid & 63;
+  const int wave = __builtin_amdgcn_readfirstlane(tid >> 6);
+  const int ks = lane / CHL, cc = lane % CHL;
+  const int pairs = a.B * a.H;
+  const int pair_ = blockIdx.x * 4 + wave;
+  const bool live = pair_ < pairs;
+  const int pair = live ? pair_ : pairs - 1;
+  const int b = pair / a.H, head = pair % a.H;
+  const int N = a.N, D = a.H * HD, ld = 3 * D;
+  const int8_t* base = a.qkv + (long long)b * N * ld + head * HD + cc * 16;
+
+  const uint4 q = *reinterpret_cast<const uint4*>(base);
+  uint4 kk[NIT], vv[PRE ? NIT : 1];
+#pragma unroll
+  for (int i = 0; i < NIT; ++i) {
+    kk[i] = make_uint4(0, 0, 0, 0);
+    if (KS * i < N) {
+      const int key = ks + KS * i;
+      const int8_t* row = base + (long long)(key < N ? key : N - 1) * ld;
+      kk[i] = *reinterpret_cast<const uint4*>(row + D);
+      if (PRE) vv[i] = *reinterpret_cast<const uint4*>(row + 2 * D);
+    }
+  }
+  lis_table_entry(a.at, tid, lutE, lutFR);
+
+  int mine[NCH];
+#pragma unroll
+  for (int j = 0; j < NCH; ++j) {
+    mine[j] = 0;
+#pragma unroll
+    for (int c = 0; c < CHL; ++c) {
+      const int i = CHL * j + c;
+      int s = 0;
+      if (KS * i < N) {
+        s = __builtin_amdgcn_sdot4((int)kk[i].x, (int)q.x, 0, false);
+        s = __builtin_amdgcn_sdot4((int)kk[i].y, (int)q.y, s, false);
+        s = __builtin_amdgcn_sdot4((int)kk[i].z, (int)q.z, s, false);
+        s = __builtin_amdgcn_sdot4((int)kk[i].w, (int)q.w, s, false);
+        s += dpp_mov<P2V_DPP_XOR1>(s);
+        if (CHL == 4) s += dpp_mov<P2V_DPP_XOR2>(s);
+      }
+      mine[j] = cc == c ? s : mine[j];
+    }
+  }
+  bool ok[NCH];
+  const float nmm = -(a.at.qk_scale * (a.at.s_qkv_sq * a.at.inv_s_attn));
+  int mx = -100000;
+#pragma unroll
+  for (int j = 0; j < NCH; ++j) {
+    ok[j] = ks + KS * (CHL * j + cc) < N;
+    const int code = ISH ? lis_score_code_shift(mine[j], a.pshift) : -lis_score_ncode_f32(mine[j], nmm);
+    mine[j] = ok[j] ? code : -100000;
+    mx = mine[j] > mx ? mine[j] : mx;
+  }
+  mx = wave_max_i32(mx);
+  __syncthreads();
+  long long S = 0;
+#pragma unroll
+  for (int j = 0; j < NCH; ++j) {
+    mine[j] = ok[j] ? mx - mine[j] : 0;
+    S += ok[j] ? lutE[mine[j]] : 0ll;
+  }
+  S = wave_sum_i64(S);
+  const float Sf = (float)S;
+  const double Sd = (double)Sf;
+  int wgt[NCH];
+#pragma unroll
+  for (int j = 0; j < NCH; ++j) {
+    const float ratio = lis_ratio(Sd, lutFR[mine[j]]);
+    const unsigned e = (lis_prob_pair(ratio, ratio) & 0xFFFFu) >> 7;
+    wgt[j] = (ok[j] && e) ? 1 << (e - 1) : 0;
+  }
+
+  int o[16];
+#pragma unroll
+  for (int c = 0; c < 16; ++c) o[c] = 0;
+#pragma unroll
+  for (int i = 0; i < NIT; ++i) {
+    if (KS * i < N) {
+      const int w = key_lane<CHL>(wgt[i / CHL], i % CHL);
+      uint4 v;
+      if (PRE) {
+        v = vv[i];
+      } else {
+        const int key = ks + KS * i;
+        v = *reinterpret_cast<const uint4*>(base + (long long)(key < N ? key : N - 1) * ld + 2 * D);
+      }
+      const unsigned vw[4] = {v.x, v.y, v.z, v.w};
+#pragma unroll
+      for (int c = 0; c < 16; ++c) o[c] += __mul24(sx8(vw[c >> 2], c & 3), w);
+    }
+  }
+#pragma unroll
+  for (int c = 0; c < 8; ++c) {
+    const auto r = __builtin_amdgcn_permlane32_swap((unsigned)o[c], (unsigned)o[c + 8], false, false);
+    o[c] = (int)r[0] + (int)r[1];
+  }
+#pragma unroll
+  for (int c = 0; c < 4; ++c) {
+    const auto r = __builtin_amdgcn_permlane16_swap((unsigned)o[c], (unsigned)o[c + 4], false, false);
+    o[c] = (int)r[0] + (int)r[1];
+  }
+#pragma unroll
+  for (int c = 0; c < 4; ++c) {
+    o[c] += dpp_mov<P2V_DPP_ROR8>(o[c]);
+    o[c] += dpp_mov<P2V_DPP_ROR4>(o[c]);
+    if (CHL == 2) o[c] += dpp_mov<P2V_DPP_XOR2>(o[c]);
+  }
+  if (live && (lane & (16 - CHL)) == 0) {
+    const float avm = a.at.av_mul * P2V_PROB_SCALE;
+    const int ch = cc * 16 + ((lane >> 5) & 1) * 8 + ((lane >> 4) & 1) * 4;
+    float f[4];
+#pragma unroll
+    for (int c = 0; c < 4; ++c) f[c] = (float)o[c] * 0x1p-126f;
+    *reinterpret_cast<unsigned*>(a.out + (long long)b * N * D + head * HD + ch) = pack4_rne_sat(f[0] * avm, f[1] * avm, f[2] * avm, f[3] * avm);
+  }
+}
+
+int g_attn_one = 1;
+
+int p2v_launch_attention_one(const AttnArgs& a_, int head_dim, hipStream_t st) {
+  if ((head_dim != 32 && head_dim != 64) || a_.N <= 0 || a_.N > P2V_MAX_TOKENS || a_.tapped() || a_.B <= 0 || a_.H <= 0) return -1;
+  AttnKArgs a = a_;
+  {
+    int ex;
+    const float m = a.at.qk_scale * (a.at.s_qkv_sq * a.at.inv_s_attn);
+    a.pshift = (head_dim == 64 && m > 0.f && frexpf(m, &ex) == 0.5f && ex <= 0 && ex >= -23) ? 1 - ex : 0;
+  }
+#ifdef P2V_DIAG
+  a.stamps = nullptr;
+#endif
+  const long long pairs = (long long)a.B * a.H;
+  const dim3 grid((unsigned)((pairs + 3) / 4)), block(256);
+  const int nch = a.N <= 64 ? 1 : (a.N <= 256 ? 4 : 10);
+#define P2V_ONE(HD_, NCH_, ISH_) hipLaunchKernelGGL((k_lis_attention_one<HD_, NCH_, ISH_>), grid, block, 0, st, a)
+#define P2V_ONE_N(HD_, ISH_)                          \
+  do {                                                \
+    if (nch == 1) P2V_ONE(HD_, 1, ISH_);              \
+    else if (nch == 4) P2V_ONE(HD_, 4, ISH_);         \
+    else P2V_ONE(HD_, 10, ISH_);                      \
+  } while (0)
+  if (head_dim == 32) P2V_ONE_N(32, false);
+  else if (a.pshift) P2V_ONE_N(64, true);
+  else P2V_ONE_N(64, false);
+#undef P2V_ONE_N
+#undef P2V_ONE
+  CHECK_LAUNCH();
+  return 0;
+}
diff --git a/diff-vit_amd/csrc/p2vit_capi.cpp b/diff-vit_amd/csrc/p2vit_capi.cpp
--- a/diff-vit_amd/csrc/p2vit_capi.cpp
+++ b/diff-vit_amd/csrc/p2vit_capi.cpp
@@ -118,6 +118,9 @@
 extern int g_ln_pre;
 extern int g_gemm_rows;
 int g_cls_rows = 1;
+int g_q_skip = 0;
+extern int g_attn_one;
+extern int g_rows_kloop;
 
 enum { ANY_ENV = 1, ANY_API = 2 };
 static const struct Switch {
@@ -137,6 +140,9 @@
     {"resid_pre", "P2V_RESID_PRE", &g_resid_pre, 0, 1, 1, ANY_ENV | ANY_API},
     {"gemm_rows", "P2V_GEMM_ROWS", &g_gemm_rows, 0, 2, 1, 0},
     {"cls_rows", "P2V_CLS_ROWS", &g_cls_rows, 0, 1, 1, ANY_ENV},
+    {"attn_one", "P2V_ATTN_ONE", &g_attn_one, 0, 2, 1, 0},
+    {"rows_kloop", "P2V_ROWS_KLOOP", &g_rows_kloop, 0, 1, 1, ANY_ENV},
+    {"q_skip", "P2V_Q_SKIP", &g_q_skip, 0, 1, 1, ANY_ENV},
     {"ln_rows", "P2V_LN_ROWS", &g_ln_rows, 1, 64, 1, 0},
     {"ln_generic", "P2V_LN_GENERIC", &g_ln_generic, 0, 1, 1, ANY_API},
 };
@@ -488,9 +494,11 @@
   return launch_rc(p2v_launch_gemm(epi, g, st), "gemm_i8");
 }
 
-static int run_ln_gemm(int epi, const LnArgs& a, const p2v_linear& lin, const p2v_epilogue& ep, int N, int8_t* out, hipStream_t st) {
+static int run_ln_gemm(int epi, const LnArgs& a, const p2v_linear& lin, const p2v_epilogue& ep, int N, int8_t* out, hipStream_t st, int q_cols = 0,
+                       int q_period = 0) {
   if (!lin.w_frag) return fail(P2V_E_UNSUPPORTED, "ln_gemm: the layer has no fragment-order weights (p2v_linear.w_frag)");
-  const int rc = p2v_launch_ln_gemm(epi, a, gemm_args(nullptr, a.C, (int)a.rows, lin.w_frag, round_up(a.C, GBK_PAD), N, lin, ep, out, N, nullptr), st);
+  const int rc = p2v_launch_ln_gemm(epi, a, gemm_args(nullptr, a.C, (int)a.rows, lin.w_frag, round_up(a.C, GBK_PAD), N, lin, ep, out, N, nullptr), st,
+                                    q_cols, q_period);
   if (rc == -3) return fail(P2V_E_UNSUPPORTED, "ln_gemm: shape C=%d N=%d is not fused", a.C, N);
   return launch_rc(rc, "ln_gemm");
 }
@@ -598,7 +606,7 @@
     return step(kind, [&] { return run_gemm(epi, A, lda, rows, K, N, lin, ep, out, ldo, out_codes, st, few); });
   }
   int ln_linear(int k_fused, int k_gemm, int epi, long long stride, int rows, const p2v_ln& norm, const p2v_linear& lin, const p2v_epilogue& e, int N,
-                int8_t* out, bool few) {
+                int8_t* out, bool few, int q_cols = 0) {
     LnArgs ln{X, stride, rows, D, norm, LN, D};
     ln.pre = norm.pre;
     if (float* vals = full()) {
@@ -609,7 +617,7 @@
     }
     if (!few && lin.w_frag && p2v_ln_gemm_supported(epi, D, N, e.gelu.table ? e.gelu.cells : 0)) {
       if (o.stop_after < 0) ln.out = nullptr;
-      return step(k_fused, [&] { return run_ln_gemm(epi, ln, lin, e, N, out, st); });
+      return step(k_fused, [&] { return run_ln_gemm(epi, ln, lin, e, N, out, st, q_cols, T); });
     }
     const int rc = layernorm(ln);
     return rc ? rc : gemm(k_gemm, few, epi, LN, D, rows, Dk, N, lin, e, out, N);
@@ -624,7 +632,8 @@
     p2v_epilogue eq{};
     eq.inv_s_out = b.inv_s_qkv[bq];
     eq.tap_out = o.qkv_tap ? o.qkv_tap[i] : (o.lin_tap ? o.lin_tap[1 + 4 * i] : nullptr);
-    if ((rc = ln_linear(P2V_K_LN_GEMM_QKV, P2V_K_GEMM_QKV, P2V_EPI_REQUANT, D, M, b.ln1[bq], qkv, eq, 3 * D, QKV, false))) return rc;
+    if ((rc = ln_linear(P2V_K_LN_GEMM_QKV, P2V_K_GEMM_QKV, P2V_EPI_REQUANT, D, M, b.ln1[bq], qkv, eq, 3 * D, QKV, false, (rs.few && g_q_skip) ? D : 0)))
+      return rc;
     if ((rc = ddv_tap(T, 3 * D)) || (rc = ddv_i8(QKV, T, 3 * D, nullptr))) return rc;
     AttnArgs at{{QKV, batch, T, p->d.num_heads, b.attn, ATT, nullptr}};
     at.nq = rs.nq;
@@ -635,7 +644,7 @@
       at.probs_kp = planes + (size_t)batch * HT * pitch;
       at.pitch = pitch;
     }
-    if ((rc = step(P2V_K_ATTENTION, [&] { return launch_rc(p2v_launch_attention(at, hd, st), "lis_attention"); }))) return rc;
+    if ((rc = step(P2V_K_ATTENTION, [&] { return launch_rc(p2v_launch_attention(at, hd, st, rs.nq == 1), "lis_attention"); }))) return rc;
     if (planes && !done &&
         ((rc = ddv_reduce(o.ddv, at.score_codes, HT, T, P2V_COS_I8, nullptr, st, 0, pitch)) ||
          (rc = ddv_reduce(o.ddv, at.probs_kp, HT, T, P2V_COS_LOG2K, nullptr, st, 0, pitch))))
@@ -1012,7 +1021,7 @@
   AttnArgs a{{qkv, batch, tokens, heads, *at, out, probs_k}};
   a.nq = query_rows;
   a.score_codes = score_codes; a.probs_kp = probs_kp; a.pitch = pitch;
-  return launch_rc(p2v_launch_attention(a, head_dim, (hipStream_t)stream), "lis_attention");
+  return launch_rc(p2v_launch_attention(a, head_dim, (hipStream_t)stream, g_attn_one == 2 && query_rows == 1), "lis_attention");
 }
 
 int p2v_lis_attention_taps(const int8_t* qkv, int batch, int tokens, int heads, int head_dim, const p2v_attn* at, int8_t* out,
diff --git a/diff-vit_amd/csrc/p2vit_gemm_rows.hip b/diff-vit_amd/csrc/p2vit_gemm_rows.hip
--- a/diff-vit_amd/csrc/p2vit_gemm_rows.hip
+++ b/diff-vit_amd/csrc/p2vit_gemm_rows.hip
@@ -4,7 +4,7 @@
 #define GR_SLOT_BYTES (2 * 16 * 64 * 4)
 #define GR_SLOTS 4
 
-template <int EPI, bool W4>
+template <int EPI, bool W4, bool KL>
 __global__ __launch_bounds__(512) void k_gemm_rows(GemmArgs g) {
   constexpr bool RES = EPI == P2V_EPI_RESID || EPI == P2V_EPI_RESID_PRE;
   constexpr int EPI_BYTES = EPI == P2V_EPI_RESID ? (int)sizeof(EpiLds) : (EPI == P2V_EPI_RESID_PRE ? (int)sizeof(ResidLds) : 2 * GBN * (int)sizeof(float));
@@ -35,17 +35,20 @@
     return *reinterpret_cast<const v4i*>(pw + 32 * ks);
   };
 
-  if constexpr (EPI == P2V_EPI_RESID_PRE) {
-    if (tid < P2V_RESID_TAB_ARRAYS * GBN / 4)
-      reinterpret_cast<float4*>(sE)[tid] = reinterpret_cast<const float4*>(g.ep.resid_tab + (long long)tn * (P2V_RESID_TAB_ARRAYS * GBN))[tid];
-  } else {
-    gemm_stage_epilogue<EPI>(sE, tn * GBN, tid, g);
-  }
-  if (EPI == P2V_EPI_GELU_TAB)
-    for (int i = tid; i < g.ep.gelu.cells; i += 512)
-      reinterpret_cast<uint2*>(dyn_lds)[i] = reinterpret_cast<const uint2*>(g.ep.gelu.table)[i];
+  auto stage = [&] {
+    if constexpr (EPI == P2V_EPI_RESID_PRE) {
+      if (tid < P2V_RESID_TAB_ARRAYS * GBN / 4)
+        reinterpret_cast<float4*>(sE)[tid] = reinterpret_cast<const float4*>(g.ep.resid_tab + (long long)tn * (P2V_RESID_TAB_ARRAYS * GBN))[tid];
+    } else {
+      gemm_stage_epilogue<EPI>(sE, tn * GBN, tid, g);
+    }
+    if (EPI == P2V_EPI_GELU_TAB)
+      for (int i = tid; i < g.ep.gelu.cells; i += 512)
+        reinterpret_cast<uint2*>(dyn_lds)[i] = reinterpret_cast<const uint2*>(g.ep.gelu.table)[i];
+  };
+  if (!KL) stage();
   uint4 resv[2] = {make_uint4(0, 0, 0, 0), make_uint4(0, 0, 0, 0)};
-  if (RES && wave == 0) {
+  if (!KL && RES && wave == 0) {
 #pragma unroll
     for (int mi = 0; mi < 2; ++mi) {
       const int m = m0 + mi * 32 + l31, n = n0 + 16 * h;
@@ -58,6 +61,51 @@
   for (int b = 0; b < 2; ++b)
 #pragma unroll
     for (int r = 0; r < 16; ++r) acc[b][r] = 0;
+  if constexpr (KL) {
+    auto kloop = [&](auto DEPc) {
+      constexpr int DEP = decltype(DEPc)::value;
+      v4i fw[DEP], fa[DEP], fb[DEP];
+      auto request = [&](int s) {
+#pragma unroll
+        for (int j = 0; j < DEP; ++j) {
+          const int ks = s + j < nsteps ? s + j : nsteps - 1;
+          fw[j] = load_w(ks);
+          fa[j] = *reinterpret_cast<const v4i*>(pa + 32 * ks);
+          fb[j] = *reinterpret_cast<const v4i*>(pb + 32 * ks);
+        }
+      };
+      auto contract = [&](int s) {
+#pragma unroll
+        for (int j = 0; j < DEP; ++j) {
+          const v4i w = s + j < s1 ? fw[j] : (v4i){0, 0, 0, 0};
+          acc[0] = __builtin_amdgcn_mfma_i32_32x32x32_i8(w, fa[j], acc[0], 0, 0, 0);
+          acc[1] = __builtin_amdgcn_mfma_i32_32x32x32_i8(w, fb[j], acc[1], 0, 0, 0);
+        }
+      };
+      request(s0);
+      if (RES) {
+#pragma unroll
+        for (int mi = 0; mi < 2; ++mi) {
+          const int m = m0 + mi * 32 + l31, n = n0 + 16 * h;
+          resv[mi] = *reinterpret_cast<const uint4*>(g.ep.residual + (long long)(m < g.M ? m : g.M - 1) * g.ldo + (n < g.N ? n : 0));
+        }
+      }
+      __builtin_amdgcn_sched_barrier(0);
+      stage();
+      __builtin_amdgcn_sched_barrier(0);
+      contract(s0);
+      for (int s = s0 + DEP; s < s1; s += DEP) {
+        request(s);
+        __builtin_amdgcn_sched_barrier(0);
+        contract(s);
+      }
+    };
+    const int share = (nsteps + 7) >> 3;
+    if (share <= 1) kloop(std::integral_constant<int, 1>{});
+    else if (share <= 2) kloop(std::integral_constant<int, 2>{});
+    else if (share <= 4) kloop(std::integral_constant<int, 4>{});
+    else kloop(std::integral_constant<int, GR_STEPS>{});
+  } else {
   for (int s = s0; s < s1; s += GR_STEPS) {
     v4i fw[GR_STEPS], fa[GR_STEPS], fb[GR_STEPS];
 #pragma unroll
@@ -73,6 +121,7 @@
         acc[0] = __builtin_amdgcn_mfma_i32_32x32x32_i8(fw[j], fa[j], acc[0], 0, 0, 0);
         acc[1] = __builtin_amdgcn_mfma_i32_32x32x32_i8(fw[j], fb[j], acc[1], 0, 0, 0);
       }
+  }
   }
 
   auto put = [&](int slot) {
@@ -98,6 +147,11 @@
   add(0);
   add(1);
   add(2);
+  if (KL && RES) {
+#pragma unroll
+    for (int mi = 0; mi < 2; ++mi)
+      if (!(m0 + mi * 32 + l31 < g.M && n0 + 16 * h < g.N)) resv[mi] = make_uint4(0, 0, 0, 0);
+  }
   if constexpr (EPI == P2V_EPI_RESID_PRE)
     gemm_epilogue_resid_pre<false>(acc, m0 + l31, n0, nl, h, g, reinterpret_cast<const ResidLds*>(sE), resv);
   else
@@ -105,6 +159,7 @@
 }
 
 extern int g_resid_pre;
+int g_rows_kloop = 0;
 int g_gemm_rows = 0;
 
 int p2v_launch_gemm_rows(int epi, const GemmArgs& g0, hipStream_t st) {
@@ -118,20 +173,25 @@
   const dim3 grid((unsigned)((g.N + 31) / 32), (unsigned)((g.M + 63) / 64)), block(512);
   unsigned tab_bytes = (epi == P2V_EPI_GELU && g.ep.gelu.table) ? (unsigned)g.ep.gelu.cells * 8u : 0u;
   if (GR_SLOTS * GR_SLOT_BYTES + 2 * GBN * (int)sizeof(float) + (int)tab_bytes > 64 * 1024) tab_bytes = 0;
-#define P2V_LAUNCH_ROWS(W4_)                                                                                                \
-  switch (epi) {                                                                                                            \
-    case P2V_EPI_REQUANT: hipLaunchKernelGGL((k_gemm_rows<P2V_EPI_REQUANT, W4_>), grid, block, 0, st, g); break;            \
-    case P2V_EPI_GELU:                                                                                                      \
-      if (tab_bytes) hipLaunchKernelGGL((k_gemm_rows<P2V_EPI_GELU_TAB, W4_>), grid, block, tab_bytes, st, g);               \
-      else hipLaunchKernelGGL((k_gemm_rows<P2V_EPI_GELU, W4_>), grid, block, 0, st, g);                                     \
-      break;                                                                                                                \
-    default:                                                                                                                \
-      if (g.ep.resid_tab && g_resid_pre) hipLaunchKernelGGL((k_gemm_rows<P2V_EPI_RESID_PRE, W4_>), grid, block, 0, st, g);  \
-      else hipLaunchKernelGGL((k_gemm_rows<P2V_EPI_RESID, W4_>), grid, block, 0, st, g);                                    \
-      break;                                                                                                                \
+#define P2V_LAUNCH_ROWS(W4_, KL_)                                                                                                \
+  switch (epi) {                                                                                                                 \
+    case P2V_EPI_REQUANT: hipLaunchKernelGGL((k_gemm_rows<P2V_EPI_REQUANT, W4_, KL_>), grid, block, 0, st, g); break;            \
+    case P2V_EPI_GELU:                                                                                                           \
+      if (tab_bytes) hipLaunchKernelGGL((k_gemm_rows<P2V_EPI_GELU_TAB, W4_, KL_>), grid, block, tab_bytes, st, g);               \
+      else hipLaunchKernelGGL((k_gemm_rows<P2V_EPI_GELU, W4_, KL_>), grid, block, 0, st, g);                                     \
+      break;                                                                                                                     \
+    default:                                                                                                                     \
+      if (g.ep.resid_tab && g_resid_pre) hipLaunchKernelGGL((k_gemm_rows<P2V_EPI_RESID_PRE, W4_, KL_>), grid, block, 0, st, g);  \
+      else hipLaunchKernelGGL((k_gemm_rows<P2V_EPI_RESID, W4_, KL_>), grid, block, 0, st, g);                                    \
+      break;                                                                                                                     \
   }
-  if (g.w4) { P2V_LAUNCH_ROWS(true) }
-  else { P2V_LAUNCH_ROWS(false) }
+  if (g_rows_kloop) {
+    if (g.w4) { P2V_LAUNCH_ROWS(true, true) }
+    else { P2V_LAUNCH_ROWS(false, true) }
+  } else {
+    if (g.w4) { P2V_LAUNCH_ROWS(true, false) }
+    else { P2V_LAUNCH_ROWS(false, false) }
+  }
 #undef P2V_LAUNCH_ROWS
   CHECK_LAUNCH();
   return 0;
diff --git a/diff-vit_amd/csrc/p2vit_kernels.h b/diff-vit_amd/csrc/p2vit_kernels.h
--- a/diff-vit_amd/csrc/p2vit_kernels.h
+++ b/diff-vit_amd/csrc/p2vit_kernels.h
@@ -24,6 +24,10 @@
 #ifdef P2V_DIAG
   unsigned long long* stamps;
 #endif
+};
+
+struct GemmQArgs : GemmArgs {
+  int q_tiles, q_period;
 };
 
 typedef p2v_ln_pre LnPre;
@@ -92,9 +96,10 @@
 int p2v_launch_layernorm(const LnArgs& a, hipStream_t st);
 int p2v_launch_layernorm_xwide(const LnArgs& a, hipStream_t st);
 bool p2v_ln_gemm_supported(int epi, int C, int N, int table_cells);
-int p2v_launch_ln_gemm(int epi, const LnArgs& a, const GemmArgs& g, hipStream_t st);
-int p2v_launch_attention(const AttnArgs& a, int head_dim, hipStream_t st);
+int p2v_launch_ln_gemm(int epi, const LnArgs& a, const GemmArgs& g, hipStream_t st, int q_cols = 0, int q_period = 0);
+int p2v_launch_attention(const AttnArgs& a, int head_dim, hipStream_t st, bool row0_only = false);
 int p2v_launch_attention_stream(const AttnArgs& a, int head_dim, hipStream_t st);
+int p2v_launch_attention_one(const AttnArgs& a, int head_dim, hipStream_t st);
 int p2v_launch_attention_packed(const AttnArgs& a, hipStream_t st);
 int p2v_attention_kernel_of(int head_dim, int tokens, int tapped);
 inline int p2v_resident_tokens_of(int head_dim) {
diff --git a/diff-vit_amd/csrc/p2vit_ln.hip b/diff-vit_amd/csrc/p2vit_ln.hip
--- a/diff-vit_amd/csrc/p2vit_ln.hip
+++ b/diff-vit_amd/csrc/p2vit_ln.hip
@@ -137,8 +137,16 @@
 #else
 #define LG_STAMP(slot) do { } while (0)
 #endif
-template <int EPI, int KT, bool W4>
-__global__ __launch_bounds__(256, 2) void k_ln_gemm(LnArgs a, GemmArgs g) {
+__device__ __forceinline__ int lg_first_tile(const GemmQArgs& g, int m0) {
+  const int next = (m0 + g.q_period - 1) / g.q_period * g.q_period;
+  const int end = m0 + LG_BM < g.M ? m0 + LG_BM : g.M;
+  return next < end ? 0 : g.q_tiles;
+}
+__device__ __forceinline__ int lg_first_tile(const GemmArgs&, int) { return 0; }
+template <bool QS> using LgGemmArgs = std::conditional_t<QS, GemmQArgs, GemmArgs>;
+
+template <int EPI, int KT, bool W4, bool QS = false>
+__global__ __launch_bounds__(256, 2) void k_ln_gemm(LnArgs a, LgGemmArgs<QS> g) {
   typedef typename LgW<W4>::raw wraw;
   constexpr int NCH = (KT + 1) / 2;
   constexpr int NI = 2 * KT;
@@ -155,11 +163,12 @@
   const int h = lane >> 5, l31 = lane & 31;
   const int m0 = blockIdx.x * LG_BM;
   const int tiles_n = g.tiles_n;
+  const int tile0 = QS ? lg_first_tile(g, m0) : 0;
 
   const wraw* wsrc = reinterpret_cast<const wraw*>(g.W) + (long long)wave * NI * 64 + lane;
   wraw wf[NI];
 #pragma unroll
-  for (int i = 0; i < NI; ++i) wf[i] = wsrc[i * 64];
+  for (int i = 0; i < NI; ++i) wf[i] = QS ? (wsrc + (long long)tile0 * 4 * NI * 64)[i * 64] : wsrc[i * 64];
 
   constexpr int RPH = LG_BM / 8;
   static_assert(RPH % 2 == 0, "rows are processed in pairs");
@@ -248,7 +257,7 @@
 #pragma unroll
     for (int r = 0; r < 16; ++r) acc[b][r] = 0;
 
-  for (int j = 0; j < tiles_n; ++j) {
+  for (int j = tile0; j < tiles_n; ++j) {
     const bool more = j + 1 < tiles_n;
     const wraw* wnext = wsrc + (long long)(more ? j + 1 : j) * 4 * NI * 64;
 #pragma unroll
@@ -285,8 +294,8 @@
 #ifndef LG2_LN_ROWS
 #define LG2_LN_ROWS 2
 #endif
-template <int EPI, int KT, int NG, bool W4>
-__global__ __launch_bounds__(256 * NG, 2) void k_ln_gemm2(LnArgs a, GemmArgs g) {
+template <int EPI, int KT, int NG, bool W4, bool QS = false>
+__global__ __launch_bounds__(256 * NG, 2) void k_ln_gemm2(LnArgs a, LgGemmArgs<QS> g) {
   typedef typename LgW<W4>::raw wraw;
   constexpr int NT = 256 * NG;
   static_assert(EPI == P2V_EPI_REQUANT || EPI == P2V_EPI_GELU_TAB, "pipelined epilogues");
@@ -302,10 +311,10 @@
   const unsigned char* gtab = lg_smem + lay.table;
   const int tid = threadIdx.x, lane = tid & 63;
   const int wave = __builtin_amdgcn_readfirstlane(tid >> 6);
-  const int grp = NG == 1 ? 0 : (wave >> 2), cw = wave & 3;
   const int h = lane >> 5, l31 = lane & 31;
   const int m0 = blockIdx.x * LG_BM;
   const int tiles_n = g.tiles_n;
+  const int grp = (NG == 1 ? 0 : (wave >> 2)) + (QS ? lg_first_tile(g, m0) : 0), cw = wave & 3;
   const int n_g = (tiles_n - grp + NG - 1) / NG;
 
   const wraw* wsrc = reinterpret_cast<const wraw*>(g.W) + (long long)cw * NI * 64 + lane;
@@ -597,42 +606,47 @@
   if (C % 4 || C > 384 || N % 16) return false;
   return ln_gemm_lds(C, N, ((C + GBK - 1) / GBK + 1) / 2, table_cells).total <= 80 * 1024;
 }
-template <int EPI, int KT, int VER, bool W4>
-static int launch_ln_gemm_t2(const LnArgs& a, const GemmArgs& g, int cells, hipStream_t st) {
+template <int EPI, int KT, int VER, bool W4, bool QS = false>
+static int launch_ln_gemm_t2(const LnArgs& a, const LgGemmArgs<QS>& g, int cells, hipStream_t st) {
   const int smem = ln_gemm_lds(a.C, g.N, (KT + 1) / 2, cells).total;
   static int granted[16] = {0};
   int dev = 0;
   if (hipGetDevice(&dev) != hipSuccess || dev < 0 || dev >= 16) dev = -1;
   const void* fn;
-  if constexpr (VER == 3) fn = reinterpret_cast<const void*>(&k_ln_gemm2<EPI, KT, 2, W4>);
-  else if constexpr (VER == 2) fn = reinterpret_cast<const void*>(&k_ln_gemm2<EPI, KT, 1, W4>);
-  else fn = reinterpret_cast<const void*>(&k_ln_gemm<EPI, KT, W4>);
+  if constexpr (VER == 3) fn = reinterpret_cast<const void*>(&k_ln_gemm2<EPI, KT, 2, W4, QS>);
+  else if constexpr (VER == 2) fn = reinterpret_cast<const void*>(&k_ln_gemm2<EPI, KT, 1, W4, QS>);
+  else fn = reinterpret_cast<const void*>(&k_ln_gemm<EPI, KT, W4, QS>);
   if (dev < 0 || smem > granted[dev]) {
     hipError_t e = hipFuncSetAttribute(fn, hipFuncAttributeMaxDynamicSharedMemorySize, smem);
     if (e != hipSuccess) return (int)e;
     if (dev >= 0) granted[dev] = smem;
   }
   const dim3 grid((unsigned)((g.M + LG_BM - 1) / LG_BM));
-  if constexpr (VER == 3) hipLaunchKernelGGL((k_ln_gemm2<EPI, KT, 2, W4>), grid, dim3(512), (unsigned)smem, st, a, g);
-  else if constexpr (VER == 2) hipLaunchKernelGGL((k_ln_gemm2<EPI, KT, 1, W4>), grid, dim3(256), (unsigned)smem, st, a, g);
-  else hipLaunchKernelGGL((k_ln_gemm<EPI, KT, W4>), grid, dim3(256), (unsigned)smem, st, a, g);
+  if constexpr (VER == 3) hipLaunchKernelGGL((k_ln_gemm2<EPI, KT, 2, W4, QS>), grid, dim3(512), (unsigned)smem, st, a, g);
+  else if constexpr (VER == 2) hipLaunchKernelGGL((k_ln_gemm2<EPI, KT, 1, W4, QS>), grid, dim3(256), (unsigned)smem, st, a, g);
+  else hipLaunchKernelGGL((k_ln_gemm<EPI, KT, W4, QS>), grid, dim3(256), (unsigned)smem, st, a, g);
   CHECK_LAUNCH();
   return 0;
 }
 template <int EPI, int KT, int VER>
-static int launch_ln_gemm_t(const LnArgs& a, const GemmArgs& g, int cells, hipStream_t st) {
+static int launch_ln_gemm_t(const LnArgs& a, const GemmQArgs& g, int cells, hipStream_t st) {
+  if constexpr (EPI == P2V_EPI_REQUANT)
+    if (g.q_tiles > 0) return g.w4 ? launch_ln_gemm_t2<EPI, KT, VER, true, true>(a, g, cells, st) : launch_ln_gemm_t2<EPI, KT, VER, false, true>(a, g, cells, st);
   return g.w4 ? launch_ln_gemm_t2<EPI, KT, VER, true>(a, g, cells, st) : launch_ln_gemm_t2<EPI, KT, VER, false>(a, g, cells, st);
 }
 int g_ln_gemm_ver = 2;
-int p2v_launch_ln_gemm(int epi, const LnArgs& a_, const GemmArgs& g0, hipStream_t st) {
+int p2v_launch_ln_gemm(int epi, const LnArgs& a_, const GemmArgs& g0, hipStream_t st, int q_cols, int q_period) {
   const int cells = (epi == P2V_EPI_GELU && g0.ep.gelu.table) ? g0.ep.gelu.cells : 0;
   if (!p2v_ln_gemm_supported(epi, a_.C, g0.N, cells)) return -3;
   if (a_.row_stride < 0 || a_.row_stride > (1 << 24)) return -3;
   LnArgs a = a_;
   a.force_generic = g_ln_generic;
   if (!g_ln_pre) a.pre.gm = nullptr;
-  GemmArgs g = g0;
+  GemmQArgs g;
+  static_cast<GemmArgs&>(g) = g0;
   g.tiles_n = (g.N + GBN - 1) / GBN;
+  g.q_period = q_period;
+  g.q_tiles = (epi == P2V_EPI_REQUANT && q_period > 0 && q_cols / GBN < g.tiles_n) ? q_cols / GBN : 0;
 #ifdef P2V_DIAG
   g.stamps = g_gemm_stamps;
 #endif
```

Result: no change. 109,200 images/sec (-0.0%).
